# auxten/go-ctr

Measured on AMD Instinct MI355X. Metric: training samples/sec (DIN, MovieLens-20M-shaped synthetic), higher is better.
Workload: dtype f32

## Files before the change

goctr_amd/csrc/ctr.hip:

```cpp
#include <array>
#include <chrono>
#include <cmath>
#include <cstdlib>
#include <map>
#include <memory>

#include "ctr_model.h"
#include "ctr_chain.h"
#include "ctr_chain_x3.h"
#include "emb_train.h"
#include "scan.h"
#include "ctr_serve.h"
#include "mfma_gemm.h"

namespace {

struct TnSchedule { int rows, S, rows_light, S_light; };
TnSchedule tn_schedule(const goctr_model* m, int B) {
  TnSchedule t{};
  const int heavy = (int)cdiv(m->Ip / 16, 3) + (int)cdiv(m->H2p / 16, 3);
  const int light = m->cfg.kind == GOCTR_DIN ? 2 : 1;
  int cus = engine().compute_units > 0 ? engine().compute_units : 256;
  const int lf = 25;
  int rows = 32;
  for (;; rows += 4) {
    const long wgs = (long)heavy * cdiv(B, rows) + (long)light * cdiv(B, round_up(rows * lf / 10, 4));
    if (wgs <= cus || rows >= B) break;
  }
  t.rows = rows; t.S = (int)cdiv(B, rows);
  t.rows_light = round_up(rows * lf / 10, 4); t.S_light = (int)cdiv(B, t.rows_light);
  return t;
}
struct TnWide { bool ok; int ktw0, kblocks0, nbt; int rows0, S0, rows1, S1, rowsL, SL; };
TnWide tn_schedule_wide_search(const goctr_model* m, int B, int nsum);
constexpr int TN_SUM_SLABS = 8;
TnWide tn_schedule_wide(const goctr_model* m, int B, int nsum = 0) {
  static std::mutex mu;
  static std::map<std::array<int, 7>, TnWide> cache;
  const std::array<int, 7> key{B, m->Ip, m->H1p, m->H2p, m->cfg.kind, engine().compute_units, nsum};
  std::lock_guard<std::mutex> lk(mu);
  auto it = cache.find(key);
  if (it != cache.end()) return it->second;
  const TnWide w = tn_schedule_wide_search(m, B, nsum);
  cache.emplace(key, w);
  return w;
}
TnWide tn_schedule_wide_search(const goctr_model* m, int B, int nsum) {
  TnWide w{};
  const int kt0 = m->Ip / 16, nt = m->H1p / 16, kt1 = m->H2p / 16;
  w.ok = (kt0 == 9 || kt0 == 15) && kt1 == 5 && nt > 8 && nt <= 16;
  if (!w.ok) return w;
  w.ktw0 = kt0 == 9 ? 9 : 8; w.kblocks0 = (int)cdiv(kt0, w.ktw0); w.nbt = (int)cdiv(nt, 2);
  const int cols0 = w.ktw0 * 16 + w.nbt * 16, cols1 = kt1 * 16 + w.nbt * 16;
  const int colsL = 16 + kt1 * 16;
  const int blocks0 = w.kblocks0 * 2, blocks1 = 2, light = m->cfg.kind == GOCTR_DIN ? 2 : 1;
  const int cus = engine().compute_units > 0 ? engine().compute_units : 256;
  const int fix0 = 512, fix1 = 384, fixL = 384;
  long best = -1; int bc0 = 0, bc1 = 0, brl = 0;
  const int cmax = (int)cdiv(B, 32);
  for (int c0 = 1; c0 <= cmax; ++c0)
    for (int c1 = 1; c1 <= cmax; ++c1) {
      long t = std::max((long)c0 * cols0 + fix0, (long)c1 * cols1 + fix1);
      if (best >= 0 && t >= best) continue;
      const long heavy = (long)blocks0 * cdiv(B, c0 * 32) + (long)blocks1 * cdiv(B, c1 * 32);
      const int mlight = light - nsum;
      const long room = cus - heavy - (long)nsum * TN_SUM_SLABS;
      const long left = mlight > 0 ? room / mlight : 1;
      if (room < 0 || left < 1) continue;
      const int rl = std::max(32, round_up((int)cdiv(B, left), 4));
      if (mlight > 0) t = std::max(t, (long)cdiv(rl, 32) * colsL + fixL);
      if (best >= 0 && t >= best) continue;
      best = t; bc0 = c0; bc1 = c1; brl = rl;
    }
  if (best < 0) { bc0 = bc1 = cmax; brl = B; }
  w.rows0 = bc0 * 32; w.S0 = (int)cdiv(B, w.rows0);
  w.rows1 = bc1 * 32; w.S1 = (int)cdiv(B, w.rows1);
  w.rowsL = brl; w.SL = (int)cdiv(B, w.rowsL);
  return w;
}
int tn_max_slabs(int B) { return (int)cdiv(B, 32); }
bool dw_wide_path(const goctr_model* m, int B) {
  int nt_max = m->H1p / 16;
  if (m->H2p / 16 > nt_max) nt_max = m->H2p / 16;
  if (m->cfg.kind == GOCTR_DIN && m->Tp / 16 > nt_max) nt_max = m->Tp / 16;
  return gemm_tn_multi_fits(nt_max) && tn_schedule_wide(m, B).ok;
}

}
int ensure_workspace(goctr_model* m, int B) {
  if (m->wsB >= B && m->tnS > 0) return 0;
  const int S = tn_max_slabs(B);
  m->tnS = S;
  if (m->h0.alloc((size_t)B * m->Ip)) return -1;
  if (m->P0.alloc((size_t)B * m->H1p)) return -1;
  if (m->A0.alloc((size_t)B * m->H1p)) return -1;
  if (m->P1.alloc((size_t)B * m->H2p)) return -1;
  if (m->A1.alloc((size_t)B * m->H2p)) return -1;
  if (m->yhat.alloc((size_t)B)) return -1;
  if (m->lossrow.alloc((size_t)B)) return -1;
  if (m->dz2.alloc((size_t)B * 16)) return -1;
  if (m->dz1.alloc((size_t)B * m->H2p)) return -1;
  if (m->dz0.alloc((size_t)B * m->H1p)) return -1;
  if (m->dp.alloc((size_t)B * m->Dp)) return -1;
  if (m->gate.alloc((size_t)2 * B * m->cfg.T)) return -1;
  if (m->wgt.alloc((size_t)2 * B * m->cfg.T)) return -1;
  if (m->gfac.alloc((size_t)2 * B * m->cfg.T)) return -1;
  m->gw_stride = (size_t)B * m->cfg.T;
  if (m->ra_flag.alloc(1)) return -1;
  if (m->slabs0.alloc((size_t)S * m->Ip * m->H1p)) return -1;
  if (m->slabs1.alloc((size_t)S * m->H1p * m->H2p)) return -1;
  if (m->slabs2.alloc((size_t)S * m->H2p * 16)) return -1;
  m->attp_blocks = (int)cdiv(B, ATTN_BWD_WAVES);
  if (m->attp.alloc((size_t)B * m->Tp)) return -1;
  if (m->slabs3.alloc((size_t)S * 16 * m->Tp)) return -1;
  if (m->tile_dw2.alloc((size_t)S * m->H2p) || m->tile_att0.alloc((size_t)S * m->Tp)) return -1;
  {
    std::vector<float> ones((size_t)B * 16, 0.f);
    for (int r = 0; r < B; ++r) ones[(size_t)r * 16] = 1.0f;
    if (m->ones16.alloc(ones.size(), false) || m->ones16.upload(ones.data(), ones.size())) return -1;
  }
  m->wsB = B;
  m->graph.destroy();
  return 0;
}

RowSource make_source(const goctr_dataset* d, const goctr_emb* e) {
  RowSource s{};
  s.rows = d->rows;
  s.Y = d->has_y ? d->Y.p : nullptr;
  s.id_mode = d->id_mode ? 1 : 0;
  if (d->id_mode) {
    s.emb = e->rows.p; s.V = e->V;
    s.ub_ids = d->ub_ids.p; s.item_ids = d->item_ids.p; s.ufeat = d->ufeat.p; s.cfeat = d->cfeat.p;
  } else {
    s.X = d->X.p; s.xcols = d->xcols;
    s.r_u = d->ranges[0]; s.r_ub = d->ranges[2]; s.r_v = d->ranges[4]; s.r_c = d->ranges[6];
  }
  return s;
}
namespace {

int serve16_attributes() {
#define GOCTR_S16(L, H) (allow_big_lds(ctr_serve16_kernel<L, 1, H>) || allow_big_lds(ctr_serve16_kernel<L, 2, H>) || allow_big_lds(ctr_serve16_kernel<L, 3, H>))
  return (GOCTR_S16(2, 10) || GOCTR_S16(2, 15) || GOCTR_S16(4, 10) || GOCTR_S16(4, 15) || GOCTR_S16(16, 10) || GOCTR_S16(16, 15)) ? -1 : 0;
#undef GOCTR_S16
}

template <class Epi>
int launch_nn(int kid, const float* A, int lda, const float* Bm, int ldb, int M, int Kp, int Np, Epi epi) {
  const int NT = Np / 16;
  int WN = NT >= 2 ? 2 : 1;
  while (WN < 4 && (int)cdiv(NT, WN) > GEMM_NN_NTW) WN *= 2;
  int ntw = (int)cdiv(NT, WN);
  if (ntw > GEMM_NN_NTW) ntw = GEMM_NN_NTW;
  ntw = ntw <= 1 ? 1 : (ntw <= 3 ? 3 : (ntw <= 4 ? 4 : 7));
  const int WM = 4 / WN;
  dim3 grid((unsigned)cdiv(M, 16 * WM), (unsigned)cdiv(NT, WN * ntw));
  const int ncols_blk = std::min(NT, WN * ntw) * 16;
  (void)ncols_blk;
  const int ncols_alloc = WN * ntw * 16;
  const int KPH = gemm_nn_phase_rows<float>(Kp, ncols_alloc);
  const size_t lds = gemm_nn_lds_bytes<float>(KPH, ncols_alloc);
  hipStream_t st = engine().active;
  ProfScope ps(kid);
  if (KPH >= Kp && ntw == 4 && (int)grid.x >= 2 * engine().compute_units) {
    const dim3 g2((unsigned)engine().compute_units, grid.y);
    hipLaunchKernelGGL((gemm_nn_rows_kernel<float, Epi, 4>), g2, dim3(256), lds, st, A, lda, Bm, ldb, M, Kp, Np, WN, epi);
    GOCTR_HIP(hipGetLastError());
    return 0;
  }
#define GOCTR_NN(N) hipLaunchKernelGGL((gemm_nn_kernel<float, Epi, N>), grid, dim3(256), lds, st, A, lda, Bm, ldb, M, Kp, Np, WN, KPH, epi)
  switch (ntw) {
    case 1: GOCTR_NN(1); break;
    case 3: GOCTR_NN(3); break;
    case 4: GOCTR_NN(4); break;
    default: GOCTR_NN(7); break;
  }
#undef GOCTR_NN
  GOCTR_HIP(hipGetLastError());
  return 0;
}

template <int KTW, int NTW, int CH>
int launch_tn_cfg(const float* A, int lda, int KT, const float* Dm, int ldd, int NT, int M, int rows_per_wg,
                  int WK, int WN, float* slabs, size_t slab_stride) {
  const int S = (int)cdiv(M, rows_per_wg);
  const int nthreads = 64 * WK * WN;
  GOCTR_CHECK((size_t)CH * (WK * KTW * 16 / 4) <= (size_t)GEMM_TN_MAXVA * nthreads &&
              (size_t)CH * (WN * NTW * 16 / 4) <= (size_t)GEMM_TN_MAXVD * nthreads,
              "gemm_tn: chunk does not fit the staging registers (WK=%d WN=%d)", WK, WN);
  dim3 grid(S, (unsigned)cdiv(KT, WK * KTW), (unsigned)cdiv(NT, WN * NTW));
  hipLaunchKernelGGL((gemm_tn_kernel<float, KTW, NTW, CH>), grid, dim3(nthreads),
                     gemm_tn_lds_bytes<float>(WK * KTW, WN * NTW, CH), engine().active, A, lda, KT, Dm, ldd, NT, M,
                     rows_per_wg, WK, WN, slabs, slab_stride);
  GOCTR_HIP(hipGetLastError());
  return 0;
}

int launch_tn(int kid, const float* A, int lda, int KT, const float* Dm, int ldd, int NT, int M, int rows_per_wg,
              float* slabs, size_t slab_stride) {
  ProfScope ps(kid);
  if (NT <= 3) {
    const int WK = std::min(4, (int)cdiv(KT, 4));
    return launch_tn_cfg<4, 3, 16>(A, lda, KT, Dm, ldd, NT, M, rows_per_wg, WK, 1, slabs, slab_stride);
  }
  if (NT <= 6) {
    const int WK = std::min(4, (int)cdiv(KT, 4)), WN = std::min(2, (int)cdiv(NT, 3));
    return launch_tn_cfg<4, 3, 32>(A, lda, KT, Dm, ldd, NT, M, rows_per_wg, WK, WN, slabs, slab_stride);
  }
  const int WN = std::min(4, (int)cdiv(NT, 4));
  return launch_tn_cfg<3, 4, 32>(A, lda, KT, Dm, ldd, NT, M, rows_per_wg, 1, WN, slabs, slab_stride);
}

}
int init_kernel_attrs() {
  bool& done = engine().kernel_attrs_done;
  if (done) return 0;
#define GOCTR_NN_ATTR(E) (allow_big_lds(gemm_nn_kernel<float, E, 1>) || allow_big_lds(gemm_nn_kernel<float, E, 3>) || \
                          allow_big_lds(gemm_nn_kernel<float, E, 4>) || allow_big_lds(gemm_nn_kernel<float, E, 7>) || \
                          allow_big_lds(gemm_nn_rows_kernel<float, E, 4>))
  if (GOCTR_NN_ATTR(EpiSigDrop) || GOCTR_NN_ATTR(EpiOut) || GOCTR_NN_ATTR(EpiDSig) || GOCTR_NN_ATTR(EpiStore) ||
      allow_big_lds(ctr_chain_kernel<7, 5, 0>) || allow_big_lds(ctr_chain_kernel<7, 5, 1>) ||
      allow_big_lds(ctr_chain_kernel<7, 5, 2>) || allow_big_lds(ctr_fwd16_kernel<4, 5>) || allow_big_lds(emb_grad_kernel<16, 0>) || allow_big_lds(emb_grad_kernel<16, 1>) || allow_big_lds(emb_grad_kernel<16, 2>) || allow_big_lds(emb_grad_kernel<32, 0>) ||
      allow_big_lds(emb_grad_kernel<32, 1>) || allow_big_lds(emb_grad_kernel<32, 2>) || allow_big_lds(emb_grad_kernel<64, 0>) || allow_big_lds(emb_grad_kernel<64, 1>) ||
      allow_big_lds(emb_grad_kernel<64, 2>) || allow_big_lds(gemm_tn_kernel<float, 4, 3, 16>) || allow_big_lds(gemm_tn_kernel<float, 4, 3, 32>) ||
      allow_big_lds(gemm_tn_kernel<float, 3, 4, 32>) ||
      allow_big_lds(gemm_tn_multi_x3_kernel<3, 4>) || allow_big_lds(gemm_tn_multi_x3w_kernel<9, 5>) || allow_big_lds(gemm_tn_multi_x3w_kernel<8, 5>) ||
      allow_big_lds(gemm_tn_multi_x3w_att0_kernel<9, 5>) || allow_big_lds(gemm_tn_multi_x3w_att0_kernel<8, 5>) || allow_big_lds(ctr_chain_x3_kernel<2>) || allow_big_lds(ctr_chain_x3_kernel<9>) ||
      allow_big_lds(ctr_chain_x3_kernel<15>) || chain_x3_fwd_attributes() || fwd4_attributes() ||
      serve16_attributes()) return -1;
  done = true;
  return 0;
}
namespace {

int launch_attn_fwd(const AttnArgs& a) {
  ProfScope ps(GOCTR_K_ATTN_FWD);
  dim3 grid((unsigned)cdiv(a.B, 4)), blk(256);
  hipStream_t st = engine().active;
  const bool vec4 = a.src.id_mode && a.D % 4 == 0;
  const int groups = vec4 ? a.D / 4 : a.D;
  const bool small_table = (unsigned long long)(a.src.V + 1) * (unsigned long long)a.D * 4ull < (1ull << 32);
  const int fast = !(vec4 && small_table && groups * 4 == a.D && (groups & (groups - 1)) == 0) ? 0
                   : a.kind != GOCTR_DIN ? 1 : (a.att == GOCTR_ATT_COSINE ? 2 : 3);
  if (ps.on) {
    static char sym[48];
    int L = 1;
    while (L < groups) L *= 2;
    if (!vec4 && L < 8) L = 8;
    if (a.src.k_users) snprintf(sym, sizeof sym, "attn_fwd_keys_kernel<%d,%d>", std::min(L, 64), fast);
    else snprintf(sym, sizeof sym, "attn_fwd_kernel<%d,%d,%d>", vec4 ? 4 : 1, std::min(L, 64), (fast && groups <= 16) ? fast : 0);
    prof_note_kernel(GOCTR_K_ATTN_FWD, sym);
  }
  if (a.src.k_users) {
    if (!(fast && groups <= 16)) { set_error("attn_fwd: key mode needs an id-mode fast shape"); return -1; }
#define GOCTR_ATTN_KEYS(L)                                                                         \
  do {                                                                                             \
    if (fast == 1) hipLaunchKernelGGL((attn_fwd_keys_kernel<L, 1>), grid, blk, 0, st, a);          \
    else if (fast == 2) hipLaunchKernelGGL((attn_fwd_keys_kernel<L, 2>), grid, blk, 0, st, a);     \
    else hipLaunchKernelGGL((attn_fwd_keys_kernel<L, 3>), grid, blk, 0, st, a);                    \
  } while (0)
    if (groups == 1) GOCTR_ATTN_KEYS(1);
    else if (groups == 2) GOCTR_ATTN_KEYS(2);
    else if (groups == 4) GOCTR_ATTN_KEYS(4);
    else if (groups == 8) GOCTR_ATTN_KEYS(8);
    else GOCTR_ATTN_KEYS(16);
#undef GOCTR_ATTN_KEYS
    GOCTR_HIP(hipGetLastError());
    return 0;
  }
#define GOCTR_ATTN_FWD(V, L) hipLaunchKernelGGL((attn_fwd_kernel<V, L, 0>), grid, blk, 0, st, a)
#define GOCTR_ATTN_FWD_FAST(L)                                                                     \
  do {                                                                                             \
    if (fast == 1) hipLaunchKernelGGL((attn_fwd_kernel<4, L, 1>), grid, blk, 0, st, a);            \
    else if (fast == 2) hipLaunchKernelGGL((attn_fwd_kernel<4, L, 2>), grid, blk, 0, st, a);       \
    else hipLaunchKernelGGL((attn_fwd_kernel<4, L, 3>), grid, blk, 0, st, a);                      \
  } while (0)
  if (fast && groups <= 16) {
    if (groups == 1) GOCTR_ATTN_FWD_FAST(1);
    else if (groups == 2) GOCTR_ATTN_FWD_FAST(2);
    else if (groups == 4) GOCTR_ATTN_FWD_FAST(4);
    else if (groups == 8) GOCTR_ATTN_FWD_FAST(8);
    else GOCTR_ATTN_FWD_FAST(16);
  } else
  if (vec4) {
    if (groups <= 1) GOCTR_ATTN_FWD(4, 1);
    else if (groups <= 2) GOCTR_ATTN_FWD(4, 2);
    else if (groups <= 4) GOCTR_ATTN_FWD(4, 4);
    else if (groups <= 8) GOCTR_ATTN_FWD(4, 8);
    else if (groups <= 16) GOCTR_ATTN_FWD(4, 16);
    else if (groups <= 32) GOCTR_ATTN_FWD(4, 32);
    else GOCTR_ATTN_FWD(4, 64);
  } else {
    if (groups <= 8) GOCTR_ATTN_FWD(1, 8);
    else if (groups <= 16) GOCTR_ATTN_FWD(1, 16);
    else if (groups <= 32) GOCTR_ATTN_FWD(1, 32);
    else GOCTR_ATTN_FWD(1, 64);
  }
#undef GOCTR_ATTN_FWD_FAST
#undef GOCTR_ATTN_FWD
  GOCTR_HIP(hipGetLastError());
  return 0;
}

int launch_attn_bwd(const AttnBwdArgs& a, int blocks) {
  ProfScope ps(GOCTR_K_ATTN_BWD);
  dim3 grid((unsigned)blocks), blk(64 * ATTN_BWD_WAVES);
  hipStream_t st = engine().active;
  const size_t lds = 0;
  const bool vec4 = a.src.id_mode && a.D % 4 == 0;
  const int groups = vec4 ? a.D / 4 : a.D;
  const bool fast = vec4 && groups * 4 == a.D && (groups & (groups - 1)) == 0 && groups <= 16;
#define GOCTR_ATTN_BWD(V, L) hipLaunchKernelGGL((attn_bwd_kernel<V, L, 0>), grid, blk, lds, st, a)
#define GOCTR_ATTN_BWD_FAST(L) hipLaunchKernelGGL((attn_bwd_kernel<4, L, 1>), grid, blk, lds, st, a)
  if (fast) {
    if (groups == 1) GOCTR_ATTN_BWD_FAST(1);
    else if (groups == 2) GOCTR_ATTN_BWD_FAST(2);
    else if (groups == 4) GOCTR_ATTN_BWD_FAST(4);
    else if (groups == 8) GOCTR_ATTN_BWD_FAST(8);
    else GOCTR_ATTN_BWD_FAST(16);
  } else
  if (vec4) {
    if (groups <= 1) GOCTR_ATTN_BWD(4, 1);
    else if (groups <= 2) GOCTR_ATTN_BWD(4, 2);
    else if (groups <= 4) GOCTR_ATTN_BWD(4, 4);
    else if (groups <= 8) GOCTR_ATTN_BWD(4, 8);
    else if (groups <= 16) GOCTR_ATTN_BWD(4, 16);
    else if (groups <= 32) GOCTR_ATTN_BWD(4, 32);
    else GOCTR_ATTN_BWD(4, 64);
  } else {
    if (groups <= 8) GOCTR_ATTN_BWD(1, 8);
    else if (groups <= 16) GOCTR_ATTN_BWD(1, 16);
    else if (groups <= 32) GOCTR_ATTN_BWD(1, 32);
    else GOCTR_ATTN_BWD(1, 64);
  }
#undef GOCTR_ATTN_BWD_FAST
#undef GOCTR_ATTN_BWD
  GOCTR_HIP(hipGetLastError());
  return 0;
}

}
bool chain_ok(const goctr_model* m) {
  const int nt0 = m->H1p / 16;
  return (nt0 == 13 || nt0 == 14) && m->H2p == 80 && (m->cfg.kind != GOCTR_DIN || m->Dp <= 16 * CHAIN_NDP) &&
         m->Ip <= 16 * CHAIN_HV &&
         chain_lds_bytes<5>(m->Ip, m->H1p, m->H2p) <= 160u * 1024u &&
         env_int("GOCTR_NO_CHAIN", 0) == 0;
}
namespace {

bool chain_x3_ok(const goctr_model* m, const StepOpts& o, int B) {
  if (m->x3_nch0 == 0) return false;
  if (o.train) return o.drop_mode != 1;
  const int cus = engine().compute_units > 0 ? engine().compute_units : 256;
  return cdiv(B, 32) >= cus;
}

}
int rebuild_x3_images(goctr_model* m) {
  if (!m->x3_nch0) return 0;
  hipLaunchKernelGGL(x3_build_images_kernel, dim3((unsigned)cdiv(m->off2, 256)), dim3(256), 0, engine().stream, m->W.p, m->off1, m->off2,
                     m->H1p, m->H2p, m->cfg.U, m->cfg.D, m->x3_images());
  GOCTR_HIP(hipGetLastError());
  return 0;
}
namespace {

template <int NCH0>
void launch_chain_x3_n(const ChainX3Args& a, dim3 grid, hipStream_t s, bool fwd) {
  if (fwd) launch_chain_x3_fwd(NCH0, a, grid, s);
  else hipLaunchKernelGGL((ctr_chain_x3_kernel<NCH0, false>), grid, dim3(512), chain_x3_lds_bytes<NCH0>(), s, a);
}

bool emb_plan_active(const goctr_model* m) { return m->emb_lr > 0.f && m->plan.valid; }

bool gate_fac_mode(const goctr_model* m, const RowSource& src, const StepOpts& o, int B);
int launch_chain_x3(goctr_model* m, const RowSource& src, int B, const StepOpts& o, const StepState* st, const FwdBufs& fb) {
  const goctr_ctr_cfg& c = m->cfg;
  Engine& e = engine();
  const uint32_t row_off = (uint32_t)(e.eff_rank() * B);
  const bool drop = o.drop_mode == 2;
  const CxImages im = m->x3_images();
  ChainX3Args a{};
  a.h0 = fb.h0; a.Ip = m->Ip;
  a.img0 = im.img0; a.img1 = im.img1; a.img2 = im.img2; a.img3 = im.img3; a.w2 = m->W2T.p;
  a.H1 = c.H1; a.H2 = c.H2; a.H1p = m->H1p; a.H2p = m->H2p; a.Dp = m->Dp; a.B = B; a.kind = c.kind;
  a.d0 = DropCfg{drop && o.p0 > 0 ? 2 : 0, o.p0, nullptr, c.H1, o.seed, 0u, row_off};
  a.d1 = DropCfg{drop && o.p1 > 0 ? 2 : 0, o.p1, nullptr, c.H2, o.seed, 1u, row_off};
  a.st = st; a.Y = src.Y; a.rows = src.rows; a.inv_bglobal = 1.0f / (float)(B * e.eff_world());
  a.A0 = m->A0.p; a.A1 = m->A1.p; a.dz0 = m->dz0.p; a.dz1 = m->dz1.p; a.dz2 = m->dz2.p; a.dp = m->dp.p;
  m->dpv_from_chain = o.train && emb_plan_active(m) && src.id_mode && c.kind == GOCTR_DIN && 2 * c.D <= 32;
  if (m->dpv_from_chain) { a.dp = m->dpv.p; a.Dp = round_up(2 * c.D, 16); }
  m->attn_bwd_in_chain = o.train && c.kind == GOCTR_DIN && src.id_mode && !emb_plan_active(m) && c.D == 16 && c.T <= 64 &&
                         env_int("GOCTR_CHAIN_ATTN_BWD", 1) != 0;
  if (m->attn_bwd_in_chain) {
    a.ab_ids = src.ub_ids; a.ab_emb = src.emb; a.ab_V = src.V; a.ab_gate = fb.gate; a.ab_wgt = fb.wgt; a.ab_out = m->attp.p;
    a.ab_fac = gate_fac_mode(m, src, o, B) ? fb.fac : nullptr;
    a.ab_T = c.T; a.ab_Tp = m->Tp;
  }
  a.yhat = fb.yhat; a.lossrow = m->lossrow.p;
  const bool tile_sums = o.train && dw_wide_path(m, B) && env_int("GOCTR_CHAIN_TILE_SUMS", 1) != 0;
  m->dw2_from_chain = tile_sums;
  m->att0_from_chain = tile_sums && m->attn_bwd_in_chain;
  a.tile_dw2 = m->dw2_from_chain ? m->tile_dw2.p : nullptr;
  a.tile_att0 = m->att0_from_chain ? m->tile_att0.p : nullptr;
  static DevBuf<unsigned long long> dbgbuf;
  const bool dbg = dbg_on("chain") && (hipStream_t)e.active == e.stream;
  if (dbg && !dbgbuf.p && dbgbuf.alloc(4096)) return -1;
  a.dbg = dbg ? dbgbuf.p : nullptr;
  ProfScope ps(GOCTR_K_CHAIN);
  const int ntiles = (int)cdiv(B, 32);
  const bool persist = !o.train && e.compute_units > 0;
  const bool fwd4 = !o.train && ntiles > e.compute_units && env_int("GOCTR_FWD4", 1) != 0;
  const dim3 grid((unsigned)(persist ? std::min(ntiles, (fwd4 ? 2 : 1) * e.compute_units) : ntiles));
  static const char* const kSym[3][2] = {{"ctr_chain_x3_kernel<2,false>", "ctr_chain_x3_kernel<2,true>"},
                                         {"ctr_chain_x3_kernel<9,false>", "ctr_chain_x3_kernel<9,true>"},
                                         {"ctr_chain_x3_kernel<15,false>", "ctr_chain_x3_kernel<15,true>"}};
  if (ps.on) prof_note_kernel(GOCTR_K_CHAIN, fwd4 ? (m->x3_nch0 == 2 ? "ctr_fwd4_kernel<2,false>" : m->x3_nch0 == 9 ? "ctr_fwd4_kernel<9,false>" : "ctr_fwd4_kernel<15,true>")
                                                  : kSym[m->x3_nch0 == 2 ? 0 : m->x3_nch0 == 9 ? 1 : 2][o.train ? 0 : 1]);
  if (fwd4) launch_fwd4(m->x3_nch0, a, grid, e.active);
  else
  switch (m->x3_nch0) {
    case 2: launch_chain_x3_n<2>(a, grid, e.active, !o.train); break;
    case 9: launch_chain_x3_n<9>(a, grid, e.active, !o.train); break;
    default: launch_chain_x3_n<15>(a, grid, e.active, !o.train); break;
  }
  GOCTR_HIP(hipGetLastError());
  if (dbg) {
    unsigned long long h[CX_NSTAMP];
    if (dbgbuf.download(h, CX_NSTAMP)) return -1;
    if (fwd4) {
      fprintf(stderr, "fwd4 phases (s_memtime ticks): h0 split+barrier %lld | F0 %lld | epi0+F1 %lld | xchg barrier %lld | epi1+z2 %lld | total %lld\n",
              (long long)(h[1] - h[0]), (long long)(h[2] - h[1]), (long long)(h[3] - h[2]), (long long)(h[4] - h[3]), (long long)(h[5] - h[4]),
              (long long)(h[5] - h[0]));
      fprintf(stderr, "fwd4 workgroup 0: %lld shader cycles in %.2f us (100 MHz clock) = %.2f GHz\n", (long long)(h[5] - h[6]),
              (double)(h[8] - h[7]) * 0.01, (double)(h[5] - h[6]) / ((double)(h[8] - h[7]) * 10.0));
      std::vector<unsigned long long> all(4096);
      if (dbgbuf.download(all.data(), 4096)) return -1;
      std::vector<double> life; std::vector<unsigned long long> where;
      for (unsigned b = 0; b < grid.x && b < 960; ++b) {
        life.push_back((double)(all[128 + 4 * b + 1] - all[128 + 4 * b]) * 0.01);
        where.push_back((all[128 + 4 * b + 3] & 0xf) << 16 | (all[128 + 4 * b + 2] & 0xff00));
      }
      std::sort(life.begin(), life.end()); std::sort(where.begin(), where.end());
      const size_t cus = (size_t)(std::unique(where.begin(), where.end()) - where.begin());
      if (!life.empty())
        fprintf(stderr, "fwd4 workgroups: %zu on %zu CUs, lifetimes min %.2f / median %.2f / max %.2f us\n", life.size(), cus, life.front(),
                life[life.size() / 2], life.back());
    } else if (!o.train) {
      fprintf(stderr, "chain_x3 forward-only phases (s_memtime ticks): h0 split+barrier %lld | F0 %lld | epi0 %lld | F1 %lld | xchg barrier %lld | epi1+z2 %lld | total %lld\n",
              (long long)(h[1] - h[0]), (long long)(h[2] - h[1]), (long long)(h[3] - h[2]), (long long)(h[4] - h[3]), (long long)(h[5] - h[4]),
              (long long)(h[6] - h[5]), (long long)(h[6] - h[0]));
      fprintf(stderr, "chain_x3 forward-only workgroup 0: %lld shader cycles in %.2f us (100 MHz clock) = %.2f GHz\n", (long long)(h[6] - h[14]),
              (double)(h[13] - h[15]) * 0.01, (double)(h[6] - h[14]) / ((double)(h[13] - h[15]) * 10.0));
    } else {
      fprintf(stderr, "chain_x3 phases (s_memtime ticks): h0 split+barrier %lld | F0(+epi tile0) %lld | F1(+epi tile1) %lld | xchg barrier %lld | epi1+z2+dz1 %lld | B0(+epi) %lld | dp %lld + xchg %lld | total %lld\n",
              (long long)(h[1] - h[0]), (long long)(h[2] - h[1]), (long long)(h[4] - h[2]), (long long)(h[5] - h[4]), (long long)(h[6] - h[5]),
              (long long)(h[7] - h[6]), (long long)(h[8] - h[7]), (long long)(h[9] > h[8] ? h[9] - h[8] : 0),
              (long long)((h[9] > h[8] ? h[9] : h[8]) - h[0]));
    }
  }
  return 0;
}

ChainArgs make_chain_args(goctr_model* m, const RowSource& src, int B, const StepOpts& o, const StepState* st, const FwdBufs& fb) {
  const goctr_ctr_cfg& c = m->cfg;
  Engine& e = engine();
  const uint32_t row_off = (uint32_t)(e.eff_rank() * B);
  const bool drop = o.train && o.drop_mode != 0;
  ChainArgs a{};
  a.h0 = fb.h0; a.Ip = m->Ip;
  a.W0i = m->img(0); a.W1i = m->img(1); a.W1Ti = m->img(2); a.W0sTi = m->img(3); a.w2 = m->W2T.p;
  a.H1 = c.H1; a.H2 = c.H2; a.H1p = m->H1p; a.H2p = m->H2p; a.Dp = m->Dp; a.B = B;
  a.train = o.train ? 1 : 0; a.kind = c.kind;
  a.d0 = DropCfg{drop && o.p0 > 0 ? o.drop_mode : 0, o.p0, m->mask0.p, c.H1, o.seed, 0u, row_off};
  a.d1 = DropCfg{drop && o.p1 > 0 ? o.drop_mode : 0, o.p1, m->mask1.p, c.H2, o.seed, 1u, row_off};
  a.st = st; a.Y = src.Y; a.rows = src.rows; a.inv_bglobal = 1.0f / (float)(B * e.eff_world());
  a.buf_floats = chain_buf_floats(m->Ip, m->H1p, m->H2p);
  a.A0 = m->A0.p; a.A1 = m->A1.p; a.dz0 = m->dz0.p; a.dz1 = m->dz1.p; a.dz2 = m->dz2.p; a.dp = m->dp.p;
  a.yhat = fb.yhat; a.lossrow = m->lossrow.p;
  return a;
}

AttnArgs make_attn_args(goctr_model* m, const RowSource& src, int B, const StepState* st, const FwdBufs& fb, bool fac);
}
bool serve16_ok(const goctr_model* m, const RowSource& src, int B) {
  int groups = 0;
  const int fast = attn_fast_mode(m, src, &groups);
  StepOpts o; o.train = false;
  return src.k_users && fast != 0 && (groups == 2 || groups == 4 || groups == 16) && chain_ok(m) && !chain_x3_ok(m, o, B) &&
         cdiv(B, 32) < engine().compute_units && env_int("GOCTR_SERVE_ONE_LAUNCH", 1) != 0;
}
int launch_serve16(goctr_model* m, const RowSource& src, int B, const StepState* st, const FwdBufs& fb, unsigned* done, unsigned epoch) {
  int groups = 0;
  const int fast = attn_fast_mode(m, src, &groups);
  StepOpts o; o.train = false;
  ChainArgs a = make_chain_args(m, src, B, o, st, fb);
  a.done = done; a.epoch = epoch;
  AttnArgs aa = make_attn_args(m, src, B, st, fb, false);
  aa.gate = nullptr; aa.wgt = nullptr;
  const size_t lds = chain_lds_bytes<5>(m->Ip, m->H1p, m->H2p);
  const dim3 grid((unsigned)cdiv(B, 16)), blk(1024);
  hipStream_t s = engine().active;
#define GOCTR_SERVE16_H(L, H)                                                                          \
  do {                                                                                                 \
    if (fast == 1) hipLaunchKernelGGL((ctr_serve16_kernel<L, 1, H>), grid, blk, lds, s, aa, a);        \
    else if (fast == 2) hipLaunchKernelGGL((ctr_serve16_kernel<L, 2, H>), grid, blk, lds, s, aa, a);   \
    else hipLaunchKernelGGL((ctr_serve16_kernel<L, 3, H>), grid, blk, lds, s, aa, a);                  \
  } while (0)
#define GOCTR_SERVE16(L) do { if (m->Ip <= 160) GOCTR_SERVE16_H(L, 10); else GOCTR_SERVE16_H(L, 15); } while (0)
  if (groups == 2) GOCTR_SERVE16(2);
  else if (groups == 4) GOCTR_SERVE16(4);
  else GOCTR_SERVE16(16);
#undef GOCTR_SERVE16_H
#undef GOCTR_SERVE16
  GOCTR_HIP(hipGetLastError());
  return 0;
}
namespace {

int launch_chain(goctr_model* m, const RowSource& src, int B, const StepOpts& o, const StepState* st, const FwdBufs& fb) {
  if (chain_x3_ok(m, o, B)) return launch_chain_x3(m, src, B, o, st, fb);
  Engine& e = engine();
  ChainArgs a = make_chain_args(m, src, B, o, st, fb);
  static DevBuf<unsigned long long> dbgbuf;
  const bool dbg = o.train && dbg_on("chain");
  if (dbg && !dbgbuf.p && dbgbuf.alloc(CHAIN_NSTAMP)) return -1;
  a.dbg = dbg ? dbgbuf.p : nullptr;
  ProfScope ps(GOCTR_K_CHAIN);
  const dim3 grid((unsigned)cdiv(B, 32));
  const size_t lds = chain_lds_bytes<5>(m->Ip, m->H1p, m->H2p);
  const int dmode = (a.d0.mode || a.d1.mode) ? o.drop_mode : 0;
  if (!o.train && cdiv(B, 32) < e.compute_units) {
    if (ps.on) prof_note_kernel(GOCTR_K_CHAIN, "ctr_fwd16_kernel<4,5>");
    hipLaunchKernelGGL((ctr_fwd16_kernel<4, 5>), dim3((unsigned)cdiv(B, 16)), dim3(512), lds, e.active, a);
  } else
  if (dmode == 0) { if (ps.on) prof_note_kernel(GOCTR_K_CHAIN, "ctr_chain_kernel<7,5,0>"); hipLaunchKernelGGL((ctr_chain_kernel<7, 5, 0>), grid, dim3(512), lds, e.active, a); }
  else if (dmode == 1) { if (ps.on) prof_note_kernel(GOCTR_K_CHAIN, "ctr_chain_kernel<7,5,1>"); hipLaunchKernelGGL((ctr_chain_kernel<7, 5, 1>), grid, dim3(512), lds, e.active, a); }
  else { if (ps.on) prof_note_kernel(GOCTR_K_CHAIN, "ctr_chain_kernel<7,5,2>"); hipLaunchKernelGGL((ctr_chain_kernel<7, 5, 2>), grid, dim3(512), lds, e.active, a); }
  GOCTR_HIP(hipGetLastError());
  if (dbg) {
    unsigned long long h[CHAIN_NSTAMP];
    if (dbgbuf.download(h, CHAIN_NSTAMP)) return -1;
    fprintf(stderr, "chain phases (s_memtime ticks):");
    for (int k = 1; k < 10; ++k) fprintf(stderr, " %d:%lld", k, (long long)(h[k] - h[k - 1]));
    fprintf(stderr, " | ph0 mma %lld bar %lld | ph1 mma %lld bar %lld | F1 mma+xw %lld bar %lld", (long long)(h[10] - h[1]), (long long)(h[2] - h[10]),
            (long long)(h[11] - h[2]), (long long)(h[3] - h[11]), (long long)(h[12] - h[4]), (long long)(h[13] - h[12]));
    fprintf(stderr, "  total %lld\n", (long long)(h[9] - h[0]));
  }
  return 0;
}

FwdBufs train_bufs(goctr_model* m, int par) { return FwdBufs{m->h0.p, m->gate_p(par), m->wgt_p(par), m->yhat.p, m->P0.p, m->P1.p, m->gfac_p(par)}; }
bool gate_fac_mode(const goctr_model* m, const RowSource& src, const StepOpts& o, int B) {
  const goctr_ctr_cfg& c = m->cfg;
  return o.train && c.kind == GOCTR_DIN && src.id_mode && m->emb_lr <= 0.f && c.D == 16 && c.T <= 64 && chain_ok(m) &&
         chain_x3_ok(m, o, B) && env_int("GOCTR_CHAIN_ATTN_BWD", 1) != 0;
}
AttnArgs make_attn_args(goctr_model* m, const RowSource& src, int B, const StepState* st, const FwdBufs& fb, bool fac) {
  const goctr_ctr_cfg& c = m->cfg;
  AttnArgs aa{};
  aa.src = src; aa.st = st; aa.B = B; aa.U = c.U; aa.T = c.T; aa.D = c.D; aa.C = c.C; aa.Ip = m->Ip;
  aa.kind = c.kind; aa.att = c.att; aa.att0 = m->W.p + m->offa; aa.h0 = fb.h0; aa.gate = fb.gate; aa.wgt = fb.wgt;
  aa.Tp_att = m->Tp;
  aa.inv_T = 1.0f / (float)c.T;
  if (fac && fb.fac) { aa.fac = fb.fac; aa.gate = nullptr; aa.wgt = nullptr; }
  return aa;
}
AttnArgs make_attn_args(goctr_model* m, const RowSource& src, int B, const StepState* st, int par, bool fac) {
  return make_attn_args(m, src, B, st, train_bufs(m, par), fac);
}

}
int attn_fast_mode(const goctr_model* m, const RowSource& src, int* groups) {
  const goctr_ctr_cfg& c = m->cfg;
  const bool vec4 = src.id_mode && c.D % 4 == 0;
  const int g = vec4 ? c.D / 4 : c.D;
  if (groups) *groups = g;
  const bool small_table = (unsigned long long)(src.V + 1) * (unsigned long long)c.D * 4ull < (1ull << 32);
  return !(vec4 && small_table && g * 4 == c.D && (g & (g - 1)) == 0) ? 0 : c.kind != GOCTR_DIN ? 1 : (c.att == GOCTR_ATT_COSINE ? 2 : 3);
}
namespace {
bool pipeline_ok(const goctr_model* m, const RowSource& src) {
  int groups = 0;
  const int fast = attn_fast_mode(m, src, &groups);
  const bool one_block = m->cfg.kind != GOCTR_DIN || (m->offa * 2) / 256 == ((m->offa + m->Tp) * 2 - 1) / 256;
  if (engine().comm_active()) {
    const bool one_adam_block = m->cfg.kind != GOCTR_DIN || m->offa / 256 == (m->offa + m->Tp - 1) / 256;
    return fast != 0 && (groups == 4 || groups == 16) && one_adam_block && chain_ok(m) && m->emb_lr <= 0.f &&
           env_int("GOCTR_PIPELINE", 1) != 0;
  }
  return fast != 0 && (groups == 4 || groups == 16) && one_block && chain_ok(m) &&
         env_int("GOCTR_PIPELINE", 1) != 0;
}

int launch_reduce_attn(goctr_model* m, const RowSource& src, int B, const StepOpts& o, const ReduceAdamArgs& p) {
  int groups = 0;
  const int fast = attn_fast_mode(m, src, &groups);
  const AttnArgs aa = make_attn_args(m, src, B, p.r.st, m->stp ^ 1, gate_fac_mode(m, src, o, B));
  const int nred = (int)cdiv((int64_t)m->nflat * 2, 256) + 1;
  const dim3 grid((unsigned)(nred + cdiv(B, 4))), blk(256);
  hipStream_t st = engine().active;
#define GOCTR_RA(L)                                                                                        \
  do {                                                                                                     \
    if (fast == 1) hipLaunchKernelGGL((reduce_attn_kernel<4, L, 1>), grid, blk, 0, st, p, aa, nred);       \
    else if (fast == 2) hipLaunchKernelGGL((reduce_attn_kernel<4, L, 2>), grid, blk, 0, st, p, aa, nred);  \
    else hipLaunchKernelGGL((reduce_attn_kernel<4, L, 3>), grid, blk, 0, st, p, aa, nred);                 \
  } while (0)
  if (groups == 4) GOCTR_RA(4);
  else GOCTR_RA(16);
#undef GOCTR_RA
  GOCTR_HIP(hipGetLastError());
  return 0;
}

}
int launch_forward(goctr_model* m, const RowSource& src, int B, const StepOpts& o, const StepState* st_override,
                   const FwdBufs* fbp) {
  const goctr_ctr_cfg& c = m->cfg;
  Engine& e = engine();
  const StepState* st = st_override ? st_override : m->st_cur();
  const FwdBufs fb = fbp ? *fbp : train_bufs(m, m->stp);
  if (!o.pipelined) {
    AttnArgs aa = make_attn_args(m, src, B, st, fb, gate_fac_mode(m, src, o, B));
    if (!o.train) { aa.gate = nullptr; aa.wgt = nullptr; }
    if (launch_attn_fwd(aa)) return -1;
  }
  if (o.train) { m->dpv_from_chain = false; m->attn_bwd_in_chain = false; m->dw2_from_chain = false; m->att0_from_chain = false; m->att0_early = false; }
  if (chain_ok(m)) return launch_chain(m, src, B, o, st, fb);

  const int bglobal = B * e.eff_world();
  const uint32_t row_off = (uint32_t)(e.eff_rank() * B);
  const bool drop = o.train && o.drop_mode != 0;
  DropCfg d0{drop && o.p0 > 0 ? o.drop_mode : 0, o.p0, m->mask0.p, c.H1, o.seed, 0u, row_off};
  DropCfg d1{drop && o.p1 > 0 ? o.drop_mode : 0, o.p1, m->mask1.p, c.H2, o.seed, 1u, row_off};
  EpiSigDrop e0{fb.P0, d0.mode ? m->A0.p : fb.P0, m->H1p, c.H1, d0, st};
  if (launch_nn(GOCTR_K_GEMM_FWD0, fb.h0, m->Ip, m->W.p, m->H1p, B, m->Ip, m->H1p, e0)) return -1;
  const float* A0 = d0.mode ? m->A0.p : fb.P0;
  EpiSigDrop e1{fb.P1, d1.mode ? m->A1.p : fb.P1, m->H2p, c.H2, d1, st};
  if (launch_nn(GOCTR_K_GEMM_FWD1, A0, m->H1p, m->W.p + m->off1, m->H2p, B, m->H1p, m->H2p, e1)) return -1;
  const float* A1 = d1.mode ? m->A1.p : fb.P1;
  EpiOut eo{fb.yhat, o.train ? m->lossrow.p : nullptr, o.train ? m->dz2.p : nullptr, src.Y, src.rows, st, B,
            1.0f / (float)bglobal};
  if (launch_nn(GOCTR_K_GEMM_OUT, A1, m->H2p, m->W.p + m->off2, 16, B, m->H2p, 16, eo)) return -1;
  return 0;
}
namespace {

AdamArgs make_adam_args(goctr_model* m, int B, const goctr_train_cfg& tc);

int ensure_emb_workspace(goctr_model* m, long long V, int B) {
  if (m->emb_lr <= 0.f || (m->emb_V == V && m->emb_B == B && m->emb_world == engine().eff_world() &&
                           m->emb_comm == engine().comm_active())) return 0;
  const goctr_ctr_cfg& c = m->cfg;
  const int Np = round_up(2 * c.D, 16);
  const int W = engine().comm_active() ? engine().eff_world() : 1;
  const long long Vw = round_up((int)cdiv(V, W), 4);
  const long long Vp = Vw * W;
  const long long cap = std::min<long long>(V, (long long)B * (c.T + 1));
  if (m->dpv.alloc((size_t)B * Np) || m->W0pvT.alloc((size_t)m->H1p * Np) || m->emb_mark.alloc((size_t)Vp) ||
      m->emb_rank.alloc((size_t)Vp, false) || m->emb_total.alloc(1) || m->emb_accum.alloc((size_t)cap * c.D) ||
      m->emb_slot_id.alloc((size_t)cap, false) || m->emb_tiles.alloc((size_t)cdiv(Vp, SCAN_TILE), false))
    return -1;
  if (engine().comm_active()) {
    if (m->ex_off.alloc(W + 1) || m->ex_cnt.alloc(W) || m->ex_allcnt.alloc((size_t)W * W) || m->ex_nred.alloc(1) ||
        m->ex_allnred.alloc(W) || m->ex_red_total.alloc(1)) return -1;
  }
  GOCTR_HIP(hipStreamSynchronize(engine().stream));
  m->emb_V = V; m->emb_B = B; m->emb_world = engine().eff_world(); m->emb_comm = engine().comm_active(); m->emb_Vw = Vw;
  m->w0pv_live = false; m->plan.valid = false;
  m->graph.destroy();
  return 0;
}

template <int GS>
void launch_emb_grad(int mode, dim3 gb, size_t lds, hipStream_t s, const EmbTrainArgs& a, int nslot) {
  if (mode == 0) hipLaunchKernelGGL((emb_grad_kernel<GS, 0>), gb, dim3(EMB_GRAD_THREADS), lds, s, a, nslot);
  else if (mode == 1) hipLaunchKernelGGL((emb_grad_kernel<GS, 1>), gb, dim3(EMB_GRAD_THREADS), lds, s, a, nslot);
  else hipLaunchKernelGGL((emb_grad_kernel<GS, 2>), gb, dim3(EMB_GRAD_THREADS), lds, s, a, nslot);
}

int launch_emb_exchange(goctr_model* m, const EmbTrainArgs& a) {
  Engine& e = engine();
  const int W = e.eff_world(), r = e.eff_rank(), D = a.D;
  hipStream_t s = e.stream;
  hipLaunchKernelGGL(emb_bucket_bounds_kernel, dim3(1), dim3(64), 0, s, m->emb_slot_id.p, m->emb_total.p, W, m->ex_off.p, m->ex_cnt.p);
  GOCTR_HIP(hipGetLastError());
  if (comm_allgather_i32(m->ex_cnt.p, m->ex_allcnt.p, (size_t)W)) return -1;
  std::vector<int> off(W + 1), allcnt((size_t)W * W);
  if (m->ex_off.download(off.data(), W + 1) || m->ex_allcnt.download(allcnt.data(), (size_t)W * W)) return -1;
  std::vector<size_t> so(W), sc(W), ro(W), rc(W);
  size_t nrecv = 0;
  for (int p = 0; p < W; ++p) {
    so[p] = (size_t)off[p]; sc[p] = (size_t)(off[p + 1] - off[p]);
    ro[p] = nrecv; rc[p] = (size_t)allcnt[(size_t)p * W + r]; nrecv += rc[p];
  }
  if (m->ex_rids.ensure(nrecv, false) || m->ex_rrows.ensure(nrecv * D, false)) return -1;
  if (comm_alltoallv(m->emb_slot_id.p, so.data(), sc.data(), m->ex_rids.p, ro.data(), rc.data(), 4)) return -1;
  std::vector<size_t> soD(W), scD(W), roD(W), rcD(W);
  for (int p = 0; p < W; ++p) { soD[p] = so[p] * D; scD[p] = sc[p] * D; roD[p] = ro[p] * D; rcD[p] = rc[p] * D; }
  if (comm_alltoallv(m->emb_accum.p, soD.data(), scD.data(), m->ex_rrows.p, roD.data(), rcD.data(), 8)) return -1;
  double sent = 0;
  for (int p = 0; p < W; ++p) sent += (double)sc[p] * (4 + 8.0 * D);
  GOCTR_HIP(hipMemsetAsync(m->emb_accum.p, 0, sizeof(long long) * (size_t)off[W] * D, s));
  const size_t cap_red = std::min<size_t>((size_t)m->emb_Vw, nrecv);
  if (m->ex_red.n < cap_red * D || !m->ex_red.p) { if (m->ex_red.alloc(std::max<size_t>(cap_red * D, 1))) return -1; }
  if (m->ex_red_ids.ensure(std::max<size_t>(cap_red, 1), false) || m->ex_delta.ensure(std::max<size_t>(cap_red * D, 1), false)) return -1;
  if (nrecv) {
    hipLaunchKernelGGL(emb_recv_mark_kernel, dim3((unsigned)cdiv((long long)nrecv, 256)), dim3(256), 0, s, m->ex_rids.p, (long long)nrecv, W,
                       m->emb_Vw, m->emb_mark.p);
    GOCTR_HIP(hipGetLastError());
  }
  if (exclusive_scan_sink(m->emb_mark.p + (size_t)r * m->emb_Vw, m->emb_Vw, m->emb_tiles, m->ex_red_total.p, EmbMultiMap{},
                          EmbRankSink{m->emb_mark.p, m->emb_rank.p, m->ex_red_ids.p, W, m->emb_Vw, (long long)r * m->emb_Vw})) return -1;
  if (nrecv) {
    hipLaunchKernelGGL(emb_recv_accumulate_kernel, dim3((unsigned)cdiv((long long)nrecv * D, 256)), dim3(256), 0, s, m->ex_rids.p,
                       m->ex_rrows.p, (long long)nrecv, D, W, m->emb_Vw, m->emb_rank.p, m->ex_red.p);
    GOCTR_HIP(hipGetLastError());
  }
  const int cus = e.compute_units > 0 ? e.compute_units : 256;
  hipLaunchKernelGGL(emb_delta_kernel, dim3((unsigned)std::min<long long>(std::max<long long>(cdiv((long long)cap_red * D, 256), 1), 16 * cus)),
                     dim3(256), 0, s, m->ex_red.p, m->ex_red_total.p, D, a.lr, m->ex_delta.p);
  GOCTR_HIP(hipGetLastError());
  hipLaunchKernelGGL(emb_count_to_i32_kernel, dim3(1), dim3(1), 0, s, m->ex_red_total.p, m->ex_nred.p);
  GOCTR_HIP(hipGetLastError());
  if (comm_allgather_i32(m->ex_nred.p, m->ex_allnred.p, 1)) return -1;
  std::vector<int> nred(W);
  if (m->ex_allnred.download(nred.data(), W)) return -1;
  std::vector<size_t> go(W), gc(W), zo(W, 0), mine(W);
  size_t ng = 0;
  for (int p = 0; p < W; ++p) { go[p] = ng; gc[p] = (size_t)nred[p]; ng += gc[p]; mine[p] = (size_t)nred[r]; }
  if (m->ex_gids.ensure(std::max<size_t>(ng, 1), false) || m->ex_gdelta.ensure(std::max<size_t>(ng * D, 1), false)) return -1;
  if (comm_alltoallv(m->ex_red_ids.p, zo.data(), mine.data(), m->ex_gids.p, go.data(), gc.data(), 4)) return -1;
  std::vector<size_t> goD(W), gcD(W), mineD(W);
  for (int p = 0; p < W; ++p) { goD[p] = go[p] * D; gcD[p] = gc[p] * D; mineD[p] = mine[p] * D; }
  if (comm_alltoallv(m->ex_delta.p, zo.data(), mineD.data(), m->ex_gdelta.p, goD.data(), gcD.data(), 4)) return -1;
  sent += (double)W * nred[r] * (4 + 4.0 * D);
  m->ex_bytes_last = sent;
  if (ng) {
    hipLaunchKernelGGL(emb_apply_gathered_kernel, dim3((unsigned)std::min<long long>(cdiv((long long)ng * D, 256), 16 * cus)), dim3(256), 0, s,
                       a.emb, m->ex_gids.p, m->ex_gdelta.p, (long long)ng, D);
    GOCTR_HIP(hipGetLastError());
  }
  return 0;
}

bool emb_plan_ok(const goctr_model* m, int B) {
  const goctr_ctr_cfg& c = m->cfg;
  const bool lay = c.kind != GOCTR_DIN || c.D == 4 || c.D == 8 || c.D == 16 || c.D == 32 || c.D == 64;
  return lay && c.D <= 64 && c.T < (1 << EMB_PAIR_TBITS) && B < (1 << (31 - EMB_PAIR_TBITS)) && env_int("GOCTR_EMB_PLAN", 1) != 0;
}

bool emb_plan_fits(const goctr_model* m, const goctr_dataset* d, long long V, int B) {
  const long long per = m->cfg.T + 1, nb = cdiv(d->rows, B);
  const double bytes = 12.0 * (double)(nb * B * per) + 8.0 * (double)(nb * std::min<long long>((long long)B * per, V));
  const double budget = (double)env_int("GOCTR_EMB_PLAN_MAX_MB", 32768) * 1048576.0;
  if (bytes <= budget) return true;
  static std::atomic<bool> said{false};
  if (!said.exchange(true))
    fprintf(stderr, "goctr: the sparse plan of this dataset would take %.1f GB (> GOCTR_EMB_PLAN_MAX_MB = %d): embedding training "
            "uses the atomics path\n", bytes / 1073741824.0, env_int("GOCTR_EMB_PLAN_MAX_MB", 32768));
  return false;
}

int ensure_emb_plan(goctr_model* m, const goctr_dataset* d, const RowSource& src, int B) {
  Engine& e = engine();
  const goctr_ctr_cfg& c = m->cfg;
  const int W = e.comm_active() ? e.eff_world() : 1;
  auto& P = m->plan;
  if (P.valid && P.ds == d->uid && P.V == src.V && P.B == B && P.W == W && P.T == c.T) return 0;
  P.valid = false;
  hipStream_t s = e.stream;
  GOCTR_HIP(hipStreamSynchronize(s));
  m->graph.destroy();
  const long long Vw = m->emb_Vw;
  const long long nb = cdiv(d->rows, B), per = c.T + 1;
  const size_t np_cap = (size_t)(nb * B * per), ns_cap = (size_t)(nb * std::min<long long>((long long)B * per, src.V));
  if (P.pair.alloc(np_cap, false) || P.pslot.alloc(np_cap, false) || P.pid.alloc(np_cap, false) || P.slot_id.alloc(ns_cap, false) ||
      P.slot_off.alloc(ns_cap + (size_t)nb, false) || P.pair_off.alloc((size_t)nb + 1, false) || P.slot_base.alloc((size_t)nb + 1, false)) return -1;
  long long tot[4] = {0, 0, 0, 0};
  const auto t_build = std::chrono::steady_clock::now();
  {
    ProfScope ps(GOCTR_K_EMB_PLAN);
    if (emb_plan_build(EmbPlanSource{src.ub_ids, src.item_ids, src.rows, src.V}, B, c.T, W, Vw, nb,
                       EmbPlanArrays{P.pair.p, P.pslot.p, P.pid.p, P.slot_id.p, P.slot_off.p, P.pair_off.p, P.slot_base.p}, tot)) return -1;
  }
  const long long max_pairs = tot[2], max_slots = tot[3];
  P.build_ms = std::chrono::duration<double, std::milli>(std::chrono::steady_clock::now() - t_build).count();
  if (c.kind == GOCTR_DIN && (m->emb_dx.ensure((size_t)B * c.T * c.D, false) || m->emb_gsum.ensure((size_t)B * c.D, false))) return -1;
  if (e.comm_active()) {
    GOCTR_CHECK(W <= 1023, "world %d too large for the bucket kernel", W);
    if (m->ex_bucket_off.alloc((size_t)nb * (W + 1), false)) return -1;
    hipLaunchKernelGGL(emb_plan_buckets_kernel, dim3((unsigned)nb), dim3((unsigned)round_up(W + 1, 64)), 0, s, P.view(), nb, W, m->ex_bucket_off.p);
    GOCTR_HIP(hipGetLastError());
    std::vector<int> boff((size_t)nb * (W + 1));
    if (m->ex_bucket_off.download(boff.data(), boff.size())) return -1;
    int smax = 1;
    for (long long k = 0; k < nb; ++k)
      for (int o = 0; o < W; ++o) smax = std::max(smax, boff[(size_t)k * (W + 1) + o + 1] - boff[(size_t)k * (W + 1) + o]);
    DevBuf<int> one, all;
    if (one.alloc(1, false) || all.alloc((size_t)W, false) || one.upload(&smax, 1)) return -1;
    if (comm_allgather_i32(one.p, all.p, 1)) return -1;
    std::vector<int> hs((size_t)W);
    if (all.download(hs.data(), (size_t)W)) return -1;
    for (int v : hs) smax = std::max(smax, v);
    const int S = round_up(smax, 4);
    const long long R = std::min<long long>(Vw, (long long)W * S);
    m->ex_S = S; m->ex_R = (int)R;
    const size_t ws = (size_t)W * S, wr = (size_t)W * (size_t)R;
    if (m->ex_send_ids.alloc(ws, false) || m->ex_recv_ids.alloc(ws, false) || m->ex_send_rows.alloc(ws * c.D, false) ||
        m->ex_recv_rows.alloc(ws * c.D, false) || m->ex_red.alloc(std::max<size_t>((size_t)R * c.D, 1)) ||
        m->ex_red_ids.alloc(std::max<size_t>((size_t)R, 1), false) || m->ex_delta.alloc(std::max<size_t>((size_t)R * c.D, 1), false) ||
        m->ex_gids.alloc(std::max<size_t>(wr, 1), false) || m->ex_gdelta.alloc(std::max<size_t>(wr * c.D, 1), false)) return -1;
    GOCTR_HIP(hipStreamSynchronize(s));
    m->ex_bytes_last = (double)W * S * (4 + 8.0 * c.D) + (double)W * (double)R * (4 + 4.0 * c.D);
  }
  P.ds = d->uid; P.V = src.V; P.B = B; P.W = W; P.T = c.T; P.nb = nb; P.max_pairs = max_pairs; P.max_slots = max_slots;
  P.total_pairs = tot[0]; P.total_slots = tot[1];
  P.valid = true;
  return 0;
}

template <int GS, int VEC>
int launch_emb_slot_gv(int mode, bool direct, long long max_pairs, hipStream_t s, const EmbSlotArgs& a) {
  const long long wgp = EmbSlotGeo<GS, VEC>::WGP;
  const dim3 grid((unsigned)std::max<long long>(cdiv(max_pairs, wgp), 1));
#define GOCTR_SLOT(M) do { if (direct) hipLaunchKernelGGL((emb_slot_kernel<GS, VEC, M, true>), grid, dim3(EMB_SLOT_THREADS), 0, s, a); \
                           else hipLaunchKernelGGL((emb_slot_kernel<GS, VEC, M, false>), grid, dim3(EMB_SLOT_THREADS), 0, s, a); } while (0)
  if (mode == 0) GOCTR_SLOT(0); else GOCTR_SLOT(1);
#undef GOCTR_SLOT
  GOCTR_HIP(hipGetLastError());
  if (direct) {
    const long long borders = std::max<long long>(cdiv(a.B * (long long)(a.T + 1), wgp), 1);
    hipLaunchKernelGGL(emb_span_apply_kernel, dim3((unsigned)cdiv(borders * a.D, 256)), dim3(256), 0, s, a, wgp);
    GOCTR_HIP(hipGetLastError());
  }
  return 0;
}
bool emb_slot_vec4(const goctr_model* m) {
  const goctr_ctr_cfg& c = m->cfg;
  const int want = c.kind != GOCTR_DIN ? 4 : 1;
  return (c.D == 16 || c.D == 32 || c.D == 64) && want == 4;
}

int launch_emb_plan_early(goctr_model* m, const RowSource& src, int B, const StepState* st) {
  const goctr_ctr_cfg& c = m->cfg;
  hipStream_t s = engine().stream;
  const int Np = round_up(2 * c.D, 16);
  if (!m->dpv_from_chain) {
    EpiStore sp{m->dpv.p, Np};
    if (launch_nn(GOCTR_K_EMB_TRAIN, m->dz0.p, m->H1p, m->W0pvT.p, Np, B, m->H1p, Np, sp)) return -1;
  }
  if (c.kind != GOCTR_DIN) return 0;
  const int mode = c.att == GOCTR_ATT_COSINE ? 1 : 2;
  ProfScope ps(GOCTR_K_ATTN_BWD);
  if (ps.on) { static char sym[40]; snprintf(sym, sizeof sym, "emb_coef_kernel<%d,%d>", c.D / 4, mode); prof_note_kernel(GOCTR_K_ATTN_BWD, sym); }
  EmbCoefArgs ca{src, st, B, c.T, c.D, m->dpv.p, Np, m->gate_p(m->stp), m->W.p + m->offa, m->emb_dx.p, m->emb_gsum.p,
                 m->wgt_p(m->stp), m->attp.p, m->Tp};
  const dim3 g((unsigned)cdiv(B, 4));
  const int lpr = c.D / 4;
#define GOCTR_COEF(L) do { if (mode == 1) hipLaunchKernelGGL((emb_coef_kernel<L, 1>), g, dim3(256), 0, s, ca); \
                           else hipLaunchKernelGGL((emb_coef_kernel<L, 2>), g, dim3(256), 0, s, ca); } while (0)
  if (lpr == 1) GOCTR_COEF(1); else if (lpr == 2) GOCTR_COEF(2); else if (lpr == 4) GOCTR_COEF(4); else if (lpr == 8) GOCTR_COEF(8); else GOCTR_COEF(16);
#undef GOCTR_COEF
  GOCTR_HIP(hipGetLastError());
  return 0;
}

int launch_emb_plan_step(goctr_model* m, const RowSource& src, int B, const StepState* st, int Np) {
  const goctr_ctr_cfg& c = m->cfg;
  Engine& e = engine();
  hipStream_t s = e.stream;
  const int mode = c.kind != GOCTR_DIN ? 0 : (c.att == GOCTR_ATT_COSINE ? 1 : 2);
  const bool direct = !e.comm_active();
  EmbSlotArgs a{};
  a.plan = m->plan.view(); a.st = st; a.B = B; a.T = c.T; a.D = c.D; a.dpv = m->dpv.p; a.ldp = Np;
  a.dx = m->emb_dx.p; a.gsum = m->emb_gsum.p;
  a.emb = const_cast<float*>(src.emb); a.accum = m->emb_accum.p; a.lr = m->emb_lr;
  {
    ProfScope ps(GOCTR_K_EMB_GRAD);
    if (ps.on) {
      static char sym[48];
      const bool v4 = emb_slot_vec4(m);
      snprintf(sym, sizeof sym, "emb_slot_kernel<%d,%d,%d,%s>", v4 ? c.D / 4 : (c.D <= 16 ? 16 : c.D <= 32 ? 32 : 64), v4 ? 4 : 1, mode ? 1 : 0,
               direct ? "true" : "false");
      prof_note_kernel(GOCTR_K_EMB_GRAD, sym);
    }
    const long long mp = m->plan.max_pairs;
    int rc;
    if (emb_slot_vec4(m)) rc = c.D == 16 ? launch_emb_slot_gv<4, 4>(mode, direct, mp, s, a) : c.D == 32 ? launch_emb_slot_gv<8, 4>(mode, direct, mp, s, a)
                                                                                                        : launch_emb_slot_gv<16, 4>(mode, direct, mp, s, a);
    else rc = c.D <= 16 ? launch_emb_slot_gv<16, 1>(mode, direct, mp, s, a) : c.D <= 32 ? launch_emb_slot_gv<32, 1>(mode, direct, mp, s, a)
                                                                                         : launch_emb_slot_gv<64, 1>(mode, direct, mp, s, a);
    if (rc) return -1;
  }
  if (direct) return 0;
  const int cus = e.compute_units > 0 ? e.compute_units : 256;
  const long long n = (long long)e.eff_world() * m->ex_S * c.D;
  hipLaunchKernelGGL(emb_pack_send_kernel, dim3((unsigned)std::min<long long>(std::max<long long>(cdiv(n, 256), 1), 8 * cus)), dim3(256), 0, s,
                     m->plan.view(), st, m->ex_bucket_off.p, e.eff_world(), m->ex_S, c.D, m->emb_accum.p, m->ex_send_ids.p, m->ex_send_rows.p);
  GOCTR_HIP(hipGetLastError());
  return 0;
}

int launch_emb_train(goctr_model* m, const RowSource& src, int B, const StepState* st) {
  const goctr_ctr_cfg& c = m->cfg;
  Engine& e = engine();
  GOCTR_CHECK(src.id_mode, "embedding training needs an id-mode dataset (the dense TrainSample rows carry no ids)");
  GOCTR_CHECK(c.D <= 64, "embedding training supports D <= 64 (got %d)", c.D);
  const int Np = round_up(2 * c.D, 16);
  const long long V = src.V;
  const long long cap = std::min<long long>(V, (long long)B * (c.T + 1));
  GOCTR_CHECK(m->emb_V == V && m->emb_B == B && m->emb_world == e.eff_world() && m->emb_comm == e.comm_active(),
              "embedding-training workspace not prepared (ensure_emb_workspace)");
  const int W = e.comm_active() ? e.eff_world() : 1;
  EmbTrainArgs a{};
  a.src = src; a.st = st; a.B = B; a.T = c.T; a.D = c.D; a.kind = c.kind; a.att = c.att;
  a.dpv = m->dpv.p; a.ldp = Np; a.gate = m->gate_p(m->stp); a.wgt = m->wgt_p(m->stp); a.att0 = m->W.p + m->offa;
  a.emb = const_cast<float*>(src.emb); a.V = V;
  a.mark = m->emb_mark.p; a.rank = m->emb_rank.p; a.accum = m->emb_accum.p; a.lr = m->emb_lr; a.dbg = 0;
  a.W = W; a.Vw = m->emb_Vw;
  hipStream_t s = e.stream;
  if (m->plan.valid) {
    return launch_emb_plan_step(m, src, B, st, Np);
  }
  {
  ProfScope ps(GOCTR_K_EMB_TRAIN);
  const long long pairs = (long long)B * (c.T + 1);
  const int singles = env_int("GOCTR_EMB_SINGLES", (!e.comm_active() && V > pairs) ? 1 : 0) != 0 && !e.comm_active();
  hipLaunchKernelGGL(emb_mark_kernel, dim3((unsigned)cdiv(pairs, 256)), dim3(256), 0, s, a, singles);
  if (singles) hipLaunchKernelGGL(emb_mark2_kernel, dim3((unsigned)cdiv(pairs, 256)), dim3(256), 0, s, a);
  GOCTR_HIP(hipGetLastError());
  if (exclusive_scan_sink(m->emb_mark.p, m->emb_Vw * W, m->emb_tiles, m->emb_total.p, EmbMultiMap{},
                          EmbRankSink{m->emb_mark.p, m->emb_rank.p, m->emb_slot_id.p, W, m->emb_Vw, 0})) return -1;
  hipLaunchKernelGGL(w0pv_transpose_kernel, dim3((unsigned)cdiv((long long)m->H1p * Np, 256)), dim3(256), 0, s, m->W.p, m->H1p,
                     c.U, 2 * c.D, Np, m->W0pvT.p);
  GOCTR_HIP(hipGetLastError());
  }
  EpiStore sp{m->dpv.p, Np};
  if (launch_nn(GOCTR_K_EMB_TRAIN, m->dz0.p, m->H1p, m->W0pvT.p, Np, B, m->H1p, Np, sp)) return -1;
  const int mode = c.kind != GOCTR_DIN ? 0 : (c.att == GOCTR_ATT_COSINE ? 1 : 2);
  int nslot = 1;
  while ((size_t)nslot * 2 * (c.D * sizeof(long long) + sizeof(int)) <= 136u * 1024u) nslot *= 2;
  const size_t lds = (size_t)nslot * (c.D * sizeof(long long) + sizeof(int));
  const int cus = e.compute_units > 0 ? e.compute_units : 256;
  const dim3 gb((unsigned)std::min<long long>(cdiv(B, EMB_GRAD_THREADS / 64), cus));
  {
    ProfScope ps(GOCTR_K_EMB_GRAD);
    if (ps.on) {
      static char sym[48];
      snprintf(sym, sizeof sym, "emb_grad_kernel<%d,%d>", c.D <= 16 ? 16 : c.D <= 32 ? 32 : 64, mode);
      prof_note_kernel(GOCTR_K_EMB_GRAD, sym);
    }
    if (c.D <= 16) launch_emb_grad<16>(mode, gb, lds, s, a, nslot);
    else if (c.D <= 32) launch_emb_grad<32>(mode, gb, lds, s, a, nslot);
    else launch_emb_grad<64>(mode, gb, lds, s, a, nslot);
  }
  if (e.comm_active()) return launch_emb_exchange(m, a);
  ProfScope ps(GOCTR_K_EMB_TRAIN);
  hipLaunchKernelGGL(emb_apply_kernel, dim3((unsigned)std::min<long long>(cdiv(cap * c.D, 256), 16 * cus)), dim3(256), 0, s, a,
                     m->emb_slot_id.p, m->emb_total.p);
  GOCTR_HIP(hipGetLastError());
  return 0;
}

bool emb_split3(const goctr_model* m) { return engine().comm_active() && m->emb_lr > 0.f && m->plan.valid; }
int emb_exchange_a2a(goctr_model* m) {
  Engine& e = engine();
  const int W = e.eff_world(), D = m->cfg.D;
  std::vector<size_t> off((size_t)W), cnt((size_t)W), offD((size_t)W), cntD((size_t)W);
  for (int p = 0; p < W; ++p) { off[p] = (size_t)p * m->ex_S; cnt[p] = (size_t)m->ex_S; offD[p] = off[p] * D; cntD[p] = cnt[p] * D; }
  ProfScope ps(GOCTR_K_ALLREDUCE);
  if (comm_alltoallv(m->ex_send_ids.p, off.data(), cnt.data(), m->ex_recv_ids.p, off.data(), cnt.data(), 4)) return -1;
  return comm_alltoallv(m->ex_send_rows.p, offD.data(), cntD.data(), m->ex_recv_rows.p, offD.data(), cntD.data(), 8);
}
int emb_exchange_owner(goctr_model* m) {
  Engine& e = engine();
  const int W = e.eff_world(), r = e.eff_rank(), D = m->cfg.D;
  hipStream_t s = e.stream;
  const long long nrecv = (long long)W * m->ex_S;
  const int cus = e.compute_units > 0 ? e.compute_units : 256;
  ProfScope ps(GOCTR_K_EMB_TRAIN);
  hipLaunchKernelGGL(emb_recv_mark_kernel, dim3((unsigned)cdiv(nrecv, 256)), dim3(256), 0, s, m->ex_recv_ids.p, nrecv, W, m->emb_Vw, m->emb_mark.p);
  GOCTR_HIP(hipGetLastError());
  if (exclusive_scan_sink(m->emb_mark.p + (size_t)r * m->emb_Vw, m->emb_Vw, m->emb_tiles, m->ex_red_total.p, EmbMultiMap{},
                          EmbRankSink{m->emb_mark.p, m->emb_rank.p, m->ex_red_ids.p, W, m->emb_Vw, (long long)r * m->emb_Vw})) return -1;
  hipLaunchKernelGGL(emb_recv_accumulate_kernel, dim3((unsigned)cdiv(nrecv * D, 256)), dim3(256), 0, s, m->ex_recv_ids.p, m->ex_recv_rows.p,
                     nrecv, D, W, m->emb_Vw, m->emb_rank.p, m->ex_red.p);
  hipLaunchKernelGGL(emb_delta_kernel, dim3((unsigned)std::min<long long>(std::max<long long>(cdiv((long long)m->ex_R * D, 256), 1), 16 * cus)), dim3(256), 0, s,
                     m->ex_red.p, m->ex_red_total.p, D, m->emb_lr, m->ex_delta.p);
  hipLaunchKernelGGL(emb_pad_ids_kernel, dim3((unsigned)std::min<long long>(std::max<long long>(cdiv((long long)m->ex_R, 256), 1), 4 * cus)), dim3(256), 0, s,
                     m->ex_red_ids.p, m->ex_red_total.p, m->ex_R);
  GOCTR_HIP(hipGetLastError());
  return 0;
}
int emb_exchange_gather(goctr_model* m) {
  const int D = m->cfg.D;
  ProfScope ps(GOCTR_K_ALLREDUCE);
  if (comm_allgather_i32(m->ex_red_ids.p, m->ex_gids.p, (size_t)m->ex_R)) return -1;
  return comm_allgather_i32(reinterpret_cast<const int*>(m->ex_delta.p), reinterpret_cast<int*>(m->ex_gdelta.p), (size_t)m->ex_R * D);
}
int emb_exchange_apply(goctr_model* m, const RowSource& src) {
  Engine& e = engine();
  const int D = m->cfg.D;
  const long long ng = (long long)e.eff_world() * m->ex_R;
  const int cus = e.compute_units > 0 ? e.compute_units : 256;
  ProfScope ps(GOCTR_K_EMB_TRAIN);
  hipLaunchKernelGGL(emb_apply_gathered_kernel, dim3((unsigned)std::min<long long>(std::max<long long>(cdiv(ng * D, 256), 1), 16 * cus)), dim3(256), 0, e.stream,
                     const_cast<float*>(src.emb), m->ex_gids.p, m->ex_gdelta.p, ng, D);
  GOCTR_HIP(hipGetLastError());
  return 0;
}

int launch_reduce_part(goctr_model* m, const RowSource& src, int B, const StepOpts& o, bool advance, bool fuse_update, const ReduceArgs& ra);
}
int launch_backward(goctr_model* m, const RowSource& src, int B, const StepOpts& o, bool advance,
                    bool fuse_update, int stage) {
  const goctr_ctr_cfg& c = m->cfg;
  Engine& e = engine();
  if (stage == 2) return launch_reduce_part(m, src, B, o, advance, fuse_update, m->pend_ra);
  const StepState* st = m->st_cur();
  const uint32_t row_off = (uint32_t)(e.eff_rank() * B);
  const bool drop = o.drop_mode != 0;
  DropCfg d0{drop && o.p0 > 0 ? o.drop_mode : 0, o.p0, m->mask0.p, c.H1, o.seed, 0u, row_off};
  DropCfg d1{drop && o.p1 > 0 ? o.drop_mode : 0, o.p1, m->mask1.p, c.H2, o.seed, 1u, row_off};
  const float* A0 = d0.mode ? m->A0.p : m->P0.p;
  const float* A1 = d1.mode ? m->A1.p : m->P1.p;
  const TnSchedule ts = tn_schedule(m, B);
  const int rpw = ts.rows, S = ts.S, rpl = ts.rows_light, SL = ts.S_light;

  const bool fused = chain_ok(m);
  if (fused) {
    A0 = m->A0.p; A1 = m->A1.p;
  } else {
    EpiDSig b1{m->dz1.p, m->P1.p, m->H2p, c.H2, d1, st};
    if (launch_nn(GOCTR_K_BWD_DZ1, m->dz2.p, 16, m->W2T.p, m->H2p, B, 16, m->H2p, b1)) return -1;
    EpiDSig b0{m->dz0.p, m->P0.p, m->H1p, c.H1, d0, st};
    if (launch_nn(GOCTR_K_BWD_DZ0, m->dz1.p, m->H2p, m->W1T.p, m->H1p, B, m->H2p, m->H1p, b0)) return -1;
  }
  if (c.kind == GOCTR_DIN) {
    if (!fused) {
      EpiStore sp{m->dp.p, m->Dp};
      if (launch_nn(GOCTR_K_BWD_DP, m->dz0.p, m->H1p, m->W0sT.p, m->Dp, B, m->H1p, m->Dp, sp)) return -1;
    }
    if (emb_plan_active(m) && src.id_mode) {
      if (launch_emb_plan_early(m, src, B, st)) return -1;
    } else if (fused && m->attn_bwd_in_chain) {
    } else {
      AttnBwdArgs ab{};
      ab.src = src; ab.st = st; ab.B = B; ab.T = c.T; ab.D = c.D; ab.Dp = m->Dp; ab.Tp = m->Tp;
      ab.dp = m->dp.p; ab.gate = m->gate_p(m->stp); ab.wgt = m->wgt_p(m->stp); ab.partial = m->attp.p;
      if (launch_attn_bwd(ab, (int)cdiv(B, ATTN_BWD_WAVES))) return -1;
    }
  } else if (emb_plan_active(m) && src.id_mode) {
    if (launch_emb_plan_early(m, src, B, st)) return -1;
  }

  int nt_max = m->H1p / 16;
  if (m->H2p / 16 > nt_max) nt_max = m->H2p / 16;
  if (c.kind == GOCTR_DIN && m->Tp / 16 > nt_max) nt_max = m->Tp / 16;
  const bool multi = gemm_tn_multi_fits(nt_max);
  const TnWide tw = multi ? tn_schedule_wide(m, B, (m->dw2_from_chain ? 1 : 0) + (m->att0_from_chain ? 1 : 0)) : TnWide{};
  int S0 = S, S1 = S, SLx = SL;
  int SL2x = -1, SL3x = -1;
  if (multi && tw.ok) {
    TnMulti tm{};
    tm.M = B; tm.np = 3;
    const int b0 = tw.kblocks0 * 2 * tw.S0, b1 = 2 * tw.S1;
    tm.p[0] = {m->h0.p, m->Ip, m->Ip / 16, m->dz0.p, m->H1p, m->H1p / 16, m->slabs0.p,
               (unsigned long long)m->Ip * m->H1p, 0, m->H1p, 0, tw.rows0, tw.S0, 2, tw.nbt};
    tm.p[1] = {m->dz1.p, m->H2p, m->H2p / 16, A0, m->H1p, m->H1p / 16, m->slabs1.p,
               (unsigned long long)m->H1p * m->H2p, 1, m->H2p, b0, tw.rows1, tw.S1, 2, tw.nbt};
    const int ntiles = (int)cdiv(B, 32);
    const int nsum = std::min(TN_SUM_SLABS, ntiles), tps = (int)cdiv(ntiles, nsum);
    int SL2 = tw.SL, SL3 = tw.SL;
    if (m->dw2_from_chain) {
      SL2 = (int)cdiv(ntiles, tps);
      tm.p[2] = {nullptr, m->H2p, 0, m->tile_dw2.p, m->H2p, 0, m->slabs2.p, (unsigned long long)m->H2p * 16, 1, 16, b0 + b1, tps, SL2, 0, 0};
    } else {
      tm.p[2] = {m->dz2.p, 16, 1, A1, m->H2p, m->H2p / 16, m->slabs2.p, (unsigned long long)m->H2p * 16, 1, 16,
                 b0 + b1, tw.rowsL, tw.SL, 0, 0};
    }
    int nblk = b0 + b1 + SL2;
    m->att0_early = c.kind == GOCTR_DIN && m->att0_from_chain && o.pipelined && fuse_update && stage == 0 && !e.comm_active() &&
                    m->Tp % 32 == 0;
    Att0EarlyArgs ae{};
    if (m->att0_early) {
      ae.tile_att0 = m->tile_att0.p; ae.ntiles = ntiles; ae.Tp = m->Tp; ae.tps = tps; ae.nslabs = (int)cdiv(ntiles, tps);
      ae.ad = make_adam_args(m, B, *o.tc); ae.st = st;
    } else
    if (c.kind == GOCTR_DIN) {
      if (m->att0_from_chain) {
        SL3 = (int)cdiv(ntiles, tps);
        tm.p[3] = {nullptr, m->Tp, 0, m->tile_att0.p, m->Tp, 0, m->slabs3.p, (unsigned long long)16 * m->Tp, 0, m->Tp, nblk, tps, SL3, 0, 0};
      } else {
        tm.p[3] = {m->ones16.p, 16, 1, m->attp.p, m->Tp, m->Tp / 16, m->slabs3.p, (unsigned long long)16 * m->Tp, 0, m->Tp,
                   nblk, tw.rowsL, tw.SL, 0, 0};
      }
      tm.np = 4;
      nblk += SL3;
    }
    static DevBuf<unsigned long long> tndbgw;
    const bool dbg = dbg_on("tn");
    if (dbg && !tndbgw.p && tndbgw.alloc(16)) return -1;
    tm.dbg = dbg ? tndbgw.p : nullptr;
    {
      ProfScope ps(GOCTR_K_DW0);
      if (ps.on) prof_note_kernel(GOCTR_K_DW0, tw.ktw0 == 9 ? "gemm_tn_multi_x3w_kernel<9,5>" : "gemm_tn_multi_x3w_kernel<8,5>");
      if (m->att0_early) {
        if (ps.on) prof_note_kernel(GOCTR_K_DW0, tw.ktw0 == 9 ? "gemm_tn_multi_x3w_att0_kernel<9,5>" : "gemm_tn_multi_x3w_att0_kernel<8,5>");
        if (tw.ktw0 == 9)
          hipLaunchKernelGGL((gemm_tn_multi_x3w_att0_kernel<9, 5>), dim3((unsigned)nblk + 1), dim3(512), gemm_tn_multi_x3w_lds_bytes<9>(), e.stream, tm, ae);
        else
          hipLaunchKernelGGL((gemm_tn_multi_x3w_att0_kernel<8, 5>), dim3((unsigned)nblk + 1), dim3(512), gemm_tn_multi_x3w_lds_bytes<8>(), e.stream, tm, ae);
      } else
      if (tw.ktw0 == 9)
        hipLaunchKernelGGL((gemm_tn_multi_x3w_kernel<9, 5>), dim3((unsigned)nblk), dim3(512), gemm_tn_multi_x3w_lds_bytes<9>(), e.stream, tm);
      else
        hipLaunchKernelGGL((gemm_tn_multi_x3w_kernel<8, 5>), dim3((unsigned)nblk), dim3(512), gemm_tn_multi_x3w_lds_bytes<8>(), e.stream, tm);
      GOCTR_HIP(hipGetLastError());
    }
    if (dbg) {
      unsigned long long h[16];
      if (tndbgw.download(h, 16)) return -1;
      fprintf(stderr, "dW x3w (rows %d/%d/%d, %d workgroups) wg 0: multiplier wave: wait for chunk 0 %lld, in MFMA sections %lld, loop total %lld, "
              "epilogue %lld | stager wave: first chunk %lld, staging sections %lld, total %lld, chunks %lld (s_memtime ticks)\n",
              tw.rows0, tw.rows1, tw.rowsL, nblk, (long long)h[0], (long long)h[1], (long long)h[2], (long long)h[3], (long long)h[8],
              (long long)h[9], (long long)h[10], (long long)h[11]);
    }
    S0 = tw.S0; S1 = tw.S1; SLx = tw.SL; SL2x = SL2; SL3x = SL3;
  } else if (multi) {
    TnMulti tm{};
    tm.M = B; tm.np = 3;
    const int kb0 = (int)cdiv(m->Ip / 16, 3), kb1 = (int)cdiv(m->H2p / 16, 3), kb2 = 1;
    tm.p[0] = {m->h0.p, m->Ip, m->Ip / 16, m->dz0.p, m->H1p, m->H1p / 16, m->slabs0.p,
               (unsigned long long)m->Ip * m->H1p, 0, m->H1p, 0, rpw, S};
    tm.p[1] = {m->dz1.p, m->H2p, m->H2p / 16, A0, m->H1p, m->H1p / 16, m->slabs1.p,
               (unsigned long long)m->H1p * m->H2p, 1, m->H2p, kb0 * S, rpw, S};
    tm.p[2] = {m->dz2.p, 16, 1, A1, m->H2p, m->H2p / 16, m->slabs2.p, (unsigned long long)m->H2p * 16, 1, 16,
               (kb0 + kb1) * S, rpl, SL};
    int nblk = (kb0 + kb1) * S + kb2 * SL;
    if (c.kind == GOCTR_DIN) {
      tm.p[3] = {m->ones16.p, 16, 1, m->attp.p, m->Tp, m->Tp / 16, m->slabs3.p, (unsigned long long)16 * m->Tp, 0, m->Tp,
                 nblk, rpl, SL};
      tm.np = 4;
      nblk += SL;
    }
    static DevBuf<unsigned long long> tndbg;
    const bool dbg = dbg_on("tn");
    if (dbg && !tndbg.p && tndbg.alloc(16)) return -1;
    tm.dbg = dbg ? tndbg.p : nullptr;
    {
      ProfScope ps(GOCTR_K_DW0);
      if (ps.on) prof_note_kernel(GOCTR_K_DW0, "gemm_tn_multi_x3_kernel<3,4>");
      hipLaunchKernelGGL((gemm_tn_multi_x3_kernel<3, 4>), dim3((unsigned)nblk), dim3(512), gemm_tn_multi_x3_lds_bytes<3>(nt_max), e.stream, tm);
      GOCTR_HIP(hipGetLastError());
    }
    if (dbg) {
      unsigned long long h[16];
      if (tndbg.download(h, 16)) return -1;
      fprintf(stderr, "dW x3 wg 0: multiplier wave: wait for chunk 0 %lld, in MFMA sections %lld, loop total %lld, epilogue %lld | stager wave: first chunk %lld, "
              "staging sections %lld, total %lld, chunks %lld (s_memtime ticks)\n", (long long)h[0], (long long)h[1], (long long)h[2], (long long)h[3],
              (long long)h[8], (long long)h[9], (long long)h[10], (long long)h[11]);
    }
  } else {
    if (launch_tn(GOCTR_K_DW0, m->h0.p, m->Ip, m->Ip / 16, m->dz0.p, m->H1p, m->H1p / 16, B, rpw, m->slabs0.p,
                  (size_t)m->Ip * m->H1p)) return -1;
    if (launch_tn(GOCTR_K_DW1, A0, m->H1p, m->H1p / 16, m->dz1.p, m->H2p, m->H2p / 16, B, rpw, m->slabs1.p,
                  (size_t)m->H1p * m->H2p)) return -1;
    if (launch_tn(GOCTR_K_DW2, A1, m->H2p, m->H2p / 16, m->dz2.p, 16, 1, B, rpw, m->slabs2.p, (size_t)m->H2p * 16)) return -1;
    if (c.kind == GOCTR_DIN &&
        launch_tn(GOCTR_K_DW2, m->ones16.p, 16, 1, m->attp.p, m->Tp, m->Tp / 16, B, rpw, m->slabs3.p, (size_t)16 * m->Tp))
      return -1;
  }

  if (m->emb_lr > 0.f && launch_emb_train(m, src, B, st)) return -1;

  ReduceArgs ra{};
  ra.seg[0] = {m->slabs0.p, S0, (unsigned long long)m->Ip * m->H1p, 0, m->Ip * m->H1p};
  ra.seg[1] = {m->slabs1.p, S1, (unsigned long long)m->H1p * m->H2p, m->off1, m->H1p * m->H2p};
  ra.seg[2] = {m->slabs2.p, SL2x > 0 ? SL2x : (multi ? SLx : S), (unsigned long long)m->H2p * 16, m->off2, m->H2p * 16};
  ra.nseg = 3;
  if (c.kind == GOCTR_DIN && !m->att0_early) {
    ra.seg[3] = {m->slabs3.p, SL3x > 0 ? SL3x : (multi ? SLx : S), (unsigned long long)16 * m->Tp, m->offa, m->Tp};
    ra.nseg = 4;
  }
  ra.nflat = m->nflat; ra.lossrow = m->lossrow.p; ra.B = B; ra.G = m->G.p; ra.st = m->st_cur(); ra.st_out = m->st_next(); ra.advance = advance ? 1 : 0;
  if (stage == 1) { m->pend_ra = ra; return 0; }
  return launch_reduce_part(m, src, B, o, advance, fuse_update, ra);
}
namespace {

int launch_reduce_part(goctr_model* m, const RowSource& src, int B, const StepOpts& o, bool advance, bool fuse_update, const ReduceArgs& ra) {
  const goctr_ctr_cfg& c = m->cfg;
  Engine& e = engine();
  if (fuse_update) {
    ReduceAdamArgs p{};
    p.r = ra; p.ad = make_adam_args(m, B, *o.tc);
    p.ra_flag = m->ra_flag.p; p.ra_block = (o.pipelined && c.kind == GOCTR_DIN) ? (m->offa * 2) / 256 : -1;
    if (m->att0_early) {
      p.ra_flag = nullptr; p.ra_block = -1; p.skip_begin = m->offa; p.skip_len = m->Tp;
    }
    ProfScope ps(GOCTR_K_REDUCE);
    if (o.pipelined) {
      if (launch_reduce_attn(m, src, B, o, p)) return -1;
    } else {
      hipLaunchKernelGGL(reduce_adam_kernel, dim3((unsigned)cdiv((int64_t)m->nflat * 2, 256) + 1), dim3(256), 0, e.stream, p);
      GOCTR_HIP(hipGetLastError());
    }
    m->stp ^= 1;
    return 0;
  }
  {
    ProfScope ps(GOCTR_K_REDUCE);
    hipLaunchKernelGGL(reduce_kernel, dim3((unsigned)cdiv((int64_t)m->nflat * 2, 256) + 1), dim3(256), 0, e.stream, ra);
    GOCTR_HIP(hipGetLastError());
  }
  if (advance) m->stp ^= 1;
  return 0;
}

AdamArgs make_adam_args(goctr_model* m, int B, const goctr_train_cfg& tc) {
  Engine& e = engine();
  AdamArgs a{};
  a.W = m->W.p; a.G = m->G.p; a.Mo = m->Mo.p; a.Vo = m->Vo.p; a.nflat = m->nflat;
  a.off1 = m->off1; a.off2 = m->off2; a.offa = m->offa;
  a.Ip = m->Ip; a.H1p = m->H1p; a.H2p = m->H2p; a.Dp = m->Dp; a.U = m->cfg.U; a.D = m->cfg.D;
  a.W1T = m->W1T.p; a.W2T = m->W2T.p; a.W0sT = m->W0sT.p;
  a.W0i = m->img(0); a.W1i = m->img(1); a.W1Ti = m->img(2); a.W0sTi = m->img(3);
  a.x3 = m->x3_images();
  a.W0pvT = (m->emb_lr > 0.f && m->w0pv_live) ? m->W0pvT.p : nullptr; a.Npv = round_up(2 * m->cfg.D, 16);
  a.lr = tc.lr; a.l2 = tc.l2; a.beta1 = tc.beta1; a.beta2 = tc.beta2; a.eps = tc.eps;
  a.div_by_batch = tc.adam_div_by_batch; a.l2_first = tc.adam_l2_before_batch_div;
  a.bglobal = B * e.eff_world(); a.st = m->st_cur(); a.costs = m->costs.p;
  return a;
}

int launch_adam(goctr_model* m, int B, const goctr_train_cfg& tc) {
  AdamArgs a = make_adam_args(m, B, tc);
  ProfScope ps(GOCTR_K_ADAM);
  hipLaunchKernelGGL(adam_kernel, dim3((unsigned)cdiv(m->nflat, 256) + 1), dim3(256), 0, engine().stream, a);
  GOCTR_HIP(hipGetLastError());
  return 0;
}

int launch_adam_step(goctr_model* m, const RowSource& src, int B, const StepOpts& o) {
  if (!(o.pipelined && engine().comm_active())) return launch_adam(m, B, *o.tc);
  int groups = 0;
  const int fast = attn_fast_mode(m, src, &groups);
  const AdamArgs ad = make_adam_args(m, B, *o.tc);
  const AttnArgs aa = make_attn_args(m, src, B, m->st_cur(), m->stp, gate_fac_mode(m, src, o, B));
  const int nadam = (int)cdiv(m->nflat, 256) + 1;
  const int ra_block = m->cfg.kind == GOCTR_DIN ? m->offa / 256 : -1;
  const dim3 grid((unsigned)(nadam + cdiv(B, 4))), blk(256);
  hipStream_t st = engine().active;
  ProfScope ps(GOCTR_K_ADAM);
#define GOCTR_AA(L)                                                                                                       \
  do {                                                                                                                    \
    if (fast == 1) hipLaunchKernelGGL((adam_attn_kernel<4, L, 1>), grid, blk, 0, st, ad, m->ra_flag.p, ra_block, aa, nadam);       \
    else if (fast == 2) hipLaunchKernelGGL((adam_attn_kernel<4, L, 2>), grid, blk, 0, st, ad, m->ra_flag.p, ra_block, aa, nadam);  \
    else hipLaunchKernelGGL((adam_attn_kernel<4, L, 3>), grid, blk, 0, st, ad, m->ra_flag.p, ra_block, aa, nadam);                 \
  } while (0)
  if (groups == 4) GOCTR_AA(4);
  else GOCTR_AA(16);
#undef GOCTR_AA
  GOCTR_HIP(hipGetLastError());
  return 0;
}

int allreduce_grads(goctr_model* m) {
  if (!engine().comm_active()) return 0;
  ProfScope ps(GOCTR_K_ALLREDUCE);
  return comm_allreduce_f32(m->G.p, (size_t)m->nflat + 1);
}

int train_step_eager(goctr_model* m, const RowSource& src, int B, const StepOpts& o) {
  if (launch_forward(m, src, B, o)) return -1;
  const bool fuse = !engine().comm_active();
  if (emb_split3(m)) {
    if (launch_backward(m, src, B, o, true, false, 1) || emb_exchange_a2a(m) || emb_exchange_owner(m) ||
        launch_backward(m, src, B, o, true, false, 2) || emb_exchange_gather(m) || allreduce_grads(m) ||
        emb_exchange_apply(m, src)) return -1;
    return launch_adam(m, B, *o.tc);
  }
  if (launch_backward(m, src, B, o, true, fuse)) return -1;
  if (fuse) return 0;
  if (allreduce_grads(m)) return -1;
  return launch_adam(m, B, *o.tc);
}

bool graph_matches(const StepGraph& g, const goctr_dataset* d, const goctr_emb* e, int B, const StepOpts& o, bool fac) {
  return g.fac == fac && g.a[0] && g.a[1] && g.ds == d->uid && g.emb == (e ? e->uid : 0) && g.B == B && g.mode == o.drop_mode && g.p0 == o.p0 && g.p1 == o.p1 &&
         g.seed == o.seed && g.lr == o.tc->lr && g.l2 == o.tc->l2 && g.b1 == o.tc->beta1 && g.b2 == o.tc->beta2 &&
         g.eps == o.tc->eps && g.flags == o.tc->adam_div_by_batch * 2 + o.tc->adam_l2_before_batch_div &&
         g.world == engine().eff_world() && g.comm == engine().comm_active() && g.pipelined == o.pipelined;
}

int build_graph(goctr_model* m, const goctr_dataset* d, const goctr_emb* emb, const RowSource& src, int B,
                const StepOpts& o) {
  Engine& e = engine();
  m->graph.destroy();
  const bool fuse = !e.comm_active();
  const int stp_now = m->stp;
  struct StpGuard {
    goctr_model* m; int stp; bool ok = false;
    ~StpGuard() { m->stp = stp; if (!ok) m->graph.destroy(); }
  } stp_guard{m, stp_now};
  for (int par = 0; par < 2; ++par) {
    m->stp = par;
    const bool split3 = emb_split3(m);
    int back = m->stp;
    auto restore = [&] { m->stp = back; };
    if (capture_graph(e.stream, &m->graph.a[par], [&] {
          int rc = launch_forward(m, src, B, o) || launch_backward(m, src, B, o, true, fuse, split3 ? 1 : 0);
          if (!rc && !e.comm_active() && !fuse) rc = launch_adam(m, B, *o.tc);
          return rc;
        }, restore)) return -1;
    if (split3) {
      back = m->stp;
      if (capture_graph(e.stream, &m->graph.mid[par], [&] { return emb_exchange_owner(m) || launch_backward(m, src, B, o, true, false, 2); },
                        restore)) return -1;
    }
    if (e.comm_active()) {
      back = m->stp;
      if (capture_graph(e.stream, &m->graph.b[par], [&] { return (split3 && emb_exchange_apply(m, src)) || launch_adam_step(m, src, B, o); },
                        restore)) return -1;
      if (!split3) {
        back = m->stp;
        if (capture_graph(e.stream, &m->graph.ba[par], [&] {
              return launch_adam_step(m, src, B, o) || launch_forward(m, src, B, o) || launch_backward(m, src, B, o, true, false, 0);
            }, restore)) return -1;
      }
    }
  }
  m->stp = stp_now;
  StepGraph& sg = m->graph;
  sg.ds = d->uid; sg.emb = emb ? emb->uid : 0; sg.B = B; sg.mode = o.drop_mode; sg.p0 = o.p0; sg.p1 = o.p1; sg.seed = o.seed;
  sg.lr = o.tc->lr; sg.l2 = o.tc->l2; sg.b1 = o.tc->beta1; sg.b2 = o.tc->beta2; sg.eps = o.tc->eps;
  sg.flags = o.tc->adam_div_by_batch * 2 + o.tc->adam_l2_before_batch_div; sg.world = e.eff_world(); sg.comm = e.comm_active();
  sg.pipelined = o.pipelined; sg.fac = gate_fac_mode(m, src, o, B);
  stp_guard.ok = true;
  return 0;
}

bool dp_capture_ok(const goctr_model* m) {
  const int mode = env_int("GOCTR_DP_CAPTURE_COMM", 1);
  if (mode == 0 || !comm_capturable() || m->emb_lr > 0.f) return false;
  return mode == 2 || engine().capture_state == 1;
}

int build_multi_graphs(goctr_model* m, const RowSource& src, int B, const StepOpts& o) {
  Engine& e = engine();
  StepGraph& sg = m->graph;
  const int stp_now = m->stp;
  const bool dp = e.comm_active();
  const bool fuse = !dp;
  for (int z = 0; z < StepGraph::kNMulti; ++z)
    for (int par = 0; par < 2 && sg.kMulti[z] >= 2; ++par) {
      m->stp = par;
      const int rcg = capture_graph(e.stream, &sg.multi[z][par], [&] {
        int rc = 0;
        for (int k = 0; k < sg.kMulti[z] && !rc; ++k) {
          rc = launch_forward(m, src, B, o) || launch_backward(m, src, B, o, true, fuse);
          if (!rc && dp) rc = allreduce_grads(m) || launch_adam_step(m, src, B, o);
          else if (!rc && !fuse) rc = launch_adam(m, B, *o.tc);
        }
        return rc;
      }, [&] { m->stp = par; });
      m->stp = stp_now;
      if (rcg) return -1;
    }
  sg.multi_on = true;
  return 0;
}

__global__ void step_state_prepare_kernel(StepState* st, double beta1, double beta2, int retarget, long long batch_idx, long long n_batches) {
  StepState s = *st;
  if (retarget) { s.slot = 0; s.batch_idx = batch_idx; s.n_batches = n_batches; }
  state_corrections(s, beta1, beta2);
  *st = s;
}

}
StepOpts opts_from(const goctr_train_cfg* tc) {
  StepOpts o;
  o.tc = tc; o.drop_mode = tc->dropout_mode; o.p0 = tc->p0; o.p1 = tc->p1; o.seed = tc->seed;
  return o;
}

int check_dataset(const goctr_model* m, const goctr_dataset* d, const goctr_emb* e) {
  const goctr_ctr_cfg& c = m->cfg;
  if (d->id_mode) {
    GOCTR_CHECK(e != nullptr, "id-mode dataset needs an embedding table");
    GOCTR_CHECK(e->D == c.D, "embedding dim %d != model D %d", e->D, c.D);
    GOCTR_CHECK(d->U == c.U && d->C == c.C && d->T == c.T, "dataset dims (U=%d,T=%d,C=%d) != model (U=%d,T=%d,C=%d)",
                d->U, d->T, d->C, c.U, c.T, c.C);
  } else {
    const int* r = d->ranges;
    GOCTR_CHECK(r[1] - r[0] == c.U && r[3] - r[2] == c.T * c.D && r[5] - r[4] == c.D && r[7] - r[6] == c.C,
                "SampleInfo ranges do not match the model dims");
    GOCTR_CHECK(r[7] <= d->xcols && r[0] >= 0, "SampleInfo ranges exceed xcols");
  }
  return 0;
}

int mark_weights_written(goctr_model* m) {
  if (!m->ev_weights) GOCTR_HIP(hipEventCreateWithFlags(&m->ev_weights, hipEventDisableTiming));
  GOCTR_HIP(hipEventRecord(m->ev_weights, engine().stream));
  m->weights_pending.store(true, std::memory_order_release);
  return 0;
}
namespace {

int emb_mark_written(goctr_emb* e) {
  if (!e->ev_rows) GOCTR_HIP(hipEventCreateWithFlags(&e->ev_rows, hipEventDisableTiming));
  GOCTR_HIP(hipEventRecord(e->ev_rows, engine().stream));
  e->rows_pending.store(true, std::memory_order_release);
  return 0;
}

int ensure_w0pv(goctr_model* m) {
  if (m->w0pv_live) return 0;
  const goctr_ctr_cfg& c = m->cfg;
  const int Np = round_up(2 * c.D, 16);
  hipLaunchKernelGGL(w0pv_transpose_kernel, dim3((unsigned)cdiv((long long)m->H1p * Np, 256)), dim3(256), 0, engine().stream, m->W.p, m->H1p,
                     c.U, 2 * c.D, Np, m->W0pvT.p);
  GOCTR_HIP(hipGetLastError());
  m->w0pv_live = true;
  m->graph.destroy();
  return 0;
}

int run_steps_impl(goctr_model* m, goctr_emb* emb, goctr_dataset* d, const goctr_train_cfg* tc, int n_steps);

}
int run_steps(goctr_model* m, goctr_emb* emb, goctr_dataset* d, const goctr_train_cfg* tc, int n_steps) {
  const int rc = run_steps_impl(m, emb, d, tc, n_steps);
  if (n_steps > 0) {
    const std::string msg = rc ? goctr_last_error() : "";
    const int mrc = mark_weights_written(m);
    if (m->emb_lr > 0.f && emb) (void)emb_mark_written(emb);
    if (rc) { set_error("%s", msg.c_str()); return -1; }
    if (mrc) return -1;
  }
  return rc;
}
namespace {

int run_steps_impl(goctr_model* m, goctr_emb* emb, goctr_dataset* d, const goctr_train_cfg* tc, int n_steps) {
  Engine& e = engine();
  const int B = tc->batch;
  if (ensure_workspace(m, B)) return -1;
  RowSource src = make_source(d, emb);
  StepOpts o = opts_from(tc);
  if (m->emb_lr > 0.f) {
    GOCTR_CHECK(src.id_mode, "embedding training needs an id-mode dataset (the dense TrainSample rows carry no ids)");
    if (ensure_emb_workspace(m, src.V, B)) return -1;
    if (emb_plan_ok(m, B) && emb_plan_fits(m, d, src.V, B)) { if (ensure_emb_plan(m, d, src, B) || ensure_w0pv(m)) return -1; }
    else { m->plan.valid = false; m->w0pv_live = false; }
  }
  const bool have_start = m->pend_retarget;
  const long long start_batch = m->pend_batch_idx, start_nb = m->pend_n_batches;
  const bool use_graph = !e.prof && env_int("GOCTR_NO_GRAPH", 0) == 0 && !(e.comm_active() && m->emb_lr > 0.f && !emb_split3(m));
  if (use_graph) o.pipelined = pipeline_ok(m, src);
  const goctr_model::H0Carry& cy = m->carry;
  const bool retargeted = have_start;
  const bool carried = use_graph && o.pipelined && n_steps > 0 && cy.valid && retargeted && cy.gen + 1 == m->gen && cy.ds_uid == d->uid &&
                       emb && cy.emb_uid == emb->uid && cy.emb_version == emb->version && cy.B == B && cy.stp == m->stp &&
                       cy.batch == start_batch && cy.beta1 == (double)o.tc->beta1 && cy.beta2 == (double)o.tc->beta2 &&
                       cy.fac == gate_fac_mode(m, src, o, B) &&
                       env_int("GOCTR_H0_CARRY", 1) != 0;
  if (!(carried && m->pend_no_costs)) {
    hipLaunchKernelGGL(step_state_prepare_kernel, dim3(1), dim3(1), 0, e.stream, m->st_cur(), o.tc->beta1, o.tc->beta2,
                       m->pend_retarget ? 1 : 0, m->pend_batch_idx, m->pend_n_batches);
    GOCTR_HIP(hipGetLastError());
  }
  m->pend_retarget = false;
  if (use_graph) {
    if (!graph_matches(m->graph, d, emb, B, o, gate_fac_mode(m, src, o, B)) && build_graph(m, d, emb, src, B, o)) return -1;
    if (o.pipelined && n_steps > 0 && !carried) {
      const AttnArgs aa = make_attn_args(m, src, B, m->st_cur(), m->stp, gate_fac_mode(m, src, o, B));
      if (launch_attn_fwd(aa)) return -1;
    }
    m->carry.valid = false;
    if (m->emb_lr > 0.f && emb && n_steps > 0) ++emb->version;
    int s = 0;
    if ((!e.comm_active() || dp_capture_ok(m)) && env_int("GOCTR_GRAPH_STEPS", 1) != 0) {
      if (!m->graph.multi_on && build_multi_graphs(m, src, B, o)) return -1;
      for (int z = 0; z < StepGraph::kNMulti; ++z) {
        const int sz = m->graph.kMulti[z];
        for (; sz >= 2 && s + sz <= n_steps; s += sz) GOCTR_HIP(hipGraphLaunch(m->graph.multi[z][m->stp], e.stream));
      }
    }
    if (e.comm_active() && m->graph.ba[0] && m->graph.ba[1] && s < n_steps) {
      int par = m->stp;
      GOCTR_HIP(hipGraphLaunch(m->graph.a[par], e.stream));
      for (; s < n_steps; ++s) {
        m->stp ^= 1;
        if (allreduce_grads(m)) return -1;
        if (s + 1 < n_steps) { GOCTR_HIP(hipGraphLaunch(m->graph.ba[par], e.stream)); par ^= 1; }
        else GOCTR_HIP(hipGraphLaunch(m->graph.b[par], e.stream));
      }
    }
    for (; s < n_steps; ++s) {
      const int par = m->stp;
      GOCTR_HIP(hipGraphLaunch(m->graph.a[par], e.stream));
      if (m->graph.mid[par]) {
        if (emb_exchange_a2a(m)) return -1;
        GOCTR_HIP(hipGraphLaunch(m->graph.mid[par], e.stream));
        if (emb_exchange_gather(m)) return -1;
      }
      m->stp ^= 1;
      if (e.comm_active()) {
        if (allreduce_grads(m)) return -1;
        GOCTR_HIP(hipGraphLaunch(m->graph.b[par], e.stream));
      }
    }
    if (o.pipelined && n_steps > 0 && retargeted && emb && start_nb > 0) {
      m->carry = goctr_model::H0Carry{true, m->gen, d->uid, emb->uid, emb->version, B, m->stp, (start_batch + n_steps) % start_nb,
                                      (double)o.tc->beta1, (double)o.tc->beta2, gate_fac_mode(m, src, o, B)};
    }
  } else {
    if (m->emb_lr > 0.f && emb && n_steps > 0) ++emb->version;
    m->carry.valid = false;
    if (!e.prof && !e.comm_active() && n_steps > 0 && env_int("GOCTR_EAGER_PIPELINE", 0) != 0 && pipeline_ok(m, src)) {
      o.pipelined = true;
      const AttnArgs aa = make_attn_args(m, src, B, m->st_cur(), m->stp, gate_fac_mode(m, src, o, B));
      if (launch_attn_fwd(aa)) return -1;
    }
    for (int s = 0; s < n_steps; ++s)
      if (train_step_eager(m, src, B, o)) return -1;
  }
  return 0;
}

}
```

goctr_amd/csrc/ctr_chain_x3.h:

```cpp
#pragma once
#include <hip/hip_runtime.h>

#include "../../include/goctr.h"
#include "ctr_chain.h"
#include "ctr_kernels.h"
#include "mfma_gemm.h"

namespace goctr {

struct ChainX3Args {
  const float* h0; int Ip;
  const unsigned short* img0; const unsigned short* img1; const unsigned short* img2; const unsigned short* img3;
  const float* w2;
  int H1, H2, H1p, H2p, Dp, B; int kind;
  DropCfg d0, d1; const StepState* st;
  const float* Y; long long rows; float inv_bglobal;
  float* A0; float* A1; float* dz0; float* dz1; float* dz2; float* dp; float* yhat; float* lossrow;
  unsigned long long* dbg;
  const int32_t* ab_ids; const float* ab_emb; long long ab_V; const float* ab_gate; const float* ab_wgt; const float* ab_fac; float* ab_out;
  int ab_T, ab_Tp;
  float* tile_dw2; float* tile_att0;
};

constexpr int CX_NSTAMP = 16;

template <int NCH0>
inline size_t chain_x3_lds_bytes() {
  return (size_t)NCH0 * 3 * 1024 + (size_t)8 * CX_NU * 4 * 1024 + (size_t)CX_NCH2 * 3 * 1024 + 8 * 32 * 4;
}

#define CX_MMA6(AH, AC, A, B)                                                         \
  do {                                                                                \
    AC = __builtin_amdgcn_mfma_f32_32x32x16_bf16(A[2], B[0], AC, 0, 0, 0);            \
    AC = __builtin_amdgcn_mfma_f32_32x32x16_bf16(A[0], B[2], AC, 0, 0, 0);            \
    AC = __builtin_amdgcn_mfma_f32_32x32x16_bf16(A[1], B[1], AC, 0, 0, 0);            \
    AC = __builtin_amdgcn_mfma_f32_32x32x16_bf16(A[1], B[0], AC, 0, 0, 0);            \
    AC = __builtin_amdgcn_mfma_f32_32x32x16_bf16(A[0], B[1], AC, 0, 0, 0);            \
    AH = __builtin_amdgcn_mfma_f32_32x32x16_bf16(A[0], B[0], AH, 0, 0, 0);            \
  } while (0)

__device__ __forceinline__ void cx_split8(const float* v, cx_bf8 (&out)[3]) {
  unsigned int h[4], m[4], l[4];
#pragma unroll
  for (int j = 0; j < 4; ++j) tn_split3_pk(v[2 * j], v[2 * j + 1], h[j], m[j], l[j]);
  out[0] = __builtin_bit_cast(cx_bf8, cx_u4{h[0], h[1], h[2], h[3]});
  out[1] = __builtin_bit_cast(cx_bf8, cx_u4{m[0], m[1], m[2], m[3]});
  out[2] = __builtin_bit_cast(cx_bf8, cx_u4{l[0], l[1], l[2], l[3]});
}

struct CxDrop {
  uint32_t hrow, thr, bits, cbase; float kv; bool on;
  __device__ __forceinline__ void init(const DropCfg& d, uint32_t gstep, int row, int col_lane) {
    on = d.mode == 2; bits = 0;
    const float keep = on ? 1.0f - d.p : 1.0f;
    kv = 1.0f / keep;
    uint32_t h = mix32(d.seed ^ 0x9E3779B9u);
    h = mix32(h ^ (gstep * 2u + d.layer));
    hrow = mix32(h ^ (d.row_off + (uint32_t)row));
    thr = on ? (uint32_t)ceilf(keep * 16777216.0f) : 0x1000000u;
    cbase = (uint32_t)col_lane * 0x85EBCA6Bu + 0xC2B2AE35u;
  }
  __device__ __forceinline__ void draw(int col_const, int slot, bool valid) {
    const bool k = valid & ((mix32(hrow ^ (cbase + (uint32_t)col_const * 0x85EBCA6Bu)) >> 8) < thr);
    bits |= k ? (1u << slot) : 0u;
  }
  __device__ __forceinline__ float factor(int slot) const { return (bits >> slot) & 1u ? kv : 0.0f; }
};


template <class Args>
__device__ __forceinline__ void cx_ab_ids_load(const Args& a, int tile, int w, int lane, int (&idv)[4]) {
  const long long b0 = a.st->batch_idx * (long long)a.B;
  const int lc = lane < a.ab_T ? lane : a.ab_T - 1;
#pragma unroll
  for (int s = 0; s < 4; ++s) {
    const int b = tile * 32 + 4 * w + s;
    const int bc = b < a.B ? b : a.B - 1;
    const long long gr = b0 + bc < a.rows ? b0 + bc : a.rows - 1;
    idv[s] = a.ab_ids[gr * a.ab_T + lc];
  }
}
template <class Args>
__device__ __forceinline__ void cx_ab_ids_check(const Args& a, int tile, int w, int lane, long long b0, const int (&idv)[4], int (&abid)[4]) {
#pragma unroll
  for (int s = 0; s < 4; ++s) {
    const int b = tile * 32 + 4 * w + s;
    const int ok = (int)(b < a.B) & (int)(lane < a.ab_T) & (int)(b0 + b < a.rows) & (int)(idv[s] >= 0) & (int)(idv[s] < a.ab_V);
    abid[s] = ok ? idv[s] : (int)a.ab_V;
  }
}
template <class Args>
__device__ __forceinline__ void cx_ab_gw(const Args& a, int tile, int w, int lane, float (&abf)[4]) {
  const int lc = lane < a.ab_T ? lane : a.ab_T - 1;
  if (a.ab_fac) {
    float fv[4];
#pragma unroll
    for (int s = 0; s < 4; ++s) {
      const int b = tile * 32 + 4 * w + s;
      const int bc = b < a.B ? b : a.B - 1;
      fv[s] = a.ab_fac[(size_t)bc * a.ab_T + lc];
    }
#pragma unroll
    for (int s = 0; s < 4; ++s) {
      const int b = tile * 32 + 4 * w + s;
      abf[s] = ((int)(b < a.B) & (int)(lane < a.ab_T)) ? fv[s] : 0.f;
    }
    return;
  }
  float gv[4], wv[4];
#pragma unroll
  for (int s = 0; s < 4; ++s) {
    const int b = tile * 32 + 4 * w + s;
    const int bc = b < a.B ? b : a.B - 1;
    gv[s] = a.ab_gate[(size_t)bc * a.ab_T + lc]; wv[s] = a.ab_wgt[(size_t)bc * a.ab_T + lc];
  }
#pragma unroll
  for (int s = 0; s < 4; ++s) {
    const int b = tile * 32 + 4 * w + s;
    const float f = (gv[s] * (1.0f - gv[s])) * wv[s];
    abf[s] = ((int)(b < a.B) & (int)(lane < a.ab_T)) ? f : 0.f;
  }
}
constexpr int CX_AB_EARLY = 2;
template <class Args>
__device__ __forceinline__ void cx_ab_gather_one(const Args& a, const int (&abid)[4], int lane, int s, int p, float (&abx)[4][4][4]) {
  const int rl = lane >> 2, dl = lane & 3;
  const int id = __shfl(abid[s], 16 * p + rl, 64);
  const float4 t4 = *reinterpret_cast<const float4*>(a.ab_emb + 4 * dl + (size_t)(unsigned)id * 16);
  abx[s][p][0] = t4.x; abx[s][p][1] = t4.y; abx[s][p][2] = t4.z; abx[s][p][3] = t4.w;
}

#ifndef CX_FWD_NFP
#define CX_FWD_NFP 4
#endif
template <int NCH0, bool FWD = false>
__global__ __launch_bounds__(512, 1) void ctr_chain_x3_kernel(ChainX3Args a) {
  extern __shared__ __attribute__((aligned(16))) unsigned char cx_smem[];
  unsigned char* const h0img = cx_smem;
  float* const xch = reinterpret_cast<float*>(cx_smem + (size_t)NCH0 * 3 * 1024);
  unsigned char* const dz1img = reinterpret_cast<unsigned char*>(xch) + (size_t)8 * CX_NU * 4 * 1024;
  float* const z2p = reinterpret_cast<float*>(dz1img + (size_t)CX_NCH2 * 3 * 1024);

  const int tid = threadIdx.x, lane = tid & 63;
  const int w = __builtin_amdgcn_readfirstlane(tid >> 6);
  int n = lane & 31, h = lane >> 5;
  const int ntiles = (a.B + 31) >> 5;
  int vblk = (int)blockIdx.x;
  int tile = xcd_unit_of_block(vblk, ntiles, 4);
  const int tile_first = tile;
  int row = tile * 32 + n;
  bool vrow = row < a.B;
  int rowc = vrow ? row : a.B - 1;
  const int H1p = a.H1p, H2p = a.H2p, Ip = a.Ip;
  const bool own = w < CX_NT0;
  const int tt = own ? w : CX_NT0 - 1;
  const bool din = a.kind == GOCTR_DIN;

  unsigned long long ts[CX_NSTAMP];
#pragma unroll
  for (int k = 0; k < CX_NSTAMP; ++k) ts[k] = 0;
  auto stamp = [&](int k) { if (a.dbg) ts[k] = __builtin_amdgcn_s_memtime(); };
  stamp(0);
  if (FWD && a.dbg) { ts[14] = ts[0]; ts[15] = __builtin_amdgcn_s_memrealtime(); }

  constexpr int NHQ = (NCH0 + 7) / 8;
  cx_f4 hv[NHQ][2];
  auto load_hv = [&](int rc) {
    const float* hp = a.h0 + (size_t)rc * Ip + 8 * h;
#pragma unroll
    for (int cq = 0; cq < NHQ; ++cq) {
      const int c = cq * 8 + w < NCH0 ? cq * 8 + w : NCH0 - 1;
      hv[cq][0] = *reinterpret_cast<const cx_f4*>(hp + c * 16);
      hv[cq][1] = *reinterpret_cast<const cx_f4*>(hp + c * 16 + 4);
    }
  };
  load_hv(rowc);
  int lane_v = lane;
  const cx_u4* g0 = reinterpret_cast<const cx_u4*>(a.img0) + lane_v;
  const cx_u4* g1 = reinterpret_cast<const cx_u4*>(a.img1) + lane_v;
  const cx_u4* g2 = reinterpret_cast<const cx_u4*>(a.img2) + lane_v;
  const cx_u4* g3 = reinterpret_cast<const cx_u4*>(a.img3) + lane_v;

  constexpr int CX_PF0 = NCH0 < 6 ? NCH0 : (FWD ? 5 : 6);
  cx_u4 ra0[CX_PF0][3];
  auto load0 = [&](int c, int slot) {
#pragma unroll
    for (int p = 0; p < 3; ++p) ra0[slot][p] = *(g0 + (size_t)((tt * NCH0 + c) * 3 + p) * 64);
  };
#pragma unroll
  for (int c = 0; c < CX_PF0; ++c) load0(c, c);

  const uint32_t gstep0 = a.st->gstep;
  float y = 0.f;
  if (!FWD) {
    const long long gr = a.st->batch_idx * (long long)a.B + row;
    y = (a.Y && vrow && gr < a.rows) ? a.Y[gr] : 0.f;
  }
  const bool ab = !FWD && din && a.ab_ids != nullptr;
  int abid[4] = {-1, -1, -1, -1}; float abf[4] = {0.f, 0.f, 0.f, 0.f};
  float abx[4][4][4];
  int abidv[4] = {0, 0, 0, 0};
  const long long ab_b0 = ab ? a.st->batch_idx * (long long)a.B : 0;
  if (ab) cx_ab_ids_load(a, tile, w, lane, abidv);
  const int fA = 32 * (w >> 2) + 8 * (w & 3) + 4 * h, fB = 64 + 8 * (w & 3) + 4 * h;
  const bool hasB = w < 4;
  cx_f4 w2pre[2] = {cx_f4{0.f, 0.f, 0.f, 0.f}, cx_f4{0.f, 0.f, 0.f, 0.f}};
  if (FWD) {
    if (fA < H2p) w2pre[0] = *reinterpret_cast<const cx_f4*>(a.w2 + fA);
    if (hasB && fB < H2p) w2pre[1] = *reinterpret_cast<const cx_f4*>(a.w2 + fB);
  }
  for (;;) {
  if (FWD) {
    asm volatile("" : "+v"(lane_v), "+v"(n), "+v"(h));
    g0 = reinterpret_cast<const cx_u4*>(a.img0) + lane_v; g1 = reinterpret_cast<const cx_u4*>(a.img1) + lane_v;
    g2 = reinterpret_cast<const cx_u4*>(a.img2) + lane_v; g3 = reinterpret_cast<const cx_u4*>(a.img3) + lane_v;
  }
  if (FWD && tile != tile_first) {
    stamp(0);
#pragma unroll
    for (int c = CX_FWD_NFP; c < CX_PF0; ++c) load0(c, c);
  }
  CxDrop dr0, dr1;
  dr0.init(a.d0, gstep0, row, 32 * tt + 4 * h);
  dr1.init(a.d1, gstep0, row, 0);

#pragma unroll
  for (int cq = 0; cq < NHQ; ++cq) {
    const int c = cq * 8 + w;
    if (c < NCH0) {
      float v[8] = {hv[cq][0][0], hv[cq][0][1], hv[cq][0][2], hv[cq][0][3], hv[cq][1][0], hv[cq][1][1], hv[cq][1][2], hv[cq][1][3]};
      if (!vrow) {
#pragma unroll
        for (int j = 0; j < 8; ++j) v[j] = 0.f;
      }
      cx_bf8 pl[3];
      cx_split8(v, pl);
#pragma unroll
      for (int p = 0; p < 3; ++p) *reinterpret_cast<cx_bf8*>(h0img + ((size_t)(c * 3 + p) * 64 + lane) * 16) = pl[p];
    }
  }
  __syncthreads();
  stamp(1);
  if (ab) cx_ab_ids_check(a, tile, w, lane, ab_b0, abidv, abid);

  cx_acc ah0, ac0;
#pragma unroll
  for (int i = 0; i < 16; ++i) { ah0[i] = 0.f; ac0[i] = 0.f; }
  auto draw_job = [&](int e) {
    if (FWD) {
      if (e < 16) {
        const int cc = 8 * (e >> 2) + (e & 3);
        dr0.bits |= (own && 32 * tt + 4 * h + cc < a.H1) ? (1u << e) : 0u;
      } else if (e < 24) {
        const bool second = e >= 20;
        const int f = (second ? fB : fA) + (e & 3);
        dr1.bits |= (f < a.H2 && (!second || hasB)) ? (1u << (e - 16)) : 0u;
      }
      return;
    }
    if (e < 16) {
      const int cc = 8 * (e >> 2) + (e & 3);
      dr0.draw(cc, e, own && 32 * tt + 4 * h + cc < a.H1);
    } else if (e < 24) {
      const int r = e & 3;
      const bool second = e >= 20;
      const int f = (second ? fB : fA) + r;
      const bool k = (f < a.H2 && (!second || hasB)) &
                     ((mix32(dr1.hrow ^ ((uint32_t)f * 0x85EBCA6Bu + 0xC2B2AE35u)) >> 8) < dr1.thr);
      dr1.bits |= k ? (1u << (e - 16)) : 0u;
    }
  };
  constexpr int QDRAW = (24 + NCH0 - 1) / NCH0;
  cx_u4 ra1[2][CX_NU][3];
  auto load1_piece = [&](int k) {
    const int j = k / CX_NU, u = k - j * CX_NU;
#pragma unroll
    for (int p = 0; p < 3; ++p) ra1[j][u][p] = *(g1 + (size_t)(((2 * tt + j) * CX_NU + u) * 3 + p) * 64);
  };
#pragma unroll
  for (int c = 0; c < NCH0; ++c) {
    cx_bf8 bf[3], af[3];
#pragma unroll
    for (int p = 0; p < 3; ++p) bf[p] = *reinterpret_cast<const cx_bf8*>(h0img + ((size_t)(c * 3 + p) * 64 + lane) * 16);
#pragma unroll
    for (int p = 0; p < 3; ++p) af[p] = __builtin_bit_cast(cx_bf8, ra0[c % CX_PF0][p]);
    if (c + CX_PF0 < NCH0) load0(c + CX_PF0, c % CX_PF0);
    else if (c + CX_PF0 - NCH0 < 2 * CX_NU) load1_piece(c + CX_PF0 - NCH0);
    CX_MMA6(ah0, ac0, af, bf);
    if (ab) {
      constexpr int NE = 4 * CX_AB_EARLY;
      constexpr int C0 = NCH0 > 4 ? 1 : 0, PER = (NE + (NCH0 - C0) - 1) / (NCH0 - C0);
#pragma unroll
      for (int k = (c - C0) * PER; c >= C0 && k < (c - C0 + 1) * PER && k < NE; ++k) cx_ab_gather_one(a, abid, lane, k >> 2, k & 3, abx);
    }
#pragma unroll
    for (int e = c * QDRAW; e < (c + 1) * QDRAW && e < 24; ++e) draw_job(e);
    asm volatile("" : "+v"(dr0.bits), "+v"(dr1.bits));
    __builtin_amdgcn_sched_barrier(0);
  }
  stamp(2);

#pragma unroll
  for (int k = CX_PF0; k < 2 * CX_NU; ++k) load1_piece(k);

  float p0[16];
  float a0[16];
#pragma unroll
  for (int i = 0; i < 16; ++i) {
    const float s = chain_sigm(ah0[i] + ac0[i]);
    p0[i] = s;
    a0[i] = s * dr0.factor(i);
  }
  if (!FWD && vrow && own) {
#pragma unroll
    for (int g = 0; g < 4; ++g) {
      const int f = 32 * tt + 8 * g + 4 * h;
      if (f < H1p) *reinterpret_cast<cx_f4*>(a.A0 + (size_t)row * H1p + f) = cx_f4{a0[4 * g], a0[4 * g + 1], a0[4 * g + 2], a0[4 * g + 3]};
    }
  }
  stamp(3);

  cx_acc ah1[CX_NU], ac1[CX_NU];
#pragma unroll
  for (int u = 0; u < CX_NU; ++u)
#pragma unroll
    for (int i = 0; i < 16; ++i) { ah1[u][i] = 0.f; ac1[u][i] = 0.f; }
#pragma unroll
  for (int j = 0; j < 2; ++j) {
    cx_bf8 bf[3];
    cx_split8(&a0[8 * j], bf);
#pragma unroll
    for (int u = 0; u < CX_NU; ++u) {
      cx_bf8 af[3];
#pragma unroll
      for (int p = 0; p < 3; ++p) af[p] = __builtin_bit_cast(cx_bf8, ra1[j][u][p]);
      CX_MMA6(ah1[u], ac1[u], af, bf);
    }
  }
  stamp(4);
  cx_u4 ra2[CX_NCH2][3];
  if (!FWD) {
#pragma unroll
    for (int c = 0; c < CX_NCH2; ++c)
#pragma unroll
      for (int p = 0; p < 3; ++p) ra2[c][p] = *(g2 + (size_t)((tt * CX_NCH2 + c) * 3 + p) * 64);
  }

  if (own) {
    float* xw = xch + ((size_t)(w * CX_NU) * 4 * 64 + lane) * 4;
#pragma unroll
    for (int u = 0; u < CX_NU; ++u)
#pragma unroll
      for (int g = 0; g < 4; ++g)
        *reinterpret_cast<cx_f4*>(xw + (size_t)(u * 4 + g) * 256) =
            cx_f4{ah1[u][4 * g] + ac1[u][4 * g], ah1[u][4 * g + 1] + ac1[u][4 * g + 1], ah1[u][4 * g + 2] + ac1[u][4 * g + 2],
                  ah1[u][4 * g + 3] + ac1[u][4 * g + 3]};
  }
  int next_tile = tile;
  if (FWD) {
    vblk += (int)gridDim.x;
    next_tile = vblk < ntiles ? xcd_unit_of_block(vblk, ntiles, 4) : ntiles;
    if (next_tile < ntiles) {
      const int nrow = next_tile * 32 + n;
      load_hv(nrow < a.B ? nrow : a.B - 1);
#pragma unroll
      for (int c = 0; c < CX_FWD_NFP && c < CX_PF0; ++c) load0(c, c);
    }
  }
  __syncthreads();
  stamp(5);
  float s1[2][4], w2v[2][4];
  float part = 0.f;
#pragma unroll
  for (int k = 0; k < 2; ++k) {
    const int u = k == 0 ? (w >> 2) : 2, g = w & 3;
    const int f0 = k == 0 ? fA : fB;
    const bool act = (k == 0 || hasB) && f0 < H2p;
    cx_f4 z = cx_f4{0.f, 0.f, 0.f, 0.f};
    if (k == 0 || hasB) {
#pragma unroll
      for (int ws = 0; ws < CX_NT0; ++ws)
        z += *reinterpret_cast<const cx_f4*>(xch + ((size_t)((ws * CX_NU + u) * 4 + g) * 64 + lane) * 4);
    }
    cx_f4 wv = cx_f4{0.f, 0.f, 0.f, 0.f};
    if (FWD) wv = w2pre[k];
    else if (act) wv = *reinterpret_cast<const cx_f4*>(a.w2 + f0);
    float a1v[4];
#pragma unroll
    for (int r = 0; r < 4; ++r) {
      const float s = chain_sigm(z[r]);
      s1[k][r] = s;
      a1v[r] = s * dr1.factor(k * 4 + r);
      w2v[k][r] = wv[r];
      part += a1v[r] * wv[r];
    }
    if (!FWD && vrow && act && !a.tile_dw2) *reinterpret_cast<cx_f4*>(a.A1 + (size_t)row * H2p + f0) = cx_f4{a1v[0], a1v[1], a1v[2], a1v[3]};
  }
  part += __shfl_xor(part, 32, 64);
  if (h == 0) z2p[w * 32 + n] = part;
  __syncthreads();
  float z2 = z2p[n];
#pragma unroll
  for (int ws = 1; ws < 8; ++ws) z2 += z2p[ws * 32 + n];
  const float yh = sigm_out(z2);
  const bool writer = w == 0 && h == 0 && vrow;
  if (FWD) {
    if (writer) a.yhat[row] = yh;
    stamp(6);
    if (a.dbg) ts[13] = __builtin_amdgcn_s_memrealtime();
    if (a.dbg && blockIdx.x == 0 && lane == 0) {
#pragma unroll
      for (int k = 0; k < CX_NSTAMP; ++k) a.dbg[w * CX_NSTAMP + k] = ts[k];
    }
    if (next_tile >= ntiles) return;
    tile = next_tile;
    row = tile * 32 + n; vrow = row < a.B; rowc = vrow ? row : a.B - 1;
    continue;
  }
  const float one_eps = (float)(1.0 + 1e-8);
  const float dy = -((y / yh) - ((1.0f - y) / (one_eps - yh))) * a.inv_bglobal;
  const float d2 = dy * (yh * (1.0f - yh));
  if (writer) {
    a.yhat[row] = yh;
    a.lossrow[row] = logf(yh) * y + logf(one_eps - yh) * (1.0f - y);
    if (!a.tile_dw2) a.dz2[(size_t)row * 16] = d2;
  }
#pragma unroll
  for (int k = 0; k < 2; ++k) {
    const int f0 = k == 0 ? fA : fB;
    const bool act = (k == 0 || hasB) && f0 < H2p;
    float dz[4];
#pragma unroll
    for (int r = 0; r < 4; ++r) {
      const float s = s1[k][r];
      dz[r] = ((d2 * w2v[k][r]) * dr1.factor(k * 4 + r)) * (s * (1.0f - s));
    }
    if (a.tile_dw2 && (k == 0 || hasB)) {
      const float dv = vrow ? d2 : 0.f;
      cx_f4 pw;
#pragma unroll
      for (int r = 0; r < 4; ++r) pw[r] = group_sum<32>((s1[k][r] * dr1.factor(k * 4 + r)) * dv);
      if (n == 0 && act) *reinterpret_cast<cx_f4*>(a.tile_dw2 + (size_t)tile * H2p + f0) = pw;
    }
    if (act) {
      if (vrow) *reinterpret_cast<cx_f4*>(a.dz1 + (size_t)row * H2p + f0) = cx_f4{dz[0], dz[1], dz[2], dz[3]};
      unsigned int hh[2], mm[2], ll[2];
      tn_split3_pk(dz[0], dz[1], hh[0], mm[0], ll[0]);
      tn_split3_pk(dz[2], dz[3], hh[1], mm[1], ll[1]);
      const int c = f0 >> 4, kg = (f0 >> 3) & 1;
      unsigned char* d = dz1img + ((size_t)(c * 3) * 64 + kg * 32 + n) * 16 + h * 8;
      *reinterpret_cast<cx_u2*>(d) = cx_u2{hh[0], hh[1]};
      *reinterpret_cast<cx_u2*>(d + 1024) = cx_u2{mm[0], mm[1]};
      *reinterpret_cast<cx_u2*>(d + 2048) = cx_u2{ll[0], ll[1]};
    }
  }
  cx_u4 ra3[2][3];
  if (din) {
#pragma unroll
    for (int j = 0; j < 2; ++j)
#pragma unroll
      for (int p = 0; p < 3; ++p) ra3[j][p] = *(g3 + (size_t)((2 * tt + j) * 3 + p) * 64);
  }
  __syncthreads();
  stamp(6);

  cx_acc ahb, acb;
#pragma unroll
  for (int i = 0; i < 16; ++i) { ahb[i] = 0.f; acb[i] = 0.f; }
#pragma unroll
  for (int c = 0; c < CX_NCH2; ++c) {
    cx_bf8 bf[3], af[3];
#pragma unroll
    for (int p = 0; p < 3; ++p) bf[p] = *reinterpret_cast<const cx_bf8*>(dz1img + ((size_t)(c * 3 + p) * 64 + lane) * 16);
#pragma unroll
    for (int p = 0; p < 3; ++p) af[p] = __builtin_bit_cast(cx_bf8, ra2[c][p]);
    CX_MMA6(ahb, acb, af, bf);
  }
  if (ab) cx_ab_gw(a, tile, w, lane, abf);
  if (ab) {
#pragma unroll
    for (int k = 4 * CX_AB_EARLY; k < 16; ++k) cx_ab_gather_one(a, abid, lane, k >> 2, k & 3, abx);
  }
  stamp(7);
  float dzv[16];
#pragma unroll
  for (int i = 0; i < 16; ++i) {
    const float s = p0[i];
    dzv[i] = ((ahb[i] + acb[i]) * dr0.factor(i)) * (s * (1.0f - s));
  }
  if (vrow && own) {
#pragma unroll
    for (int g = 0; g < 4; ++g) {
      const int f = 32 * tt + 8 * g + 4 * h;
      if (f < H1p) *reinterpret_cast<cx_f4*>(a.dz0 + (size_t)row * H1p + f) = cx_f4{dzv[4 * g], dzv[4 * g + 1], dzv[4 * g + 2], dzv[4 * g + 3]};
    }
  }
  if (!din) {
    stamp(8);
    if (a.dbg && blockIdx.x == 0 && lane == 0) {
#pragma unroll
      for (int k = 0; k < CX_NSTAMP; ++k) a.dbg[w * CX_NSTAMP + k] = ts[k];
    }
    return;
  }

  cx_acc ahp, acp;
#pragma unroll
  for (int i = 0; i < 16; ++i) { ahp[i] = 0.f; acp[i] = 0.f; }
#pragma unroll
  for (int j = 0; j < 2; ++j) {
    cx_bf8 bf[3], af[3];
    cx_split8(&dzv[8 * j], bf);
#pragma unroll
    for (int p = 0; p < 3; ++p) af[p] = __builtin_bit_cast(cx_bf8, ra3[j][p]);
    CX_MMA6(ahp, acp, af, bf);
  }
  stamp(8);
  if (own) {
    float* xw = xch + ((size_t)w * 4 * 64 + lane) * 4;
#pragma unroll
    for (int g = 0; g < 4; ++g)
      *reinterpret_cast<cx_f4*>(xw + (size_t)g * 256) = cx_f4{ahp[4 * g] + acp[4 * g], ahp[4 * g + 1] + acp[4 * g + 1],
                                                               ahp[4 * g + 2] + acp[4 * g + 2], ahp[4 * g + 3] + acp[4 * g + 3]};
  }
  __syncthreads();
  if (w < 4) {
    const int d0 = 8 * w + 4 * h;
    if (d0 < a.Dp) {
      cx_f4 z = cx_f4{0.f, 0.f, 0.f, 0.f};
#pragma unroll
      for (int ws = 0; ws < CX_NT0; ++ws) z += *reinterpret_cast<const cx_f4*>(xch + ((size_t)(ws * 4 + w) * 64 + lane) * 4);
      if (vrow && !a.tile_att0) *reinterpret_cast<cx_f4*>(a.dp + (size_t)row * a.Dp + d0) = z;
      if (ab && d0 < 16) {
        const float Tf = (float)a.ab_T;
        *reinterpret_cast<cx_f4*>(reinterpret_cast<float*>(h0img) + n * 16 + d0) = cx_f4{z[0] / Tf, z[1] / Tf, z[2] / Tf, z[3] / Tf};
      }
    }
  }
  if (ab) {
    __syncthreads();
    const float* dpl = reinterpret_cast<const float*>(h0img);
    const int dl = lane & 3, T = a.ab_T;
    const int src = (lane & 15) * 4, pw = lane >> 4;
    float term[4];
#pragma unroll
    for (int s = 0; s < 4; ++s) {
      const cx_f4 dpt = *reinterpret_cast<const cx_f4*>(dpl + (4 * w + s) * 16 + 4 * dl);
      term[s] = 0.f;
#pragma unroll
      for (int p = 0; p < 4; ++p) {
        float dg = 0.f;
#pragma unroll
        for (int e = 0; e < 4; ++e) dg += dpt[e] * abx[s][p][e];
        dg = group_sum<4>(dg);
        const float dgs = __shfl(dg, src, 64);
        if (pw == p) term[s] = dgs;
      }
    }
    if (a.tile_att0) {
      float tsum = 0.f;
#pragma unroll
      for (int s = 0; s < 4; ++s) {
        const int b = tile * 32 + 4 * w + s;
        tsum += (b < a.B && lane < T) ? term[s] * abf[s] : 0.f;
      }
      xch[w * 64 + lane] = tsum;
      __syncthreads();
      if (w == 0 && lane < a.ab_Tp) {
        float sacc = xch[lane];
#pragma unroll
        for (int ws = 1; ws < 8; ++ws) sacc += xch[ws * 64 + lane];
        a.tile_att0[(size_t)tile * a.ab_Tp + lane] = sacc;
      }
    } else {
#pragma unroll
    for (int s = 0; s < 4; ++s) {
      const int b = tile * 32 + 4 * w + s;
      if (b < a.B) {
        float* out = a.ab_out + (size_t)b * a.ab_Tp;
        if (lane < T) out[lane] = term[s] * abf[s];
        for (int t = T + lane; t < a.ab_Tp; t += 64) out[t] = 0.f;
      }
    }
    }
  }
  stamp(9);
  if (a.dbg && blockIdx.x == 0 && lane == 0) {
#pragma unroll
    for (int k = 0; k < CX_NSTAMP; ++k) a.dbg[w * CX_NSTAMP + k] = ts[k];
  }
  break;
  }
}

struct Att0EarlyArgs {
  const float* tile_att0; int ntiles, Tp, tps, nslabs;
  AdamArgs ad; const StepState* st;
};
__device__ __forceinline__ void att0_early_body(const Att0EarlyArgs& e) {
  const int gid = (int)threadIdx.x;
  if (gid >= 2 * e.Tp) return;
  const int c0 = (gid >> 3) * 4, pl = gid & 7;
  const int idx = e.ad.offa + c0 + pl;
  const bool mine = pl < 4 && c0 + pl < e.Tp;
  float w0 = 0.f, m0 = 0.f, v0 = 0.f;
  if (mine) { w0 = e.ad.W[idx]; m0 = e.ad.Mo[idx]; v0 = e.ad.Vo[idx]; }
  const float corr1 = e.st->corr1, corr2 = e.st->corr2;
  const int spp = (e.nslabs + 7) >> 3;
  const int lo = pl * spp;
  int hi = lo + spp; if (hi > e.nslabs) hi = e.nslabs;
  float4 acc = make_float4(0.f, 0.f, 0.f, 0.f);
  for (int j = lo; j < hi; ++j) {
    const int t0 = j * e.tps;
    int t1 = t0 + e.tps; if (t1 > e.ntiles) t1 = e.ntiles;
    float4 s = make_float4(0.f, 0.f, 0.f, 0.f);
    for (int tb = t0; tb < t1; tb += 32) {
      float4 v[32];
#pragma unroll
      for (int u = 0; u < 32; ++u) {
        const int t = tb + u < t1 ? tb + u : t1 - 1;
        v[u] = *reinterpret_cast<const float4*>(e.tile_att0 + (size_t)t * e.Tp + c0);
      }
#pragma unroll
      for (int u = 0; u < 32; ++u) {
        const bool in = tb + u < t1;
        s.x += in ? v[u].x : 0.f; s.y += in ? v[u].y : 0.f; s.z += in ? v[u].z : 0.f; s.w += in ? v[u].w : 0.f;
      }
    }
    acc.x += s.x; acc.y += s.y; acc.z += s.z; acc.w += s.w;
  }
#pragma unroll
  for (int o = 1; o < 8; o <<= 1) {
    acc.x += __shfl_xor(acc.x, o, 64); acc.y += __shfl_xor(acc.y, o, 64);
    acc.z += __shfl_xor(acc.z, o, 64); acc.w += __shfl_xor(acc.w, o, 64);
  }
  if (mine) {
    const float g = pl == 0 ? acc.x : (pl == 1 ? acc.y : (pl == 2 ? acc.z : acc.w));
    adam_apply_pre(e.ad, idx, g, corr1, corr2, w0, m0, v0);
  }
}
template <int KTW0, int KTW1>
__global__ __launch_bounds__(512) void gemm_tn_multi_x3w_att0_kernel(TnMulti a, Att0EarlyArgs e) {
  extern __shared__ __attribute__((aligned(16))) unsigned char goctr_smem[];
  if (blockIdx.x == gridDim.x - 1) { att0_early_body(e); return; }
  tn_multi_x3w_block<KTW0, KTW1>(a, goctr_smem);
}

int chain_x3_fwd_attributes();
int fwd4_attributes();
void launch_fwd4(int nch0, const ChainX3Args& a, dim3 grid, hipStream_t s);
void launch_chain_x3_fwd(int nch0, const ChainX3Args& a, dim3 grid, hipStream_t s);

}
```

goctr_amd/csrc/ctr_kernels.h:

```cpp
#pragma once
#include <hip/hip_runtime.h>
#include <stdint.h>

#include "ctr_x3_images.h"

namespace goctr {

struct StepState {
  unsigned int gstep;
  unsigned int slot;
  long long batch_idx;
  long long n_batches;
  float corr1, corr2;
  float pcorr1, pcorr2;
};
__device__ __forceinline__ void state_corrections(StepState& s, double beta1, double beta2) {
  const double it = (double)s.gstep + 1.0;
  s.corr1 = 1.0f / (float)(1.0 - pow(beta1, it));
  s.corr2 = 1.0f / (float)(1.0 - pow(beta2, it));
}

constexpr int COST_RING = 1 << 16;

__device__ __forceinline__ float sigm_hidden(float x) {
  if (x < -88.f) return 0.f;
  if (x > 15.f) return 1.f;
  return __builtin_amdgcn_rcpf(1.0f + __expf(-x));
}
__device__ __forceinline__ float sigm_out(float x) {
  if (x < -88.f) return 0.f;
  if (x > 15.f) return 1.f;
  return (float)(1.0 / (1.0 + exp((double)(-x))));
}

__device__ __forceinline__ uint32_t mix32(uint32_t x) {
  x ^= x >> 16; x *= 0x7feb352dU; x ^= x >> 15; x *= 0x846ca68bU; x ^= x >> 16;
  return x;
}
__device__ __forceinline__ float dropout_keep(uint32_t seed, uint32_t step, uint32_t layer, uint32_t row,
                                              uint32_t col, float p) {
  uint32_t h = mix32(seed ^ 0x9E3779B9u);
  h = mix32(h ^ (step * 2u + layer));
  h = mix32(h ^ row);
  h = mix32(h ^ (col * 0x85EBCA6Bu + 0xC2B2AE35u));
  float u = (float)(h >> 8) * (1.0f / 16777216.0f);
  return u < (1.0f - p) ? 1.0f : 0.0f;
}

struct RowSource {
  const float* X; int xcols; int r_u, r_ub, r_v, r_c;
  const float* emb; long long V;
  const int32_t* ub_ids; const int32_t* item_ids; const float* ufeat; const float* cfeat;
  const float* Y;
  long long rows;
  int id_mode;
  const int32_t* k_users; const int32_t* k_items; const long long* k_ts;
  const long long* ub_off; const int32_t* ub_items; const long long* ub_ts;
  const float* user_table; const float* item_table; long long n_users, n_items;
  unsigned char* k_failed;
};

struct DropCfg {
  int mode; float p; const float* mask; int mask_ld; uint32_t seed; uint32_t layer; uint32_t row_off;
};

struct AttnArgs {
  RowSource src;
  const StepState* st;
  int B, U, T, D, C, Ip;
  int kind, att;
  const float* att0;
  float* h0;
  float* gate;
  float* wgt;
  float* fac;
  int Tp_att;
  float inv_T;
};

__device__ __forceinline__ float attn_sqrt(float x) { return __builtin_amdgcn_sqrtf(x); }
__device__ __forceinline__ float attn_rcp(float x) { return __builtin_amdgcn_rcpf(x); }

__device__ __forceinline__ int xcd_unit_of_block(int b, int nunits, int per) {
  if (nunits % (8 * per) != 0) return b;
  const int x = b & 7, k = b >> 3;
  return per * (x + 8 * (k / per)) + k % per;
}

__device__ __forceinline__ int xcd_unit_of_block_after(int v, int first, int nunits, int per) {
  if (nunits % (8 * per) != 0) return v - first;
  const int x = v & 7;
  const int k = (v - (first + ((x - first) & 7))) >> 3;
  return per * (x + 8 * (k / per)) + k % per;
}

template <int CTRL>
__device__ __forceinline__ float dpp_f32(float v) {
  return __builtin_bit_cast(float, __builtin_amdgcn_update_dpp(0, __builtin_bit_cast(int, v), CTRL, 0xf, 0xf, true));
}
template <int LPR>
__device__ __forceinline__ float group_sum(float v) {
  if (LPR >= 2) v += dpp_f32<0xB1>(v);
  if (LPR >= 4) v += dpp_f32<0x4E>(v);
  if (LPR >= 8) v += dpp_f32<0x141>(v);
  if (LPR >= 16) v += dpp_f32<0x140>(v);
  if (LPR >= 32) v += __shfl_xor(v, 16, 64);
  if (LPR >= 64) v += __shfl_xor(v, 32, 64);
  return v;
}
template <int LPR>
__device__ __forceinline__ float cross_row_sum(float v) {
  if (LPR <= 1) v += dpp_f32<0xB1>(v);
  if (LPR <= 2) v += dpp_f32<0x4E>(v);
  if (LPR <= 4) v += dpp_f32<0x124>(v);
  if (LPR <= 8) v += dpp_f32<0x128>(v);
  if (LPR <= 16) v += __shfl_xor(v, 16, 64);
  if (LPR <= 32) v += __shfl_xor(v, 32, 64);
  return v;
}

template <int VEC>
__device__ __forceinline__ void load_row(const float* row, int d0, int D, float x[VEC]) {
#pragma unroll
  for (int e = 0; e < VEC; ++e) x[e] = 0.f;
  if (row && d0 < D) {
    if (VEC == 4) {
      float4 t4 = *reinterpret_cast<const float4*>(row + d0);
      x[0] = t4.x; x[1] = t4.y; x[2] = t4.z; x[3] = t4.w;
    } else {
#pragma unroll
      for (int e = 0; e < VEC; ++e) x[e] = d0 + e < D ? row[d0 + e] : 0.f;
    }
  }
}

template <int VEC>
__device__ __forceinline__ void load_row_nn(const float* row, int d0, int D, bool full, float x[VEC]) {
  if (VEC == 4 && full) {
    float4 t4 = *reinterpret_cast<const float4*>(row + d0);
    x[0] = t4.x; x[1] = t4.y; x[2] = t4.z; x[3] = t4.w;
  } else {
    load_row<VEC>(row, d0, D, x);
  }
}

template <int VEC>
__device__ __forceinline__ void load_row_off32(const float* base, int row, int D, int d0, float x[VEC]) {
  const unsigned off = ((unsigned)row * (unsigned)D + (unsigned)d0) * 4u;
  const float4 t4 = *reinterpret_cast<const float4*>(reinterpret_cast<const char*>(base) + off);
  x[0] = t4.x; x[1 % VEC] = t4.y; x[2 % VEC] = t4.z; x[3 % VEC] = t4.w;
}

struct RaCtx { const unsigned int* flag; unsigned int expect; const float* att0; };

struct AttnKey { int user, item; long long ts; };
template <int VEC, int LPR, int FAST, bool KEYS = false>
__device__ __forceinline__ void attn_fwd_body(const AttnArgs& a, int blk, long long batch_idx, const float* att0w,
                                              const RaCtx* ra = nullptr, int sample = -1, const AttnKey* key = nullptr) {
#pragma clang fp contract(fast)
  const bool idm = FAST ? true : (bool)a.src.id_mode;
  const bool din = FAST ? FAST >= 2 : a.kind == GOCTR_DIN;
  const bool cosine = FAST ? FAST == 2 : a.att == GOCTR_ATT_COSINE;
  constexpr int RPP = 64 / LPR;
  constexpr int NPB = LPR < 4 ? LPR : 4;
  const int lane = threadIdx.x & 63;
  const int wave = __builtin_amdgcn_readfirstlane(threadIdx.x >> 6);
  const int b = sample >= 0 ? sample : blk * 4 + wave;
  if (b >= a.B) return;
  const RowSource& s = a.src;
  const long long gr = batch_idx * (long long)a.B + b;
  const bool valid = gr < s.rows;
  const int dl = lane % LPR, rl = lane / LPR;
  const int d0 = dl * VEC;
  const int D = a.D, T = a.T;

  const float* kurow = nullptr; const float* kirow = nullptr;
  int kitem = -1;
  long long kb = 0, kcnt = 0;
  if (KEYS && valid) {
    const int u = key ? key->user : s.k_users[gr];
    const int it = key ? key->item : s.k_items[gr];
    const long long mts = key ? key->ts : (s.k_ts ? s.k_ts[gr] : 0);
    const bool ok = u >= 0 && u < s.n_users && it >= 0 && it < s.n_items;
    if (lane == 0 && s.k_failed) s.k_failed[gr] = ok ? 0 : 1;
    if (ok) {
      kurow = s.user_table + (long long)u * a.U; kirow = s.item_table + (long long)it * a.C; kitem = it;
      const long long b0 = s.ub_off ? s.ub_off[u] : 0, len = s.ub_off ? s.ub_off[u + 1] - b0 : 0;
      if (len > 0) {
        long long lo = 0;
        if (mts != 0) {
          if (len <= 256) {
            lo = len;
            for (long long base = 0; base < len; base += 64) {
              const long long i = base + lane;
              const unsigned long long le = __ballot(i < len && s.ub_ts[b0 + i] <= mts);
              if (le) { lo = base + (long long)__builtin_ctzll(le); break; }
            }
          } else {
            long long hi = len;
            while (lo < hi) {
              const long long mid = (lo + hi) >> 1;
              if (s.ub_ts[b0 + mid] <= mts) hi = mid; else lo = mid + 1;
            }
          }
        }
        kb = b0 + lo;
        kcnt = len - lo < T ? len - lo : T;
      }
    }
  }
  float uside[2] = {0.f, 0.f}, cside[2] = {0.f, 0.f};
  const bool side2 = a.U > 64 || a.C > 64;
#pragma unroll
  for (int k = 0; k < 2; ++k) {
    if (k == 1 && !side2) break;
    const int ju = lane + 64 * k;
    if (KEYS) {
      uside[k] = (kurow && ju < a.U) ? kurow[ju] : 0.f;
      cside[k] = (kirow && ju < a.C) ? kirow[ju] : 0.f;
    } else {
      uside[k] = (valid && ju < a.U) ? (idm ? s.ufeat[gr * a.U + ju] : s.X[gr * (long long)s.xcols + s.r_u + ju]) : 0.f;
      cside[k] = (valid && ju < a.C) ? (idm ? s.cfeat[gr * a.C + ju] : s.X[gr * (long long)s.xcols + s.r_c + ju]) : 0.f;
    }
  }
  int ids64_first = -1;
  if (KEYS) { if (lane < kcnt) ids64_first = s.ub_items[kb + lane]; }
  else if (idm && valid && lane < T) ids64_first = s.ub_ids[gr * T + lane];
  const bool full = FAST ? true : D == LPR * VEC;
  float vv[VEC];
  if (idm) {
    const int it = KEYS ? kitem : (valid ? s.item_ids[gr] : -1);
    if (FAST) load_row_off32<VEC>(s.emb, (it >= 0 && it < s.V) ? it : (int)s.V, D, d0, vv);
    else load_row_nn<VEC>(s.emb + (long long)((it >= 0 && it < s.V) ? it : s.V) * D, d0, D, full, vv);
  } else {
    load_row<VEC>(valid ? s.X + gr * (long long)s.xcols + s.r_v : nullptr, d0, D, vv);
  }
  float syy = 0.f;
#pragma unroll
  for (int e = 0; e < VEC; ++e) syy += vv[e] * vv[e];
  const float yn = attn_sqrt(group_sum<LPR>(syy));

  float psum[VEC];
#pragma unroll
  for (int e = 0; e < VEC; ++e) psum[e] = 0.f;

  constexpr int SLOTS = NPB * RPP;
  for (int tb0 = 0; tb0 < T; tb0 += 64) {
  int ids64 = ids64_first;
  if (tb0 > 0) {
    ids64 = -1;
    if (KEYS) { if (tb0 + lane < kcnt) ids64 = s.ub_items[kb + tb0 + lane]; }
    else if (idm && valid && tb0 + lane < T) ids64 = s.ub_ids[gr * T + tb0 + lane];
  }
  if (FAST) ids64 = (unsigned)ids64 < (unsigned)s.V ? ids64 : (int)s.V;
  auto load_block = [&](int tbx, float (&xx)[NPB][VEC]) {
#pragma unroll
    for (int p = 0; p < NPB; ++p) {
      const int t = tbx + p * RPP + rl;
      if (idm) {
        const int id = __shfl(ids64, (tbx - tb0) + p * RPP + rl, 64);
        if (FAST) load_row_off32<VEC>(s.emb, id, D, d0, xx[p]);
        else load_row_nn<VEC>(s.emb + (long long)((t < T && id >= 0 && id < s.V) ? id : s.V) * D, d0, D, full, xx[p]);
      } else {
        load_row<VEC>((valid && t < T) ? s.X + gr * (long long)s.xcols + s.r_ub + t * D : nullptr, d0, D, xx[p]);
      }
    }
  };
  constexpr int NB = 64 / SLOTS;
  float xb[NB][NPB][VEC];
#pragma unroll
  for (int k = 0; k < NB; ++k)
    if (k == 0 || tb0 + k * SLOTS < T) load_block(tb0 + k * SLOTS, xb[k]);
#pragma unroll
  for (int k = 0; k < NB; ++k) {
    const int tb = tb0 + k * SLOTS;
    if (tb >= T) break;
    float (&x)[NPB][VEC] = xb[k];
    const int src = (lane % RPP) * LPR, pw = lane / RPP;
    float g_l = 1.0f, w_l = 0.f;
    if (din) {
      float s0 = 0.f, s1 = 0.f;
#pragma unroll
      for (int p = 0; p < NPB; ++p) {
        float u0 = 0.f, u1 = 0.f;
        if (cosine) {
#pragma unroll
          for (int e = 0; e < VEC; ++e) { u0 += x[p][e] * x[p][e]; u1 += x[p][e] * vv[e]; }
          u0 = group_sum<LPR>(u0);
          u1 = group_sum<LPR>(u1);
        } else {
#pragma unroll
          for (int e = 0; e < VEC; ++e) { float df = x[p][e] - vv[e]; u0 += (d0 + e < D) ? df * df : 0.f; }
          u0 = group_sum<LPR>(u0);
        }
        const float v0 = __shfl(u0, src, 64), v1 = __shfl(u1, src, 64);
        if (pw == p) { s0 = v0; s1 = v1; }
      }
      if (cosine) {
        const float cosv = s1 * attn_rcp(attn_sqrt(s0) * yn + 1e-8f);
        w_l = (cosv + 1.0f) / 2.0f;
      } else {
        w_l = 1.0f - attn_sqrt(s0);
      }
      const int tl = tb + lane;
      float aw = 0.f;
      if (ra && ra->flag) {
        bool ok = true;
        if (tb == 0) {
          unsigned int spins = 0;
          while (__hip_atomic_load(ra->flag, __ATOMIC_RELAXED, __HIP_MEMORY_SCOPE_AGENT) != ra->expect && ++spins < (1u << 22))
            __builtin_amdgcn_s_sleep(1);
          ok = spins < (1u << 22);
          __builtin_amdgcn_fence(__ATOMIC_ACQUIRE, "wavefront");
        }
        if (lane < NPB * RPP && tl < T) aw = __hip_atomic_load(ra->att0 + tl, __ATOMIC_RELAXED, __HIP_MEMORY_SCOPE_AGENT);
        if (!ok) aw = __builtin_nanf("");
      } else if (lane < NPB * RPP && tl < T) {
        aw = att0w[tl];
      }
      g_l = sigm_hidden(w_l * aw);
    }
    if (a.fac) {
      if (lane < NPB * RPP && tb + lane < T) a.fac[(size_t)b * T + tb + lane] = (g_l * (1.0f - g_l)) * w_l;
    } else if (a.gate && lane < NPB * RPP && tb + lane < T) {
      a.gate[(size_t)b * T + tb + lane] = g_l;
      a.wgt[(size_t)b * T + tb + lane] = w_l;
    }
#pragma unroll
    for (int p = 0; p < NPB; ++p) {
      const int t = tb + p * RPP + rl;
      const float g = din ? __shfl(g_l, p * RPP + rl, 64) : 1.0f;
      if (FAST || t < T) {
#pragma unroll
        for (int e = 0; e < VEC; ++e) psum[e] += g * x[p][e];
      }
    }
  }
  }
  const float invT = a.inv_T;
  float* hrow = a.h0 + (size_t)b * a.Ip;
  if (VEC == 4 && (a.U & 3) == 0 && (a.Ip & 3) == 0 && (D & 3) == 0) {
    typedef float v4 __attribute__((ext_vector_type(4)));
    v4 pv;
#pragma unroll
    for (int e = 0; e < 4; ++e) pv[e] = cross_row_sum<LPR>(psum[e]) * invT;
    if (rl == 0 && d0 < D) {
      *reinterpret_cast<v4*>(hrow + a.U + d0) = pv;
      *reinterpret_cast<v4*>(hrow + a.U + D + d0) = v4{vv[0], vv[1], vv[2], vv[3]};
    }
  } else {
#pragma unroll
    for (int e = 0; e < VEC; ++e) {
      float p = cross_row_sum<LPR>(psum[e]) * invT;
      if (rl == 0 && d0 + e < D) {
        hrow[a.U + d0 + e] = p;
        hrow[a.U + D + d0 + e] = vv[e];
      }
    }
  }
#pragma unroll
  for (int k = 0; k < 2; ++k) {
    if (k == 1 && !side2) break;
    const int j = lane + 64 * k;
    if (j < a.U) hrow[j] = uside[k];
    if (j < a.C) hrow[a.U + 2 * D + j] = cside[k];
  }
  for (int j = lane + 128; j < a.U; j += 64)
    hrow[j] = KEYS ? (kurow ? kurow[j] : 0.f) : (valid ? (idm ? s.ufeat[gr * a.U + j] : s.X[gr * (long long)s.xcols + s.r_u + j]) : 0.f);
  for (int j = lane + 128; j < a.C; j += 64)
    hrow[a.U + 2 * D + j] = KEYS ? (kirow ? kirow[j] : 0.f) : (valid ? (idm ? s.cfeat[gr * a.C + j] : s.X[gr * (long long)s.xcols + s.r_c + j]) : 0.f);
}

template <int VEC, int LPR, int FAST>
__global__ __launch_bounds__(256) void attn_fwd_kernel(AttnArgs a) {
  const int grp = xcd_unit_of_block((int)blockIdx.x, (a.B + 3) >> 2, 32);
  attn_fwd_body<VEC, LPR, FAST>(a, grp, a.st->batch_idx, a.att0);
}
template <int LPR, int FAST>
__global__ __launch_bounds__(256) void attn_fwd_keys_kernel(AttnArgs a) {
  attn_fwd_body<4, LPR, FAST, true>(a, (int)blockIdx.x, 0, a.att0);
}

struct AttnBwdArgs {
  RowSource src;
  const StepState* st;
  int B, T, D, Dp, Tp;
  const float* dp;
  const float* gate;
  const float* wgt;
  float* partial;
};

constexpr int ATTN_BWD_WAVES = 16;

template <int VEC, int LPR, int FAST>
__global__ __launch_bounds__(64 * ATTN_BWD_WAVES) void attn_bwd_kernel(AttnBwdArgs a) {
  const bool idm = FAST ? true : (bool)a.src.id_mode;
  constexpr int RPP = 64 / LPR;
  constexpr int NPB = LPR < 4 ? LPR : 4;
  const int lane = threadIdx.x & 63;
  const int wave = __builtin_amdgcn_readfirstlane(threadIdx.x >> 6);
  const RowSource& s = a.src;
  const int dl = lane % LPR, rl = lane / LPR, d0 = dl * VEC;
  const int D = a.D, T = a.T;
  const int b = blockIdx.x * ATTN_BWD_WAVES + wave;
  if (b >= a.B) return;
  const long long gr = a.st->batch_idx * (long long)a.B + b;
  const bool valid = gr < s.rows;
  float dpt[VEC];
#pragma unroll
  for (int e = 0; e < VEC; ++e) dpt[e] = d0 + e < D ? a.dp[(size_t)b * a.Dp + d0 + e] / (float)T : 0.f;
  float* out = a.partial + (size_t)b * a.Tp;
  for (int t = T + lane; t < a.Tp; t += 64) out[t] = 0.f;
  for (int tb = 0; tb < T; tb += NPB * RPP) {
    int myid = -1;
    if (idm && valid && lane < NPB * RPP && tb + lane < T) myid = s.ub_ids[gr * T + tb + lane];
    float gl = 0.f, wl = 0.f;
    if (lane < NPB * RPP && tb + lane < T) {
      gl = a.gate[(size_t)b * T + tb + lane];
      wl = a.wgt[(size_t)b * T + tb + lane];
    }
    float x[NPB][VEC];
#pragma unroll
    for (int p = 0; p < NPB; ++p) {
      const int t = tb + p * RPP + rl;
      if (idm) {
        const int id = __shfl(myid, p * RPP + rl, 64);
        load_row_nn<VEC>(s.emb + (long long)((t < T && id >= 0 && id < s.V) ? id : s.V) * D, d0, D, FAST ? true : D == LPR * VEC, x[p]);
      } else {
        load_row<VEC>((valid && t < T) ? s.X + gr * (long long)s.xcols + s.r_ub + t * D : nullptr, d0, D, x[p]);
      }
    }
    const float gw = (gl * (1.0f - gl));
    const int src = (lane % RPP) * LPR, pw = lane / RPP;
    float term = 0.f;
#pragma unroll
    for (int p = 0; p < NPB; ++p) {
      float dg = 0.f;
#pragma unroll
      for (int e = 0; e < VEC; ++e) dg += dpt[e] * x[p][e];
      dg = group_sum<LPR>(dg);
      const float dgs = __shfl(dg, src, 64);
      if (pw == p) term = dgs;
    }
    if (lane < NPB * RPP && tb + lane < T) out[tb + lane] = term * (gw * wl);
  }
}

struct EpiSigDrop {
  float* P; float* Aout; int ld; int ncols; DropCfg dr; const StepState* st;
  __device__ __forceinline__ void operator()(int row, int col, float z) const {
    float a = 0.f, post = 0.f;
    if (col < ncols) {
      a = sigm_hidden(z);
      post = a;
      if (dr.mode) {
        const float keep = 1.0f - dr.p;
        float m = dr.mode == 1 ? dr.mask[(size_t)row * dr.mask_ld + col]
                               : dropout_keep(dr.seed, st->gstep, dr.layer, dr.row_off + row, col, dr.p);
        post = a * m / keep;
      }
    }
    P[(size_t)row * ld + col] = a;
    if (Aout != P) Aout[(size_t)row * ld + col] = post;
  }
};

struct EpiOut {
  float* yhat;
  float* lossrow;
  float* dz2;
  const float* Y; long long rows; const StepState* st; int B; float inv_bglobal;
  __device__ __forceinline__ void operator()(int row, int col, float z) const {
    if (col != 0) {
      if (dz2) dz2[(size_t)row * 16 + col] = 0.f;
      return;
    }
    const float p = sigm_out(z);
    yhat[row] = p;
    if (!lossrow) return;
    const long long gr = st->batch_idx * (long long)B + row;
    const float y = (Y && gr < rows) ? Y[gr] : 0.f;
    const float one_eps = (float)(1.0 + 1e-8);
    const float positive = logf(p) * y;
    const float negative = logf(one_eps - p) * (1.0f - y);
    lossrow[row] = positive + negative;
    const float dy = -((y / p) - ((1.0f - y) / (one_eps - p))) * inv_bglobal;
    dz2[(size_t)row * 16] = dy * (p * (1.0f - p));
  }
};

struct EpiDSig {
  float* out; const float* P; int ld; int ncols; DropCfg dr; const StepState* st;
  __device__ __forceinline__ void operator()(int row, int col, float s) const {
    float r = 0.f;
    if (col < ncols) {
      float k = 1.0f;
      if (dr.mode) {
        const float keep = 1.0f - dr.p;
        float m = dr.mode == 1 ? dr.mask[(size_t)row * dr.mask_ld + col]
                               : dropout_keep(dr.seed, st->gstep, dr.layer, dr.row_off + row, col, dr.p);
        k = m / keep;
      }
      const float a = P[(size_t)row * ld + col];
      r = (s * k) * (a * (1.0f - a));
    }
    out[(size_t)row * ld + col] = r;
  }
};

struct EpiStore {
  float* out; int ld;
  __device__ __forceinline__ void operator()(int row, int col, float v) const { out[(size_t)row * ld + col] = v; }
};

struct ReduceSeg { const float* slabs; int nslabs; unsigned long long stride; int begin; int len; };
struct ReduceArgs {
  ReduceSeg seg[4];
  int nseg; int nflat;
  const float* lossrow; int B;
  float* G;
  const StepState* st;
  StepState* st_out;
  int advance;
};

__device__ __forceinline__ void advance_state(const StepState* in, StepState* out) {
  StepState s = *in;
  s.gstep += 1;
  s.slot += 1;
  const long long nb = s.batch_idx + 1;
  s.batch_idx = nb >= s.n_batches ? 0 : nb;
  s.pcorr1 = in->corr1; s.pcorr2 = in->corr2;
  *out = s;
}

__device__ __forceinline__ void loss_sum_block(const float* lossrow, int B, float* red) {
  float s = 0.f;
  for (int i0 = threadIdx.x * 4; i0 < B; i0 += 256 * 4 * 8) {
    float4 v[8];
#pragma unroll
    for (int u = 0; u < 8; ++u) {
      const int i = i0 + u * 1024;
      v[u] = make_float4(0.f, 0.f, 0.f, 0.f);
      if (i + 3 < B) v[u] = *reinterpret_cast<const float4*>(lossrow + i);
      else if (i < B) { v[u].x = lossrow[i]; if (i + 1 < B) v[u].y = lossrow[i + 1]; if (i + 2 < B) v[u].z = lossrow[i + 2]; }
    }
#pragma unroll
    for (int u = 0; u < 8; ++u) s += (v[u].x + v[u].y) + (v[u].z + v[u].w);
  }
  red[threadIdx.x] = s;
  __syncthreads();
  for (int o = 128; o > 0; o >>= 1) {
    if (threadIdx.x < o) red[threadIdx.x] += red[threadIdx.x + o];
    __syncthreads();
  }
}

#ifndef GOCTR_NO_PLAIN_KERNELS
__global__ __launch_bounds__(256) void reduce_kernel(ReduceArgs a) {
  if (blockIdx.x == gridDim.x - 1) {
    __shared__ float red[256];
    loss_sum_block(a.lossrow, a.B, red);
    if (threadIdx.x == 0) {
      a.G[a.nflat] = red[0];
      if (a.advance) advance_state(a.st, a.st_out);
    }
    return;
  }
  const int gid = blockIdx.x * 256 + threadIdx.x;
  const int e0 = (gid >> 3) * 4, p = gid & 7;
  float4 acc = make_float4(0.f, 0.f, 0.f, 0.f);
  if (e0 < a.nflat) {
#pragma unroll
    for (int k = 0; k < 4; ++k) {
      if (k < a.nseg && e0 >= a.seg[k].begin && e0 < a.seg[k].begin + a.seg[k].len) {
        const int spp = (a.seg[k].nslabs + 7) >> 3;
        int lo = p * spp, hi = lo + spp;
        if (hi > a.seg[k].nslabs) hi = a.seg[k].nslabs;
        const float* base = a.seg[k].slabs + (e0 - a.seg[k].begin);
#pragma unroll 8
        for (int j = lo; j < hi; ++j) {
          const float4 v = *reinterpret_cast<const float4*>(base + (size_t)j * a.seg[k].stride);
          acc.x += v.x; acc.y += v.y; acc.z += v.z; acc.w += v.w;
        }
      }
    }
  }
#pragma unroll
  for (int o = 1; o < 8; o <<= 1) {
    acc.x += __shfl_xor(acc.x, o, 64); acc.y += __shfl_xor(acc.y, o, 64);
    acc.z += __shfl_xor(acc.z, o, 64); acc.w += __shfl_xor(acc.w, o, 64);
  }
  if (p == 0 && e0 < a.nflat) *reinterpret_cast<float4*>(a.G + e0) = acc;
}
#endif

struct AdamArgs {
  float* W; float* G; float* Mo; float* Vo; int nflat;
  int off1, off2, offa;
  int Ip, H1p, H2p, Dp, U, D;
  float* W1T; float* W2T; float* W0sT;
  float* W0i; float* W1i; float* W1Ti; float* W0sTi;
  float* W0pvT; int Npv;
  CxImages x3;
  double lr, l2, beta1, beta2, eps;
  int div_by_batch, l2_first;
  int bglobal;
  const StepState* st;
  float* costs;
};

__host__ __device__ inline size_t img_index(int k, int n, int N) { return ((size_t)(k >> 2) * N + n) * 4 + (k & 3); }

__device__ __forceinline__ void adam_apply_pre(const AdamArgs& a, int idx, float g, float corr1, float corr2, float w0, float m0, float v0);
__device__ __forceinline__ void adam_apply(const AdamArgs& a, int idx, float g, float corr1, float corr2) {
  adam_apply_pre(a, idx, g, corr1, corr2, a.W[idx], a.Mo[idx], a.Vo[idx]);
}
__device__ __forceinline__ float adam_new_weight(const AdamArgs& a, float g, float corr1, float corr2, float w0, float m0, float v0,
                                                 float& m, float& v) {
  const float b1 = (float)a.beta1, b2 = (float)a.beta2;
  const float omb1 = 1.0f - b1, omb2 = 1.0f - b2;
  const float l2 = (float)a.l2, eps = (float)a.eps, neg_eta = (float)(-a.lr);
  const float one_per_batch = 1.0f / (float)a.bglobal;
  if (a.l2_first) {
    if (l2 != 0.f) g = g + w0 * l2;
    if (a.div_by_batch && a.bglobal > 1) g = g * one_per_batch;
  } else {
    if (a.div_by_batch && a.bglobal > 1) g = g * one_per_batch;
    if (l2 != 0.f) g = g + w0 * l2;
  }
  const float t1 = omb1 * g;
  const float g2 = (g * g) * omb2;
  m = b1 * m0 + t1;
  v = b2 * v0 + g2;
  const float mhat = m * corr1;
  const float vhat = v * corr2;
  return w0 + (neg_eta * mhat) / (sqrtf(vhat) + eps);
}
__device__ __forceinline__ void adam_apply_pre(const AdamArgs& a, int idx, float g, float corr1, float corr2, float w0, float m0, float v0) {
  float w = w0;
  float m, v;
  w = adam_new_weight(a, g, corr1, corr2, w0, m0, v0, m, v);
  a.Mo[idx] = m; a.Vo[idx] = v;
  a.W[idx] = w;
  if (idx < a.off1) {
    const int r = idx / a.H1p, c = idx - r * a.H1p;
    a.W0i[img_index(r, c, a.H1p)] = w;
    if (r >= a.U && r < a.U + a.D) {
      a.W0sT[(size_t)c * a.Dp + (r - a.U)] = w;
      a.W0sTi[img_index(c, r - a.U, a.Dp)] = w;
    }
    if (a.W0pvT && r >= a.U && r < a.U + 2 * a.D) a.W0pvT[(size_t)c * a.Npv + (r - a.U)] = w;
  } else if (idx < a.off2) {
    const int k = idx - a.off1;
    const int r = k / a.H2p, c = k - r * a.H2p;
    a.W1T[(size_t)c * a.H1p + r] = w;
    a.W1i[img_index(r, c, a.H2p)] = w;
    a.W1Ti[img_index(c, r, a.H1p)] = w;
  } else if (idx < a.offa) {
    const int k = idx - a.off2;
    const int r = k / 16, c = k - r * 16;
    a.W2T[(size_t)c * a.H2p + r] = w;
  }
  cx_scatter_weight(a.x3, w, idx, a.off1, a.off2, a.H1p, a.H2p, a.U, a.D);
}

#ifndef GOCTR_NO_PLAIN_KERNELS
__global__ __launch_bounds__(256) void adam_kernel(AdamArgs a) {
  if (blockIdx.x == gridDim.x - 1) {
    if (threadIdx.x == 0) {
      StepState* w = const_cast<StepState*>(a.st);
      StepState t = *w;
      state_corrections(t, a.beta1, a.beta2);
      w->corr1 = t.corr1; w->corr2 = t.corr2;
    }
    return;
  }
  const int idx = blockIdx.x * 256 + threadIdx.x;
  const float corr[2] = {a.st->pcorr1, a.st->pcorr2};
  if (idx == 0) {
    const float s = a.G[a.nflat];
    a.costs[(a.st->slot - 1u) % COST_RING] = -(s / (float)a.bglobal);
  }
  if (idx >= a.nflat) return;
  const float g = a.G[idx];
  a.G[idx] = 0.f;
  adam_apply(a, idx, g, corr[0], corr[1]);
}
#endif

struct ReduceAdamArgs {
  ReduceArgs r; AdamArgs ad;
  unsigned int* ra_flag; int ra_block;
  int skip_begin, skip_len;
};

__device__ __forceinline__ float4 slab_group_sum(const ReduceArgs& a, int e0, int pl) {
  float4 acc = make_float4(0.f, 0.f, 0.f, 0.f);
  const float* base = a.seg[0].slabs;
  unsigned long long stride = 0;
  int lo = 0, hi = 0;
  if (e0 < a.nflat) {
#pragma unroll
    for (int k = 0; k < 4; ++k) {
      if (k < a.nseg && e0 >= a.seg[k].begin && e0 < a.seg[k].begin + a.seg[k].len) {
        const int spp = (a.seg[k].nslabs + 7) >> 3;
        lo = pl * spp; hi = lo + spp;
        if (hi > a.seg[k].nslabs) hi = a.seg[k].nslabs;
        base = a.seg[k].slabs + (e0 - a.seg[k].begin);
        stride = a.seg[k].stride;
      }
    }
  }
  if (__all(hi - lo <= 8)) {
    float4 v[8];
#pragma unroll
    for (int u = 0; u < 8; ++u) {
      const int j = lo + u < hi ? lo + u : (hi > lo ? hi - 1 : 0);
      v[u] = (hi > lo) ? *reinterpret_cast<const float4*>(base + (size_t)j * stride) : make_float4(0.f, 0.f, 0.f, 0.f);
    }
#pragma unroll
    for (int u = 0; u < 8; ++u)
      if (lo + u < hi) { acc.x += v[u].x; acc.y += v[u].y; acc.z += v[u].z; acc.w += v[u].w; }
  } else {
#pragma unroll 8
    for (int j = lo; j < hi; ++j) {
      const float4 v = *reinterpret_cast<const float4*>(base + (size_t)j * stride);
      acc.x += v.x; acc.y += v.y; acc.z += v.z; acc.w += v.w;
    }
  }
#pragma unroll
  for (int o = 1; o < 8; o <<= 1) {
    acc.x += __shfl_xor(acc.x, o, 64); acc.y += __shfl_xor(acc.y, o, 64);
    acc.z += __shfl_xor(acc.z, o, 64); acc.w += __shfl_xor(acc.w, o, 64);
  }
  return acc;
}

__device__ __forceinline__ void reduce_adam_body(const ReduceAdamArgs& p, int blk_in, int nblk) {
  const ReduceArgs& a = p.r;
  const int blk = p.ra_block < 0 ? blk_in : (blk_in == 0 ? p.ra_block : (blk_in == p.ra_block ? 0 : blk_in));
  __shared__ float red[256];
  if (blk == nblk - 1) {
    StepState ns = *a.st;
    if (threadIdx.x == 0) {
      ns.gstep += 1; ns.slot += 1;
      const long long nb = ns.batch_idx + 1;
      ns.batch_idx = nb >= ns.n_batches ? 0 : nb;
      ns.pcorr1 = ns.corr1; ns.pcorr2 = ns.corr2;
      state_corrections(ns, p.ad.beta1, p.ad.beta2);
    }
    loss_sum_block(a.lossrow, a.B, red);
    if (threadIdx.x == 0) {
      a.G[a.nflat] = red[0];
      p.ad.costs[a.st->slot % COST_RING] = -(red[0] / (float)p.ad.bglobal);
      *a.st_out = ns;
    }
  } else {
    const int gid = blk * 256 + threadIdx.x;
    const int e0 = (gid >> 3) * 4, pl = gid & 7;
    const bool mine = pl < 4 && e0 + pl < a.nflat &&
                      !(e0 + pl >= p.skip_begin && e0 + pl < p.skip_begin + p.skip_len);
    float w0 = 0.f, m0 = 0.f, v0 = 0.f;
    if (mine) { w0 = p.ad.W[e0 + pl]; m0 = p.ad.Mo[e0 + pl]; v0 = p.ad.Vo[e0 + pl]; }
    const float corr1 = a.st->corr1, corr2 = a.st->corr2;
    const float4 acc = slab_group_sum(a, e0, pl);
    if (mine) {
      const float g = pl == 0 ? acc.x : (pl == 1 ? acc.y : (pl == 2 ? acc.z : acc.w));
      adam_apply_pre(p.ad, e0 + pl, g, corr1, corr2, w0, m0, v0);
    }
    if (blk == p.ra_block) {
      if (mine) {
        const float wn = p.ad.W[e0 + pl];
        __hip_atomic_store(p.ad.W + e0 + pl, wn, __ATOMIC_RELAXED, __HIP_MEMORY_SCOPE_AGENT);
      }
      __syncthreads();
      __builtin_amdgcn_fence(__ATOMIC_RELEASE, "wavefront");
      if (threadIdx.x == 0) __hip_atomic_store(p.ra_flag, a.st->gstep + 1u, __ATOMIC_RELAXED, __HIP_MEMORY_SCOPE_AGENT);
    }
  }
}

#ifndef GOCTR_NO_PLAIN_KERNELS
__global__ void step_state_corr_kernel(StepState* st, double beta1, double beta2) {
  StepState s = *st;
  state_corrections(s, beta1, beta2);
  st->corr1 = s.corr1; st->corr2 = s.corr2;
}
#endif

#ifndef GOCTR_NO_PLAIN_KERNELS
__global__ __launch_bounds__(256) void reduce_adam_kernel(ReduceAdamArgs p) {
  reduce_adam_body(p, (int)blockIdx.x, (int)gridDim.x);
}
#endif

template <int VEC, int LPR, int FAST>
__global__ __launch_bounds__(256) void reduce_attn_kernel(ReduceAdamArgs p, AttnArgs a, int nred) {
  if ((int)blockIdx.x < nred) { reduce_adam_body(p, (int)blockIdx.x, nred); return; }
  const ReduceArgs& r = p.r;
  long long nb = r.st->batch_idx + 1;
  if (nb >= r.st->n_batches) nb = 0;
  const RaCtx ctx{p.ra_flag, r.st->gstep + 1u, a.att0};
  const int grp = xcd_unit_of_block_after((int)blockIdx.x, nred, (a.B + 3) >> 2, 32);
  attn_fwd_body<VEC, LPR, FAST>(a, grp, nb, a.att0, FAST >= 2 ? &ctx : nullptr);
}

template <int VEC, int LPR, int FAST>
__global__ __launch_bounds__(256) void adam_attn_kernel(AdamArgs ad, unsigned int* ra_flag, int ra_block, AttnArgs a, int nadam) {
  const int bi = (int)blockIdx.x;
  if (bi < nadam) {
    const int blk = ra_block < 0 ? bi : (bi == 0 ? ra_block : (bi == ra_block ? 0 : bi));
    if (blk == nadam - 1) {
      if (threadIdx.x == 0) {
        StepState* w = const_cast<StepState*>(ad.st);
        StepState t = *w;
        state_corrections(t, ad.beta1, ad.beta2);
        w->corr1 = t.corr1; w->corr2 = t.corr2;
      }
      return;
    }
    const int idx = blk * 256 + threadIdx.x;
    const float c1 = ad.st->pcorr1, c2 = ad.st->pcorr2;
    if (idx == 0) {
      const float sum = ad.G[ad.nflat];
      ad.costs[(ad.st->slot - 1u) % COST_RING] = -(sum / (float)ad.bglobal);
    }
    if (idx < ad.nflat) {
      const float g = ad.G[idx];
      ad.G[idx] = 0.f;
      adam_apply(ad, idx, g, c1, c2);
    }
    if (blk == ra_block) {
      if (idx < ad.nflat) {
        const float wn = ad.W[idx];
        __hip_atomic_store(ad.W + idx, wn, __ATOMIC_RELAXED, __HIP_MEMORY_SCOPE_AGENT);
      }
      __syncthreads();
      __builtin_amdgcn_fence(__ATOMIC_RELEASE, "wavefront");
      if (threadIdx.x == 0) __hip_atomic_store(ra_flag, ad.st->gstep, __ATOMIC_RELAXED, __HIP_MEMORY_SCOPE_AGENT);
    }
    return;
  }
  const RaCtx ctx{ra_flag, ad.st->gstep, a.att0};
  const int grp = xcd_unit_of_block_after(bi, nadam, (a.B + 3) >> 2, 32);
  attn_fwd_body<VEC, LPR, FAST>(a, grp, ad.st->batch_idx, a.att0, FAST >= 2 ? &ctx : nullptr);
}

}
```

goctr_amd/csrc/ctr_model.h:

```cpp
#pragma once
#include <atomic>
#include <functional>
#include <shared_mutex>
#include <vector>

#include "common.h"
#include "ctr_kernels.h"
#include "emb_plan.h"

using namespace goctr;

struct goctr_emb {
  goctr::Engine* const eng = &goctr::engine();
  const uint64_t uid = next_uid();
  uint64_t version = 0;
  int64_t V = 0; int D = 0;
  DevBuf<float> rows;
  std::vector<goctr_emb*> reps; uint64_t reps_version = ~0ull;
  std::shared_mutex mu;
  hipEvent_t ev_rows = nullptr; std::atomic<bool> rows_pending{false};
};

struct goctr_dataset {
  goctr::Engine* const eng = &goctr::engine();
  const uint64_t uid = next_uid();
  bool id_mode = false;
  int64_t rows = 0;
  bool has_y = false;
  DevBuf<float> X; int xcols = 0; int ranges[8] = {0};
  DevBuf<int32_t> ub_ids, item_ids; DevBuf<float> ufeat, cfeat; int U = 0, C = 0, T = 0;
  DevBuf<float> Y;
  std::vector<goctr_dataset*> shards; int shard_B = 0;
  const float* host_X = nullptr; const float* host_Y = nullptr;
};

struct StepGraph {
  hipGraphExec_t a[2] = {nullptr, nullptr}, b[2] = {nullptr, nullptr};
  hipGraphExec_t mid[2] = {nullptr, nullptr};
  hipGraphExec_t ba[2] = {nullptr, nullptr};
  static constexpr int kNMulti = 3;
  int kMulti[kNMulti] = {16, 4, 2};
  hipGraphExec_t multi[kNMulti][2] = {{nullptr, nullptr}, {nullptr, nullptr}, {nullptr, nullptr}};
  bool multi_on = false;
  uint64_t ds = 0, emb = 0; int B = 0; int mode = 0; float p0 = 0, p1 = 0;
  uint32_t seed = 0; double lr = 0, l2 = 0, b1 = 0, b2 = 0, eps = 0; int flags = 0; int world = 1; bool comm = false;
  bool pipelined = false;
  bool fac = false;
  void destroy() {
    bool any = false;
    for (int k = 0; k < 2; ++k) {
      any = any || a[k] || b[k] || mid[k] || ba[k];
      for (int z = 0; z < kNMulti; ++z) any = any || multi[z][k];
    }
    if (any && engine().inited) (void)hipStreamSynchronize(engine().stream);
    for (int k = 0; k < 2; ++k) {
      if (a[k]) (void)hipGraphExecDestroy(a[k]);
      if (b[k]) (void)hipGraphExecDestroy(b[k]);
      if (mid[k]) (void)hipGraphExecDestroy(mid[k]);
      if (ba[k]) (void)hipGraphExecDestroy(ba[k]);
      for (int z = 0; z < kNMulti; ++z) { if (multi[z][k]) (void)hipGraphExecDestroy(multi[z][k]); multi[z][k] = nullptr; }
      a[k] = b[k] = mid[k] = ba[k] = nullptr;
    }
    multi_on = false;
  }
};

struct FwdBufs { float* h0; float* gate; float* wgt; float* yhat; float* P0; float* P1; float* fac = nullptr; };
struct FwdWs {
  DevBuf<float> h0, gate, wgt, yhat, P0, P1;
  int B = 0, Ip = 0, T = 0;
  FwdBufs bufs() { return FwdBufs{h0.p, gate.p, wgt.p, yhat.p, P0.p, P1.p}; }
  int ensure(int Bn, int Ipn, int Tn, int H1p, int H2p, bool modular, hipStream_t st) {
    if (Bn <= B && Ipn == Ip && Tn == T && h0.p && (!modular || P0.p)) return 0;
    GOCTR_HIP(hipStreamSynchronize(st));
    B = 0;
    auto z = [&](DevBuf<float>& b, size_t n) -> int {
      if (b.alloc(n, false)) return -1;
      GOCTR_HIP(hipMemsetAsync(b.p, 0, n * sizeof(float), st));
      return 0;
    };
    const size_t Br = (size_t)round_up(Bn, 32);
    if (z(h0, Br * Ipn) || z(gate, Br * Tn) || z(wgt, Br * Tn) || z(yhat, Br)) return -1;
    if (modular && (z(P0, Br * H1p) || z(P1, Br * H2p))) return -1;
    B = Bn; Ip = Ipn; T = Tn;
    return 0;
  }
};

struct goctr_model {
  goctr::Engine* const eng = &goctr::engine();
  goctr_ctr_cfg cfg{};
  int I = 0, Ip = 0, H1p = 0, H2p = 0, Dp = 0, Tp = 0;
  int off1 = 0, off2 = 0, offa = 0, nflat = 0;
  DevBuf<float> W, G, Mo, Vo, W1T, W2T, W0sT;
  DevBuf<float> Wimg;
  DevBuf<unsigned short> Wx3; int x3_nch0 = 0;
  CxImages x3_images() {
    CxImages im{nullptr, nullptr, nullptr, nullptr, 0};
    if (!x3_nch0) return im;
    im.nch0 = x3_nch0;
    im.img0 = Wx3.p; im.img1 = im.img0 + cx_img0_elems(x3_nch0); im.img2 = im.img1 + cx_img1_elems(); im.img3 = im.img2 + cx_img2_elems();
    return im;
  }
  float* img(int which) { return Wimg.p + (which == 0 ? 0 : which == 1 ? off1 : which == 2 ? off1 + H1p * H2p : off1 + 2 * H1p * H2p); }
  int wsB = 0, tnS = 0;
  DevBuf<float> h0, P0, A0, P1, A1, yhat, lossrow, dz2, dz1, dz0, dp, gate, wgt, gfac, slabs0, slabs1, slabs2, attp;
  DevBuf<float> mask0, mask1, slabs3, ones16;
  size_t gw_stride = 0;
  float* gate_p(int par) { return gate.p + (size_t)par * gw_stride; }
  float* gfac_p(int par) { return gfac.p + (size_t)par * gw_stride; }
  float* wgt_p(int par) { return wgt.p + (size_t)par * gw_stride; }
  DevBuf<unsigned int> ra_flag;
  DevBuf<float> yall;
  FwdWs pws;
  DevBuf<StepState> st, pst;
  int stp = 0;
  StepState* st_cur() { return st.p + stp; }
  StepState* st_next() { return st.p + (stp ^ 1); }
  DevBuf<float> costs;
  std::shared_mutex mu;
  hipEvent_t ev_weights = nullptr; std::atomic<bool> weights_pending{false};
  StepGraph graph;
  int attp_blocks = 0;
  float emb_lr = 0.f;
  long long emb_V = 0; int emb_B = 0, emb_world = 0; bool emb_comm = false;
  DevBuf<float> dpv, W0pvT;
  bool w0pv_live = false;
  uint64_t gen = 0;
  struct H0Carry { bool valid = false; uint64_t gen = 0, ds_uid = 0, emb_uid = 0, emb_version = 0; int B = 0, stp = 0; long long batch = -1;
                   double beta1 = 0, beta2 = 0;
                   bool fac = false;  } carry;
  bool attn_bwd_in_chain = false;
  bool dpv_from_chain = false;
  bool dw2_from_chain = false, att0_from_chain = false;
  bool att0_early = false;
  DevBuf<float> tile_dw2, tile_att0;
  DevBuf<unsigned int> emb_mark, emb_rank, emb_tiles;
  DevBuf<unsigned long long> emb_total;
  DevBuf<long long> emb_accum;
  DevBuf<int> emb_slot_id;
  long long emb_Vw = 0;
  struct EmbPlan {
    bool valid = false; uint64_t ds = 0; long long V = 0; int B = 0, W = 0, T = 0;
    DevBuf<int> pair, pslot, pid, slot_id; DevBuf<unsigned int> slot_off; DevBuf<long long> pair_off, slot_base;
    long long nb = 0, max_pairs = 0, max_slots = 0, total_pairs = 0, total_slots = 0;
    double build_ms = 0;
    EmbPlanView view() const { return EmbPlanView{pair.p, pslot.p, pid.p, pair_off.p, slot_id.p, slot_off.p, slot_base.p}; }
  } plan;
  DevBuf<float> emb_dx, emb_gsum;
  int ex_S = 0, ex_R = 0;
  DevBuf<int> ex_bucket_off, ex_send_ids, ex_recv_ids; DevBuf<long long> ex_send_rows, ex_recv_rows;
  ReduceArgs pend_ra{};
  bool pend_no_costs = false;
  bool pend_retarget = false; long long pend_batch_idx = 0, pend_n_batches = 1;
  DevBuf<int> ex_off, ex_cnt, ex_allcnt, ex_rids, ex_red_ids, ex_nred, ex_allnred, ex_gids;
  DevBuf<long long> ex_rrows, ex_red;
  DevBuf<float> ex_delta, ex_gdelta;
  DevBuf<unsigned long long> ex_red_total;
  double ex_bytes_last = 0;
  std::vector<goctr_model*> reps; uint64_t reps_gen = ~0ull;
};

struct StepOpts {
  bool train = true;
  bool update = true;
  int drop_mode = 0; float p0 = 0, p1 = 0; uint32_t seed = 0;
  const goctr_train_cfg* tc = nullptr;
  bool pipelined = false;
};

int init_kernel_attrs();
int ensure_workspace(goctr_model* m, int B);
RowSource make_source(const goctr_dataset* d, const goctr_emb* e);
StepOpts opts_from(const goctr_train_cfg* tc);
int check_dataset(const goctr_model* m, const goctr_dataset* d, const goctr_emb* e);
bool chain_ok(const goctr_model* m);
int rebuild_x3_images(goctr_model* m);
int attn_fast_mode(const goctr_model* m, const RowSource& src, int* groups);
int launch_forward(goctr_model* m, const RowSource& src, int B, const StepOpts& o, const StepState* st_override = nullptr,
                   const FwdBufs* fbp = nullptr);
int launch_backward(goctr_model* m, const RowSource& src, int B, const StepOpts& o, bool advance,
                    bool fuse_update = false, int stage = 0);
bool serve16_ok(const goctr_model* m, const RowSource& src, int B);
int launch_serve16(goctr_model* m, const RowSource& src, int B, const StepState* st, const FwdBufs& fb, unsigned* done, unsigned epoch);
int mark_weights_written(goctr_model* m);
int run_steps(goctr_model* m, goctr_emb* emb, goctr_dataset* d, const goctr_train_cfg* tc, int n_steps);

bool multi_call(const goctr_model* m, const goctr_train_cfg* cfg);
int train_multi(goctr_model* m, goctr_emb* emb, goctr_dataset* d, const goctr_train_cfg* cfg,
                const std::function<int(goctr_model*, goctr_emb*, goctr_dataset*, const goctr_train_cfg*, int)>& per_rank);
```

Baseline: 202.2 million.

## Stage next batch's behaviour ids, items and labels into a compact double buffer

Adds a staging pass that copies the next batch's user-behaviour ids, item ids and labels into a contiguous, double-buffered scratch buffer. The pass runs as extra workgroups appended to the weight-gradient/att0 launch, and once standalone on the first pipelined step. The attention forward (inside reduce_attn) and the fused chain backward then read ids and labels from this staged buffer. This replaces their scattered, batch-index-dependent dataset gathers, taking the gather off their critical path and letting it overlap with GEMM work. It costs extra memory, an extra grid slice in the TN launch, and more template variants and graph-match state.

```diff
diff --git a/goctr_amd/csrc/ctr.hip b/goctr_amd/csrc/ctr.hip
--- a/goctr_amd/csrc/ctr.hip
+++ b/goctr_amd/csrc/ctr.hip
@@ -106,6 +106,8 @@
   if (m->wgt.alloc((size_t)2 * B * m->cfg.T)) return -1;
   if (m->gfac.alloc((size_t)2 * B * m->cfg.T)) return -1;
   m->gw_stride = (size_t)B * m->cfg.T;
+  m->stage_stride = stage_ints(B, m->cfg.T);
+  if (m->stage.alloc(2 * m->stage_stride)) return -1;
   if (m->ra_flag.alloc(1)) return -1;
   if (m->slabs0.alloc((size_t)S * m->Ip * m->H1p)) return -1;
   if (m->slabs1.alloc((size_t)S * m->H1p * m->H2p)) return -1;
@@ -227,6 +229,8 @@
       allow_big_lds(gemm_tn_kernel<float, 3, 4, 32>) ||
       allow_big_lds(gemm_tn_multi_x3_kernel<3, 4>) || allow_big_lds(gemm_tn_multi_x3w_kernel<9, 5>) || allow_big_lds(gemm_tn_multi_x3w_kernel<8, 5>) ||
       allow_big_lds(gemm_tn_multi_x3w_att0_kernel<9, 5>) || allow_big_lds(gemm_tn_multi_x3w_att0_kernel<8, 5>) || allow_big_lds(ctr_chain_x3_kernel<2>) || allow_big_lds(ctr_chain_x3_kernel<9>) ||
+      allow_big_lds(gemm_tn_multi_x3w_att0_kernel<9, 5, true>) || allow_big_lds(gemm_tn_multi_x3w_att0_kernel<8, 5, true>) ||
+      allow_big_lds(ctr_chain_x3_kernel<2, false, true>) || allow_big_lds(ctr_chain_x3_kernel<9, false, true>) || allow_big_lds(ctr_chain_x3_kernel<15, false, true>) ||
       allow_big_lds(ctr_chain_x3_kernel<15>) || chain_x3_fwd_attributes() || fwd4_attributes() ||
       serve16_attributes()) return -1;
   done = true;
@@ -370,12 +374,14 @@
 template <int NCH0>
 void launch_chain_x3_n(const ChainX3Args& a, dim3 grid, hipStream_t s, bool fwd) {
   if (fwd) launch_chain_x3_fwd(NCH0, a, grid, s);
+  else if (a.stage) hipLaunchKernelGGL((ctr_chain_x3_kernel<NCH0, false, true>), grid, dim3(512), chain_x3_lds_bytes<NCH0>(), s, a);
   else hipLaunchKernelGGL((ctr_chain_x3_kernel<NCH0, false>), grid, dim3(512), chain_x3_lds_bytes<NCH0>(), s, a);
 }
 
 bool emb_plan_active(const goctr_model* m) { return m->emb_lr > 0.f && m->plan.valid; }
 
 bool gate_fac_mode(const goctr_model* m, const RowSource& src, const StepOpts& o, int B);
+bool stage_ids_mode(const goctr_model* m, const RowSource& src, const StepOpts& o, int B);
 int launch_chain_x3(goctr_model* m, const RowSource& src, int B, const StepOpts& o, const StepState* st, const FwdBufs& fb) {
   const goctr_ctr_cfg& c = m->cfg;
   Engine& e = engine();
@@ -398,6 +404,7 @@
     a.ab_ids = src.ub_ids; a.ab_emb = src.emb; a.ab_V = src.V; a.ab_gate = fb.gate; a.ab_wgt = fb.wgt; a.ab_out = m->attp.p;
     a.ab_fac = gate_fac_mode(m, src, o, B) ? fb.fac : nullptr;
     a.ab_T = c.T; a.ab_Tp = m->Tp;
+    a.stage = stage_ids_mode(m, src, o, B) ? m->stage_p(m->stp) : nullptr;
   }
   a.yhat = fb.yhat; a.lossrow = m->lossrow.p;
   const bool tile_sums = o.train && dw_wide_path(m, B) && env_int("GOCTR_CHAIN_TILE_SUMS", 1) != 0;
@@ -558,6 +565,13 @@
   return o.train && c.kind == GOCTR_DIN && src.id_mode && m->emb_lr <= 0.f && c.D == 16 && c.T <= 64 && chain_ok(m) &&
          chain_x3_ok(m, o, B) && env_int("GOCTR_CHAIN_ATTN_BWD", 1) != 0;
 }
+bool stage_ids_mode(const goctr_model* m, const RowSource& src, const StepOpts& o, int B) {
+  return o.pipelined && !engine().comm_active() && gate_fac_mode(m, src, o, B) && dw_wide_path(m, B) &&
+         env_int("GOCTR_CHAIN_TILE_SUMS", 1) != 0 && m->Tp % 32 == 0 && env_int("GOCTR_STAGE_IDS", 1) != 0;
+}
+StageArgs make_stage_args(goctr_model* m, const RowSource& src, int B, const StepState* st, bool advance, int32_t* out, int nblk) {
+  return StageArgs{src.ub_ids, src.item_ids, src.Y, src.rows, st, B, m->cfg.T, advance ? 1 : 0, out, nblk};
+}
 AttnArgs make_attn_args(goctr_model* m, const RowSource& src, int B, const StepState* st, const FwdBufs& fb, bool fac) {
   const goctr_ctr_cfg& c = m->cfg;
   AttnArgs aa{};
@@ -598,13 +612,16 @@
 int launch_reduce_attn(goctr_model* m, const RowSource& src, int B, const StepOpts& o, const ReduceAdamArgs& p) {
   int groups = 0;
   const int fast = attn_fast_mode(m, src, &groups);
-  const AttnArgs aa = make_attn_args(m, src, B, p.r.st, m->stp ^ 1, gate_fac_mode(m, src, o, B));
+  AttnArgs aa = make_attn_args(m, src, B, p.r.st, m->stp ^ 1, gate_fac_mode(m, src, o, B));
+  if (stage_ids_mode(m, src, o, B) && groups == 4) aa.stage = m->stage_p(m->stp ^ 1);
   const int nred = (int)cdiv((int64_t)m->nflat * 2, 256) + 1;
   const dim3 grid((unsigned)(nred + cdiv(B, 4))), blk(256);
   hipStream_t st = engine().active;
 #define GOCTR_RA(L)                                                                                        \
   do {                                                                                                     \
     if (fast == 1) hipLaunchKernelGGL((reduce_attn_kernel<4, L, 1>), grid, blk, 0, st, p, aa, nred);       \
+    else if (aa.stage && fast == 2) hipLaunchKernelGGL((reduce_attn_kernel<4, L, 2, true>), grid, blk, 0, st, p, aa, nred);  \
+    else if (aa.stage) hipLaunchKernelGGL((reduce_attn_kernel<4, L, 3, true>), grid, blk, 0, st, p, aa, nred);               \
     else if (fast == 2) hipLaunchKernelGGL((reduce_attn_kernel<4, L, 2>), grid, blk, 0, st, p, aa, nred);  \
     else hipLaunchKernelGGL((reduce_attn_kernel<4, L, 3>), grid, blk, 0, st, p, aa, nred);                 \
   } while (0)
@@ -1101,6 +1118,9 @@
       tm.np = 4;
       nblk += SL3;
     }
+    const bool stage_w = stage_ids_mode(m, src, o, B);
+    GOCTR_CHECK(!stage_w || m->att0_early, "id staging needs the weight-gradient launch's att0 workgroup");
+    const StageArgs sg = make_stage_args(m, src, B, st, true, m->stage_p(m->stp ^ 1), stage_w ? 15 : 0);
     static DevBuf<unsigned long long> tndbgw;
     const bool dbg = dbg_on("tn");
     if (dbg && !tndbgw.p && tndbgw.alloc(16)) return -1;
@@ -1111,9 +1131,12 @@
       if (m->att0_early) {
         if (ps.on) prof_note_kernel(GOCTR_K_DW0, tw.ktw0 == 9 ? "gemm_tn_multi_x3w_att0_kernel<9,5>" : "gemm_tn_multi_x3w_att0_kernel<8,5>");
         if (tw.ktw0 == 9)
-          hipLaunchKernelGGL((gemm_tn_multi_x3w_att0_kernel<9, 5>), dim3((unsigned)nblk + 1), dim3(512), gemm_tn_multi_x3w_lds_bytes<9>(), e.stream, tm, ae);
+          if (stage_w) hipLaunchKernelGGL((gemm_tn_multi_x3w_att0_kernel<9, 5, true>), dim3((unsigned)(nblk + 1 + sg.nblk)), dim3(512), gemm_tn_multi_x3w_lds_bytes<9>(), e.stream, tm, ae, sg);
+          else hipLaunchKernelGGL((gemm_tn_multi_x3w_att0_kernel<9, 5>), dim3((unsigned)nblk + 1), dim3(512), gemm_tn_multi_x3w_lds_bytes<9>(), e.stream, tm, ae, sg);
+        else if (stage_w)
+          hipLaunchKernelGGL((gemm_tn_multi_x3w_att0_kernel<8, 5, true>), dim3((unsigned)(nblk + 1 + sg.nblk)), dim3(512), gemm_tn_multi_x3w_lds_bytes<8>(), e.stream, tm, ae, sg);
         else
-          hipLaunchKernelGGL((gemm_tn_multi_x3w_att0_kernel<8, 5>), dim3((unsigned)nblk + 1), dim3(512), gemm_tn_multi_x3w_lds_bytes<8>(), e.stream, tm, ae);
+          hipLaunchKernelGGL((gemm_tn_multi_x3w_att0_kernel<8, 5>), dim3((unsigned)nblk + 1), dim3(512), gemm_tn_multi_x3w_lds_bytes<8>(), e.stream, tm, ae, sg);
       } else
       if (tw.ktw0 == 9)
         hipLaunchKernelGGL((gemm_tn_multi_x3w_kernel<9, 5>), dim3((unsigned)nblk), dim3(512), gemm_tn_multi_x3w_lds_bytes<9>(), e.stream, tm);
@@ -1290,8 +1313,8 @@
   return launch_adam(m, B, *o.tc);
 }
 
-bool graph_matches(const StepGraph& g, const goctr_dataset* d, const goctr_emb* e, int B, const StepOpts& o, bool fac) {
-  return g.fac == fac && g.a[0] && g.a[1] && g.ds == d->uid && g.emb == (e ? e->uid : 0) && g.B == B && g.mode == o.drop_mode && g.p0 == o.p0 && g.p1 == o.p1 &&
+bool graph_matches(const StepGraph& g, const goctr_dataset* d, const goctr_emb* e, int B, const StepOpts& o, bool fac, bool stage) {
+  return g.fac == fac && g.stage == stage && g.a[0] && g.a[1] && g.ds == d->uid && g.emb == (e ? e->uid : 0) && g.B == B && g.mode == o.drop_mode && g.p0 == o.p0 && g.p1 == o.p1 &&
          g.seed == o.seed && g.lr == o.tc->lr && g.l2 == o.tc->l2 && g.b1 == o.tc->beta1 && g.b2 == o.tc->beta2 &&
          g.eps == o.tc->eps && g.flags == o.tc->adam_div_by_batch * 2 + o.tc->adam_l2_before_batch_div &&
          g.world == engine().eff_world() && g.comm == engine().comm_active() && g.pipelined == o.pipelined;
@@ -1339,7 +1362,7 @@
   sg.ds = d->uid; sg.emb = emb ? emb->uid : 0; sg.B = B; sg.mode = o.drop_mode; sg.p0 = o.p0; sg.p1 = o.p1; sg.seed = o.seed;
   sg.lr = o.tc->lr; sg.l2 = o.tc->l2; sg.b1 = o.tc->beta1; sg.b2 = o.tc->beta2; sg.eps = o.tc->eps;
   sg.flags = o.tc->adam_div_by_batch * 2 + o.tc->adam_l2_before_batch_div; sg.world = e.eff_world(); sg.comm = e.comm_active();
-  sg.pipelined = o.pipelined; sg.fac = gate_fac_mode(m, src, o, B);
+  sg.pipelined = o.pipelined; sg.fac = gate_fac_mode(m, src, o, B); sg.stage = stage_ids_mode(m, src, o, B);
   stp_guard.ok = true;
   return 0;
 }
@@ -1375,6 +1398,15 @@
   return 0;
 }
 
+int launch_stage_first(goctr_model* m, const RowSource& src, int B, const StepOpts& o) {
+  if (!stage_ids_mode(m, src, o, B)) return 0;
+  const int nblk = (int)std::min<long long>(64, cdiv((long long)B * m->cfg.T, 256 * 4 * 8));
+  const StageArgs sg = make_stage_args(m, src, B, m->st_cur(), false, m->stage_p(m->stp), std::max(1, nblk));
+  hipLaunchKernelGGL(stage_ids_kernel, dim3((unsigned)sg.nblk), dim3(256), 0, engine().stream, sg);
+  GOCTR_HIP(hipGetLastError());
+  return 0;
+}
+
 __global__ void step_state_prepare_kernel(StepState* st, double beta1, double beta2, int retarget, long long batch_idx, long long n_batches) {
   StepState s = *st;
   if (retarget) { s.slot = 0; s.batch_idx = batch_idx; s.n_batches = n_batches; }
@@ -1469,7 +1501,7 @@
   const bool carried = use_graph && o.pipelined && n_steps > 0 && cy.valid && retargeted && cy.gen + 1 == m->gen && cy.ds_uid == d->uid &&
                        emb && cy.emb_uid == emb->uid && cy.emb_version == emb->version && cy.B == B && cy.stp == m->stp &&
                        cy.batch == start_batch && cy.beta1 == (double)o.tc->beta1 && cy.beta2 == (double)o.tc->beta2 &&
-                       cy.fac == gate_fac_mode(m, src, o, B) &&
+                       cy.fac == gate_fac_mode(m, src, o, B) && cy.stage == stage_ids_mode(m, src, o, B) &&
                        env_int("GOCTR_H0_CARRY", 1) != 0;
   if (!(carried && m->pend_no_costs)) {
     hipLaunchKernelGGL(step_state_prepare_kernel, dim3(1), dim3(1), 0, e.stream, m->st_cur(), o.tc->beta1, o.tc->beta2,
@@ -1478,8 +1510,10 @@
   }
   m->pend_retarget = false;
   if (use_graph) {
-    if (!graph_matches(m->graph, d, emb, B, o, gate_fac_mode(m, src, o, B)) && build_graph(m, d, emb, src, B, o)) return -1;
+    if (!graph_matches(m->graph, d, emb, B, o, gate_fac_mode(m, src, o, B), stage_ids_mode(m, src, o, B)) && build_graph(m, d, emb, src, B, o))
+      return -1;
     if (o.pipelined && n_steps > 0 && !carried) {
+      if (launch_stage_first(m, src, B, o)) return -1;
       const AttnArgs aa = make_attn_args(m, src, B, m->st_cur(), m->stp, gate_fac_mode(m, src, o, B));
       if (launch_attn_fwd(aa)) return -1;
     }
@@ -1519,13 +1553,14 @@
     }
     if (o.pipelined && n_steps > 0 && retargeted && emb && start_nb > 0) {
       m->carry = goctr_model::H0Carry{true, m->gen, d->uid, emb->uid, emb->version, B, m->stp, (start_batch + n_steps) % start_nb,
-                                      (double)o.tc->beta1, (double)o.tc->beta2, gate_fac_mode(m, src, o, B)};
+                                      (double)o.tc->beta1, (double)o.tc->beta2, gate_fac_mode(m, src, o, B), stage_ids_mode(m, src, o, B)};
     }
   } else {
     if (m->emb_lr > 0.f && emb && n_steps > 0) ++emb->version;
     m->carry.valid = false;
     if (!e.prof && !e.comm_active() && n_steps > 0 && env_int("GOCTR_EAGER_PIPELINE", 0) != 0 && pipeline_ok(m, src)) {
       o.pipelined = true;
+      if (launch_stage_first(m, src, B, o)) return -1;
       const AttnArgs aa = make_attn_args(m, src, B, m->st_cur(), m->stp, gate_fac_mode(m, src, o, B));
       if (launch_attn_fwd(aa)) return -1;
     }
diff --git a/goctr_amd/csrc/ctr_chain_x3.h b/goctr_amd/csrc/ctr_chain_x3.h
--- a/goctr_amd/csrc/ctr_chain_x3.h
+++ b/goctr_amd/csrc/ctr_chain_x3.h
@@ -20,6 +20,7 @@
   const int32_t* ab_ids; const float* ab_emb; long long ab_V; const float* ab_gate; const float* ab_wgt; const float* ab_fac; float* ab_out;
   int ab_T, ab_Tp;
   float* tile_dw2; float* tile_att0;
+  const int32_t* stage;
 };
 
 constexpr int CX_NSTAMP = 16;
@@ -81,11 +82,22 @@
   }
 }
 template <class Args>
-__device__ __forceinline__ void cx_ab_ids_check(const Args& a, int tile, int w, int lane, long long b0, const int (&idv)[4], int (&abid)[4]) {
+__device__ __forceinline__ void cx_ab_ids_load_staged(const Args& a, int tile, int w, int lane, int (&idv)[4]) {
+  const int lc = lane < a.ab_T ? lane : a.ab_T - 1;
 #pragma unroll
   for (int s = 0; s < 4; ++s) {
     const int b = tile * 32 + 4 * w + s;
-    const int ok = (int)(b < a.B) & (int)(lane < a.ab_T) & (int)(b0 + b < a.rows) & (int)(idv[s] >= 0) & (int)(idv[s] < a.ab_V);
+    const int bc = b < a.B ? b : a.B - 1;
+    idv[s] = a.stage[(size_t)bc * a.ab_T + lc];
+  }
+}
+template <bool STAGED, class Args>
+__device__ __forceinline__ void cx_ab_ids_check(const Args& a, int tile, int w, int lane, long long b0, const int (&idv)[4], int (&abid)[4]) {
+#pragma unroll
+  for (int s = 0; s < 4; ++s) {
+    const int b = tile * 32 + 4 * w + s;
+    const int in_rows = STAGED ? 1 : (int)(b0 + b < a.rows);
+    const int ok = (int)(b < a.B) & (int)(lane < a.ab_T) & in_rows & (int)(idv[s] >= 0) & (int)(idv[s] < a.ab_V);
     abid[s] = ok ? idv[s] : (int)a.ab_V;
   }
 }
@@ -133,7 +145,7 @@
 #ifndef CX_FWD_NFP
 #define CX_FWD_NFP 4
 #endif
-template <int NCH0, bool FWD = false>
+template <int NCH0, bool FWD = false, bool STAGE = false>
 __global__ __launch_bounds__(512, 1) void ctr_chain_x3_kernel(ChainX3Args a) {
   extern __shared__ __attribute__((aligned(16))) unsigned char cx_smem[];
   unsigned char* const h0img = cx_smem;
@@ -156,6 +168,12 @@
   const int tt = own ? w : CX_NT0 - 1;
   const bool din = a.kind == GOCTR_DIN;
 
+  float y = 0.f;
+  const bool ab = !FWD && din && a.ab_ids != nullptr;
+  int abid[4] = {-1, -1, -1, -1}; float abf[4] = {0.f, 0.f, 0.f, 0.f};
+  float abx[4][4][4];
+  int abidv[4] = {0, 0, 0, 0};
+
   unsigned long long ts[CX_NSTAMP];
 #pragma unroll
   for (int k = 0; k < CX_NSTAMP; ++k) ts[k] = 0;
@@ -175,6 +193,10 @@
     }
   };
   load_hv(rowc);
+  if constexpr (STAGE) {
+    y = stage_labels(a.stage, a.B, a.ab_T)[rowc];
+    if (ab) cx_ab_ids_load_staged(a, tile, w, lane, abidv);
+  }
   int lane_v = lane;
   const cx_u4* g0 = reinterpret_cast<const cx_u4*>(a.img0) + lane_v;
   const cx_u4* g1 = reinterpret_cast<const cx_u4*>(a.img1) + lane_v;
@@ -191,17 +213,15 @@
   for (int c = 0; c < CX_PF0; ++c) load0(c, c);
 
   const uint32_t gstep0 = a.st->gstep;
-  float y = 0.f;
-  if (!FWD) {
-    const long long gr = a.st->batch_idx * (long long)a.B + row;
-    y = (a.Y && vrow && gr < a.rows) ? a.Y[gr] : 0.f;
-  }
-  const bool ab = !FWD && din && a.ab_ids != nullptr;
-  int abid[4] = {-1, -1, -1, -1}; float abf[4] = {0.f, 0.f, 0.f, 0.f};
-  float abx[4][4][4];
-  int abidv[4] = {0, 0, 0, 0};
-  const long long ab_b0 = ab ? a.st->batch_idx * (long long)a.B : 0;
-  if (ab) cx_ab_ids_load(a, tile, w, lane, abidv);
+  long long ab_b0 = 0;
+  if constexpr (!STAGE) {
+    if (!FWD) {
+      const long long gr = a.st->batch_idx * (long long)a.B + row;
+      y = (a.Y && vrow && gr < a.rows) ? a.Y[gr] : 0.f;
+    }
+    ab_b0 = ab ? a.st->batch_idx * (long long)a.B : 0;
+    if (ab) cx_ab_ids_load(a, tile, w, lane, abidv);
+  }
   const int fA = 32 * (w >> 2) + 8 * (w & 3) + 4 * h, fB = 64 + 8 * (w & 3) + 4 * h;
   const bool hasB = w < 4;
   cx_f4 w2pre[2] = {cx_f4{0.f, 0.f, 0.f, 0.f}, cx_f4{0.f, 0.f, 0.f, 0.f}};
@@ -241,7 +261,7 @@
   }
   __syncthreads();
   stamp(1);
-  if (ab) cx_ab_ids_check(a, tile, w, lane, ab_b0, abidv, abid);
+  if (ab) cx_ab_ids_check<STAGE>(a, tile, w, lane, ab_b0, abidv, abid);
 
   cx_acc ah0, ac0;
 #pragma unroll
@@ -418,6 +438,7 @@
     continue;
   }
   const float one_eps = (float)(1.0 + 1e-8);
+  if constexpr (STAGE) y = vrow ? y : 0.f;
   const float dy = -((y / yh) - ((1.0f - y) / (one_eps - yh))) * a.inv_bglobal;
   const float d2 = dy * (yh * (1.0f - yh));
   if (writer) {
@@ -639,10 +660,16 @@
     adam_apply_pre(e.ad, idx, g, corr1, corr2, w0, m0, v0);
   }
 }
-template <int KTW0, int KTW1>
-__global__ __launch_bounds__(512) void gemm_tn_multi_x3w_att0_kernel(TnMulti a, Att0EarlyArgs e) {
+template <int KTW0, int KTW1, bool STAGE = false>
+__global__ __launch_bounds__(512) void gemm_tn_multi_x3w_att0_kernel(TnMulti a, Att0EarlyArgs e, StageArgs sg) {
   extern __shared__ __attribute__((aligned(16))) unsigned char goctr_smem[];
-  if (blockIdx.x == gridDim.x - 1) { att0_early_body(e); return; }
+  if constexpr (STAGE) {
+    const int first_stage = (int)gridDim.x - sg.nblk;
+    if ((int)blockIdx.x >= first_stage) { stage_ids_body(sg, (int)blockIdx.x - first_stage); return; }
+    if ((int)blockIdx.x == first_stage - 1) { att0_early_body(e); return; }
+  } else {
+    if (blockIdx.x == gridDim.x - 1) { att0_early_body(e); return; }
+  }
   tn_multi_x3w_block<KTW0, KTW1>(a, goctr_smem);
 }
 
diff --git a/goctr_amd/csrc/ctr_kernels.h b/goctr_amd/csrc/ctr_kernels.h
--- a/goctr_amd/csrc/ctr_kernels.h
+++ b/goctr_amd/csrc/ctr_kernels.h
@@ -76,7 +76,73 @@
   float* fac;
   int Tp_att;
   float inv_T;
-};
+  const int32_t* stage;
+};
+
+__host__ __device__ inline const int32_t* stage_items(const int32_t* stage, int B, int T) { return stage + (size_t)B * T; }
+__host__ __device__ inline const float* stage_labels(const int32_t* stage, int B, int T) {
+  return reinterpret_cast<const float*>(stage + (size_t)B * T + B);
+}
+__host__ __device__ inline size_t stage_ints(int B, int T) { return ((size_t)B * T + 2 * (size_t)B + 63) & ~(size_t)63; }
+
+struct StageArgs {
+  const int32_t* ub_ids; const int32_t* item_ids; const float* Y; long long rows;
+  const StepState* st; int B, T;
+  int advance;
+  int32_t* out;
+  int nblk;
+};
+typedef int stage_v4 __attribute__((ext_vector_type(4)));
+__device__ __forceinline__ void stage_store4(int32_t* base, unsigned idx, stage_v4 v) {
+  asm volatile("global_store_dwordx4 %0, %1, %2 sc1" : : "v"(idx * 4u), "v"(v), "s"(base) : "memory");
+}
+__device__ __forceinline__ void stage_store1(int32_t* base, unsigned idx, int v) {
+  asm volatile("global_store_dword %0, %1, %2 sc1" : : "v"(idx * 4u), "v"(v), "s"(base) : "memory");
+}
+__device__ __forceinline__ void stage_ids_body(const StageArgs& s, int blk) {
+  long long nb = s.st->batch_idx;
+  if (s.advance) { nb += 1; if (nb >= s.st->n_batches) nb = 0; }
+  const long long nids = (long long)s.B * s.T;
+  const long long id0 = nb * nids, id_end = s.rows * (long long)s.T;
+  const int nthr = s.nblk * (int)blockDim.x, tid = blk * (int)blockDim.x + (int)threadIdx.x;
+  if ((nids & 3) == 0) {
+    const long long nvec = nids >> 2;
+    for (long long j0 = tid; j0 < nvec; j0 += 8ll * nthr) {
+      stage_v4 v[8];
+#pragma unroll
+      for (int u = 0; u < 8; ++u) {
+        const long long j = j0 + (long long)u * nthr, g = id0 + 4 * j;
+        v[u] = stage_v4{-1, -1, -1, -1};
+        if (j < nvec) {
+          if (g + 4 <= id_end) v[u] = *reinterpret_cast<const stage_v4*>(s.ub_ids + g);
+          else {
+            if (g < id_end) v[u][0] = s.ub_ids[g];
+            if (g + 1 < id_end) v[u][1] = s.ub_ids[g + 1];
+            if (g + 2 < id_end) v[u][2] = s.ub_ids[g + 2];
+          }
+        }
+      }
+#pragma unroll
+      for (int u = 0; u < 8; ++u) {
+        const long long j = j0 + (long long)u * nthr;
+        if (j < nvec) stage_store4(s.out, (unsigned)(4 * j), v[u]);
+      }
+    }
+  } else {
+    for (long long i = tid; i < nids; i += nthr) stage_store1(s.out, (unsigned)i, id0 + i < id_end ? s.ub_ids[id0 + i] : -1);
+  }
+  for (int b = tid; b < s.B; b += nthr) {
+    const long long gr = nb * s.B + b;
+    const bool valid = gr < s.rows;
+    const int it = valid ? s.item_ids[gr] : -1;
+    const float y = (valid && s.Y) ? s.Y[gr] : 0.f;
+    stage_store1(s.out, (unsigned)(nids + b), it);
+    stage_store1(s.out, (unsigned)(nids + s.B + b), __float_as_int(y));
+  }
+}
+#ifndef GOCTR_NO_PLAIN_KERNELS
+__global__ __launch_bounds__(256) void stage_ids_kernel(StageArgs s) { stage_ids_body(s, (int)blockIdx.x); }
+#endif
 
 __device__ __forceinline__ float attn_sqrt(float x) { return __builtin_amdgcn_sqrtf(x); }
 __device__ __forceinline__ float attn_rcp(float x) { return __builtin_amdgcn_rcpf(x); }
@@ -154,9 +220,10 @@
 struct RaCtx { const unsigned int* flag; unsigned int expect; const float* att0; };
 
 struct AttnKey { int user, item; long long ts; };
-template <int VEC, int LPR, int FAST, bool KEYS = false>
+template <int VEC, int LPR, int FAST, bool KEYS = false, bool STAGE = false>
 __device__ __forceinline__ void attn_fwd_body(const AttnArgs& a, int blk, long long batch_idx, const float* att0w,
-                                              const RaCtx* ra = nullptr, int sample = -1, const AttnKey* key = nullptr) {
+                                              const RaCtx* ra = nullptr, int sample = -1, const AttnKey* key = nullptr,
+                                              const StepState* next_of = nullptr) {
 #pragma clang fp contract(fast)
   const bool idm = FAST ? true : (bool)a.src.id_mode;
   const bool din = FAST ? FAST >= 2 : a.kind == GOCTR_DIN;
@@ -168,6 +235,16 @@
   const int b = sample >= 0 ? sample : blk * 4 + wave;
   if (b >= a.B) return;
   const RowSource& s = a.src;
+  int st_id = -1, st_item = -1;
+  if constexpr (STAGE) {
+    if (lane < a.T) st_id = a.stage[(size_t)b * a.T + lane];
+    st_item = stage_items(a.stage, a.B, a.T)[b];
+    __builtin_amdgcn_sched_barrier(0);
+    if (next_of) {
+      batch_idx = next_of->batch_idx + 1;
+      if (batch_idx >= next_of->n_batches) batch_idx = 0;
+    }
+  }
   const long long gr = batch_idx * (long long)a.B + b;
   const bool valid = gr < s.rows;
   const int dl = lane % LPR, rl = lane / LPR;
@@ -225,11 +302,12 @@
   }
   int ids64_first = -1;
   if (KEYS) { if (lane < kcnt) ids64_first = s.ub_items[kb + lane]; }
+  else if (STAGE) ids64_first = st_id;
   else if (idm && valid && lane < T) ids64_first = s.ub_ids[gr * T + lane];
   const bool full = FAST ? true : D == LPR * VEC;
   float vv[VEC];
   if (idm) {
-    const int it = KEYS ? kitem : (valid ? s.item_ids[gr] : -1);
+    const int it = KEYS ? kitem : STAGE ? st_item : (valid ? s.item_ids[gr] : -1);
     if (FAST) load_row_off32<VEC>(s.emb, (it >= 0 && it < s.V) ? it : (int)s.V, D, d0, vv);
     else load_row_nn<VEC>(s.emb + (long long)((it >= 0 && it < s.V) ? it : s.V) * D, d0, D, full, vv);
   } else {
@@ -796,10 +874,16 @@
 }
 #endif
 
-template <int VEC, int LPR, int FAST>
+template <int VEC, int LPR, int FAST, bool STAGE = false>
 __global__ __launch_bounds__(256) void reduce_attn_kernel(ReduceAdamArgs p, AttnArgs a, int nred) {
   if ((int)blockIdx.x < nred) { reduce_adam_body(p, (int)blockIdx.x, nred); return; }
   const ReduceArgs& r = p.r;
+  if constexpr (STAGE) {
+    const RaCtx ctx{p.ra_flag, p.ra_flag ? r.st->gstep + 1u : 0u, a.att0};
+    const int grp = xcd_unit_of_block_after((int)blockIdx.x, nred, (a.B + 3) >> 2, 32);
+    attn_fwd_body<VEC, LPR, FAST, false, true>(a, grp, 0, a.att0, FAST >= 2 ? &ctx : nullptr, -1, nullptr, r.st);
+    return;
+  }
   long long nb = r.st->batch_idx + 1;
   if (nb >= r.st->n_batches) nb = 0;
   const RaCtx ctx{p.ra_flag, r.st->gstep + 1u, a.att0};
diff --git a/goctr_amd/csrc/ctr_model.h b/goctr_amd/csrc/ctr_model.h
--- a/goctr_amd/csrc/ctr_model.h
+++ b/goctr_amd/csrc/ctr_model.h
@@ -46,6 +46,7 @@
   uint32_t seed = 0; double lr = 0, l2 = 0, b1 = 0, b2 = 0, eps = 0; int flags = 0; int world = 1; bool comm = false;
   bool pipelined = false;
   bool fac = false;
+  bool stage = false;
   void destroy() {
     bool any = false;
     for (int k = 0; k < 2; ++k) {
@@ -110,6 +111,8 @@
   float* gate_p(int par) { return gate.p + (size_t)par * gw_stride; }
   float* gfac_p(int par) { return gfac.p + (size_t)par * gw_stride; }
   float* wgt_p(int par) { return wgt.p + (size_t)par * gw_stride; }
+  DevBuf<int32_t> stage; size_t stage_stride = 0;
+  int32_t* stage_p(int par) { return stage.p + (size_t)par * stage_stride; }
   DevBuf<unsigned int> ra_flag;
   DevBuf<float> yall;
   FwdWs pws;
@@ -129,7 +132,8 @@
   uint64_t gen = 0;
   struct H0Carry { bool valid = false; uint64_t gen = 0, ds_uid = 0, emb_uid = 0, emb_version = 0; int B = 0, stp = 0; long long batch = -1;
                    double beta1 = 0, beta2 = 0;
-                   bool fac = false;  } carry;
+                   bool fac = false;
+                   bool stage = false;  } carry;
   bool attn_bwd_in_chain = false;
   bool dpv_from_chain = false;
   bool dw2_from_chain = false, att0_from_chain = false;
```

New measurement: 203.3 million, median of 6. No clear change (+0.5%).
